# tgsstdio/BirdNest.Audio

Measured on AMD Instinct MI355X. Metric: decoded PCM MSamples/s/GPU (bit-exact) + achieved HBM GB/s vs roofline, higher is better.
Workload: dtype int32; 1 GPU; C2: 1024-frame batches, 44.1 kHz/16-bit stereo, bs 4096, LPC-8, Rice partition order 4 -> FLACDecoder 16-bit LE interleaved PCM; frames_per_batch=1024, compressed_bytes_per_batch=10724000, pcm_bytes_per_batch=16777216, parallelism=corpus of 1 x 1024 batches partitioned per rank (shard.partition) x1

## Files before the change

### birdnest/audio_amd/csrc/bnflac_kernels.hip

```cpp
#include <stdlib.h>
#include <atomic>
#include <mutex>

#include "bnf_bitreader.h"
#include "bnf_crc16.h"
#include "bnf_crc16_tab.h"
#include "bnf_frame.h"
#include "bnf_residual.h"

#define WR_SLOTS 8
#define WR_WIN 256u
struct WR {
    const uint32_t *__restrict__ w;
    uint32_t nblk;
    lds_u32 *ring;
    uint32_t w0;
    uint32_t issued;
    uint32_t landed;
    uint64_t pos;
    uint64_t st[8];
};
DEV uint32_t wr_u(uint32_t v) { return __builtin_amdgcn_readfirstlane(v); }
DEV void wr_issue(WR &r) {
    const uint32_t j = r.issued++;
// ... 617 lines not shown
        uint32_t incl = x;
        for (int o = 1; o < 64; o <<= 1) {
            uint32_t y = __shfl_up(incl, o);
            if ((threadIdx.x & 63) >= (unsigned)o) incl += y;
        }
        if ((threadIdx.x & 63) == 63) wsum[threadIdx.x >> 6] = incl;
        __syncthreads();
        if (threadIdx.x < 16) {
            uint32_t s = wsum[threadIdx.x];
            for (int o = 1; o < 16; o <<= 1) {
                uint32_t y = __shfl_up(s, o, 16);
                if (threadIdx.x >= (unsigned)o) s += y;
            }
            wsum[threadIdx.x] = s;
        }
        __syncthreads();
        uint32_t wprefix = (threadIdx.x >= 64) ? wsum[(threadIdx.x >> 6) - 1] : 0u;
        if (i < n) v[i] = carry + wprefix + incl - x;
        __syncthreads();
        if (threadIdx.x == 1023) carry += wprefix + incl;
        __syncthreads();
    }
    if (threadIdx.x == 0) *total = carry;
}

__global__ void __launch_bounds__(SCAN_THREADS) k_sync_write(const uint8_t *__restrict__ d, uint64_t n,
                                                             const uint32_t *__restrict__ block_offs,
                                                             uint64_t *__restrict__ out, uint32_t cap) {
    __shared__ uint32_t wtot[SCAN_THREADS / 64];
    uint64_t base = ((uint64_t)blockIdx.x * SCAN_THREADS + threadIdx.x) * SCAN_BYTES_PER_THREAD;
    uint32_t c = 0;
    for (int i = 0; i < SCAN_BYTES_PER_THREAD; i++) c += is_sync(d, n, base + i) ? 1u : 0u;
    uint32_t incl = c;
    const uint32_t lane = threadIdx.x & 63;
    for (int o = 1; o < 64; o <<= 1) {
        uint32_t y = __shfl_up(incl, o);
        if (lane >= (unsigned)o) incl += y;
    }
    if (lane == 63) wtot[threadIdx.x >> 6] = incl;
    __syncthreads();
    uint32_t wpre = 0;
    for (uint32_t wv = 0; wv < (threadIdx.x >> 6); wv++) wpre += wtot[wv];
    uint32_t pos = block_offs[blockIdx.x] + wpre + incl - c;
    for (int i = 0; i < SCAN_BYTES_PER_THREAD; i++) {
        if (is_sync(d, n, base + i)) {
            if (pos < cap) out[pos] = base + i;
            pos++;
        }
    }
}

#define PARSE_RD 8
static_assert(PARSE_RD == 8, "pk_ra and the walk's pair steps (slot masks 0x3F3 / 0x1C0C, slot bits 10-12) assume an 8-slot ring");
template <int CPM>
DEV void parse_frame(const uint32_t *__restrict__ words, uint64_t nbytes, const uint64_t *__restrict__ frame_offs,
                     uint32_t nframes, const bnf_stream_params &sp, const uint64_t *__restrict__ out_sample_in,
                     uint64_t base_sample, bnf_frame_info *__restrict__ info, uint32_t ablate, lds_u32 *ring,
                     uint32_t f, uint32_t *__restrict__ crcp) {
    if (f >= nframes) return;
    bnf_frame_info fi;
    fi.status = BNF_ST_OK;
    fi.err = -1;
    fi.frame_off = frame_offs[f];
    fi.resume_bit = 0;
    fi.cached = -1;
    fi.blocksize = fi.sample_rate = fi.channels = fi.assignment = fi.bps = 0;
    fi.number_type = 0;
    fi.unparseable = 0;
    fi.number = 0;
    fi.out_sample = 0;
    fi.crc8 = fi.crc16_calc = fi.crc16_read = fi.crc_ok = 0;
    fi.flags = 0;
    fi.reserved = 0;
    uint32_t ss[8];
#pragma unroll
    for (int c = 0; c < 8; c++) ss[c] = 0;
    const uint64_t limit = nbytes * 8u;
    const uint64_t fbit = fi.frame_off * 8u;
    BR b;
    br_init(b, words, nbytes, ring, threadIdx.x, PARSE_RD);
    CrcP cp;
    crcp_init(cp);
    uint32_t st = parse_header(b, fbit, limit, sp, fi);
    if (st == BNF_ST_ERROR && br_pos(b) > limit) st = BNF_ST_TRUNC;
    if (CPM && crcp != nullptr && st == BNF_ST_OK && fi.channels == 2u && !(ablate & BNF_ABLATE_NO_WALK)) {
        const uint32_t h = (uint32_t)(fi.frame_off & 63u);
        const uint64_t l0 = fi.frame_off & ~(uint64_t)63u, lend = (nbytes + 15u) & ~(uint64_t)15u;
        const u32x4 *g = (const u32x4 *)((const uint8_t *)words + l0);
        u32x4 v[4];
#pragma unroll
        for (uint32_t i = 0; i < 4; i++) {
            v[i] = l0 + 16u * i < lend ? g[i] : u32x4{0u, 0u, 0u, 0u};
            v[i].x &= st_hmask(h, 16u * i);
            v[i].y &= st_hmask(h, 16u * i + 4u);
            v[i].z &= st_hmask(h, 16u * i + 8u);
            v[i].w &= st_hmask(h, 16u * i + 12u);
        }
        cp.wc = (uint32_t)(fi.frame_off >> 6);
        crcp_fold(cp, v);
    }
    if (st == BNF_ST_OK) {
        uint64_t sample;
        if (fi.number_type == 1) sample = fi.number;
        else if (sp.has_stream_info && sp.min_blocksize == sp.max_blocksize) sample = (uint64_t)sp.min_blocksize * fi.number;
        else sample = (uint64_t)fi.blocksize * fi.number;
        fi.out_sample = out_sample_in ? out_sample_in[f] : sample - base_sample;
        uint32_t maxorder = 0;
        bool raw = false;
        for (uint32_t ch = 0; ch < fi.channels; ch++) {
            const uint32_t here = (uint32_t)(br_pos(b) - fbit);
#pragma unroll
            for (int c = 0; c < 8; c++) ss[c] = (uint32_t)c == ch ? here : ss[c];
            if (ch + 1 == fi.channels) {
                const uint32_t x = br_peek(b) >> 24;
                if (!(x & 0x80u) && (x & 0x7Eu) >= 0x40u) maxorder = max(maxorder, ((x >> 1) & 31u) + 1u);
                raw = raw || (x & 0x7Eu) < 4u;
                break;
            }
            if (ablate & BNF_ABLATE_NO_WALK) {
#pragma unroll
                for (int c = 0; c < 8; c++) ss[c] = (uint32_t)c == ch + 1 ? here : ss[c];
                continue;
            }
            SubHdr h;
            int32_t err = -1;
            uint32_t bps = sub_bps(fi, ch);
            st = parse_subframe_head<false>(b, bps, fi.blocksize, limit, h, nullptr, nullptr, err);
            if (st == BNF_ST_OK) {
                if (h.type == T_LPC) maxorder = max(maxorder, h.order);
                raw = raw || h.type == T_CONST || h.type == T_VERB;
                if (!(h.type == T_FIXED || h.type == T_LPC) || h.order > (fi.bps > 16u ? 12u : 8u)) cp.wc = ~0u;
                if (h.type == T_VERB) br_skip(b, (uint64_t)h.bps * fi.blocksize);
                else if (h.type == T_FIXED || h.type == T_LPC) st = skip_residual<CPM != 0>(b, h, fi.blocksize, limit, ablate, cp);
                if (st == BNF_ST_OK && br_pos(b) > limit) st = BNF_ST_TRUNC;
            }
            if (st == BNF_ST_ERROR && br_pos(b) > limit) st = BNF_ST_TRUNC;
            if (st != BNF_ST_OK) {
                if (st == BNF_ST_ERROR) {
                    fi.err = err;
                    fi.resume_bit = br_pos(b);
                }
                break;
            }
        }
        if (maxorder > 16) fi.flags |= BNF_FL_W32;
        else if (maxorder > 8 || (maxorder > 0 && fi.bps > 16)) fi.flags |= BNF_FL_W16;
        else if (fi.channels == 2 && fi.bps <= 16 && !raw) fi.flags |= BNF_FL_ST;
        if (maxorder > 0 && maxorder <= 12 && fi.channels == 2 && fi.bps > 16 && fi.bps <= 24 && !raw) fi.flags |= BNF_FL_SW;
    }
    fi.status = st;
#pragma unroll
    for (int c = 0; c < 8; c++) fi.sub_start[c] = ss[c];
    info[f] = fi;
    if (CPM && crcp) {
        u32x4 o = u32x4{0u, 0u, 0u, 0u}, o2 = u32x4{0u, 0u, 0u, 0u};
        const uint32_t l1 = (uint32_t)(br_pos(b) >> 9);
        if (cp.wc != ~0u && st == BNF_ST_OK) {
            crcp_hook<true>(cp, b, threadIdx.x & 63u, l1);
            const CrcZ z = crcp_z(cp);
            o = u32x4{z.r0, (z.r1 & 0x0FFFFFFFu) | ((uint32_t)(__builtin_popcount(z.px) & 1) << 31),
                      cp.wc - (uint32_t)(fi.frame_off >> 6) + 1u, (uint32_t)fi.frame_off};
            const uint64_t nx = CPM == 2 && f + 1u < nframes ? frame_offs[f + 1u] : 0u;
            if (CPM == 2 && nx >= (uint64_t)cp.wc * 64u && nx <= nbytes && nx - fi.frame_off < (1u << 24))
                o2 = u32x4{(uint32_t)(nx - fi.frame_off),
                           st_crc16_ok<2>((const uint8_t *)words, fi.frame_off, nx, z, (uint64_t)cp.wc * 64u) ? 1u : 0u,
                           (uint32_t)fi.frame_off, 0u};
        }
        *(u32x4 *)(crcp + CRCP_WORDS * (uint64_t)f) = o;
        *(u32x4 *)(crcp + CRCP_WORDS * (uint64_t)f + 4u) = o2;
    }
}

#endif


DEV int32_t sat16(int32_t x) { return (int32_t)(int16_t)min(max(x, -32768), 32767); }
DEV int32_t tr16(int32_t x) { return (int32_t)(int16_t)(uint16_t)(uint32_t)x; }
struct Pred {
    int32_t sh;
    uint32_t order;
    uint32_t wasted;
    bool mmx, wide;
};

template <int T, int W, int NT>
DEV int32_t pred_at(const int32_t (&c)[W], const int32_t (&x)[W], const int32_t (&xt)[4], const Pred &p) {
    int64_t s0 = 0, s1 = 0;
#pragma unroll
    for (int t = 0; t < NT; t++) {
        const int32_t hv = (t < 4) ? xt[(T - 1 - t) & 3] : x[((T - 1 - t) % W + W) % W];
        if (t & 1) s1 += (int64_t)c[t] * (int64_t)hv;
        else s0 += (int64_t)c[t] * (int64_t)hv;
    }
    asm volatile("" : "+v"(s0), "+v"(s1));
    const int64_t S = s0 + s1;
    return p.wide ? (int32_t)(S >> p.sh) : ((int32_t)S >> p.sh);
}
template <int T, int W>
DEV void push_at(int32_t (&x)[W], int32_t (&xt)[4], const Pred &p, int32_t s) {
    x[T % W] = p.mmx ? sat16(s) : s;
    xt[T & 3] = p.mmx ? tr16(s) : s;
}

template <int T, int W, int NT>
DEV void restore_steps(int32_t *row, const int32_t (&c)[W], int32_t (&x)[W], int32_t (&xt)[4], const Pred &p,
                       uint32_t n, uint32_t nv, uint32_t j) {
    if constexpr (T < W) {
        const int32_t v = row[(j + T) * RP];
        const int32_t pr = pred_at<T, W, NT>(c, x, xt, p);
        const int32_t s = (n + (uint32_t)T < p.order) ? v : (int32_t)((uint32_t)v + (uint32_t)pr);
        push_at<T, W>(x, xt, p, s);
        if (j + (uint32_t)T < nv) row[(j + T) * RP] = (int32_t)((uint32_t)s << p.wasted);
        restore_steps<T + 1, W, NT>(row, c, x, xt, p, n, nv, j);
    }
}

template <int T, int W, int NT>
DEV void fused_steps(BR &b, RS &rs, int32_t *row, const int32_t (&c)[W], int32_t (&x)[W], int32_t (&xt)[4],
                     const Pred &p, uint64_t limit, uint32_t &trunc, PendW &pw, uint32_t j) {
    if constexpr (T < W) {
        const int32_t r = rice_fused(b, rs, limit, trunc, &pw);
        const int32_t s = (int32_t)((uint32_t)r + (uint32_t)pred_at<T, W, NT>(c, x, xt, p));
        push_at<T, W>(x, xt, p, s);
        pw.v = (int32_t)((uint32_t)s << p.wasted);
        pw.at = row + (j + T) * RP;
        pw.on = true;
        fused_steps<T + 1, W, NT>(b, rs, row, c, x, xt, p, limit, trunc, pw, j);
    }
}
template <int CH, int W, int NT>
DEV void fused_chunk(BR &b, RS &rs, int32_t *row, const int32_t (&c)[W], int32_t (&x)[W], int32_t (&xt)[4],
                     const Pred &p, uint64_t limit, uint32_t &trunc) {
    PendW pw;
    pw.at = row;
    pw.v = 0;
    pw.on = false;
#pragma unroll 1
    for (uint32_t j = 0; j < (uint32_t)CH; j += W) fused_steps<0, W, NT>(b, rs, row, c, x, xt, p, limit, trunc, pw, j);
    *pw.at = pw.v;
}

template <int CH, int W, int NT>
DEV void restore_chunk(int32_t *row, const int32_t (&c)[W], int32_t (&x)[W], int32_t (&xt)[4], const Pred &p,
                       uint32_t n0, uint32_t nv) {
#pragma unroll 1
    for (uint32_t j = 0; j < (uint32_t)CH; j += W) restore_steps<0, W, NT>(row, c, x, xt, p, n0 + j, nv, j);
}


#ifdef BNF_K_PARSE
template <int CPM>
__global__ void __launch_bounds__(64) k_parse(const uint32_t *__restrict__ words, uint64_t nbytes,
                                              const uint64_t *__restrict__ frame_offs, uint32_t nframes,
                                              bnf_stream_params sp, const uint64_t *__restrict__ out_sample_in,
                                              uint64_t base_sample, bnf_frame_info *__restrict__ info, uint32_t ablate,
                                              const uint32_t *__restrict__ perm, uint32_t *__restrict__ crcp) {
    __shared__ LDS_DMA_ALIGN uint32_t ring[PARSE_RD * RING_LANE_DW];
    const uint32_t slot = blockIdx.x * 64u + threadIdx.x;
    parse_frame<CPM>(words, nbytes, frame_offs, nframes, sp, out_sample_in, base_sample, info, ablate, (lds_u32 *)ring,
                (perm && slot < nframes) ? perm[slot] : slot, crcp);
}

__global__ void __launch_bounds__(64) k_parse_wave(const uint32_t *__restrict__ words, uint64_t nbytes,
                                                   const uint64_t *__restrict__ frame_offs, uint32_t nframes,
                                                   bnf_stream_params sp, const uint64_t *__restrict__ out_sample_in,
                                                   uint64_t base_sample, bnf_frame_info *__restrict__ info,
                                                   uint32_t stats, int seg) {
    __shared__ LDS_DMA_ALIGN uint32_t ring[WR_SLOTS * WR_WIN];
    const uint32_t lane = threadIdx.x, f = blockIdx.x;
    if (f >= nframes) return;
    bnf_frame_info fi;
    fi.status = BNF_ST_OK;
    fi.err = -1;
    fi.frame_off = frame_offs[f];
    fi.resume_bit = 0;
    fi.cached = -1;
    fi.blocksize = fi.sample_rate = fi.channels = fi.assignment = fi.bps = 0;
    fi.number_type = 0;
    fi.unparseable = 0;
    fi.number = 0;
    fi.out_sample = 0;
    fi.crc8 = fi.crc16_calc = fi.crc16_read = fi.crc_ok = 0;
    fi.flags = 0;
    fi.reserved = 0;
    uint32_t ss[8];
#pragma unroll
    for (int c = 0; c < 8; c++) ss[c] = 0;
    const uint64_t limit = nbytes * 8u;
    const uint64_t fbit = fi.frame_off * 8u;
    WR r;
    wr_init(r, words, nbytes, (lds_u32 *)ring, fbit);
    pw_stat(r, stats != 0u, 4);
    uint32_t st = parse_header(r, fbit, limit, sp, fi);
    if (st == BNF_ST_ERROR && br_pos(r) > limit) st = BNF_ST_TRUNC;
    if (st == BNF_ST_OK) {
        uint64_t sample;
        if (fi.number_type == 1) sample = fi.number;
        else if (sp.has_stream_info && sp.min_blocksize == sp.max_blocksize) sample = (uint64_t)sp.min_blocksize * fi.number;
        else sample = (uint64_t)fi.blocksize * fi.number;
        fi.out_sample = out_sample_in ? out_sample_in[f] : sample - base_sample;
        uint32_t maxorder = 0;
        bool raw = false;
        const uint32_t nch = wr_u(fi.channels), bs = wr_u(fi.blocksize);
        for (uint32_t ch = 0; ch < nch; ch++) {
            const uint32_t here = (uint32_t)(br_pos(r) - fbit);
#pragma unroll
            for (int c = 0; c < 8; c++) ss[c] = (uint32_t)c == ch ? here : ss[c];
            if (ch + 1 == nch) {
                const uint32_t x = br_peek(r) >> 24;
                if (!(x & 0x80u) && (x & 0x7Eu) >= 0x40u) maxorder = max(maxorder, ((x >> 1) & 31u) + 1u);
                raw = raw || (x & 0x7Eu) < 4u;
                break;
            }
            SubHdr h;
            int32_t err = -1;
            st = parse_subframe_head<false>(r, sub_bps(fi, ch), bs, limit, h, nullptr, nullptr, err);
            if (st == BNF_ST_OK) {
                if (h.type == T_LPC) maxorder = max(maxorder, h.order);
                raw = raw || h.type == T_CONST || h.type == T_VERB;
                if (h.type == T_VERB) br_skip(r, (uint64_t)h.bps * bs);
                else if (h.type == T_FIXED || h.type == T_LPC) {
                    const uint64_t t0 = stats ? __builtin_amdgcn_s_memtime() : 0ull;
                    st = wave_skip_residual(r, h, bs, limit, stats != 0u, seg);
                    if (stats) pw_stat(r, true, 5, __builtin_amdgcn_s_memtime() - t0);
                }
                if (st == BNF_ST_OK && br_pos(r) > limit) st = BNF_ST_TRUNC;
            }
            if (st == BNF_ST_ERROR && br_pos(r) > limit) st = BNF_ST_TRUNC;
            if (st != BNF_ST_OK) {
                if (st == BNF_ST_ERROR) {
                    fi.err = err;
                    fi.resume_bit = br_pos(r);
                }
                break;
            }
        }
        if (maxorder > 16) fi.flags |= BNF_FL_W32;
        else if (maxorder > 8 || (maxorder > 0 && fi.bps > 16)) fi.flags |= BNF_FL_W16;
        else if (fi.channels == 2 && fi.bps <= 16 && !raw) fi.flags |= BNF_FL_ST;
        if (maxorder > 0 && maxorder <= 12 && fi.channels == 2 && fi.bps > 16 && fi.bps <= 24 && !raw) fi.flags |= BNF_FL_SW;
    }
    fi.status = st;
#pragma unroll
    for (int c = 0; c < 8; c++) fi.sub_start[c] = ss[c];
    wait_vm();
    pw_flush(r, stats != 0u);
    const uint32_t *src = (const uint32_t *)&fi;
    uint32_t v = 0;
#pragma unroll
    for (int i = 0; i < 32; i++) v = lane == (uint32_t)i ? src[i] : v;
    if (lane < 32u) ((uint32_t *)&info[f])[lane] = v;
}


__global__ void __launch_bounds__(64) k_fill_bad(const bnf_frame_info *__restrict__ info, uint32_t nframes,
                                                 bnf_stream_params sp, int fmt, uint8_t *__restrict__ out,
                                                 uint64_t out_bytes) {
    const uint32_t f = blockIdx.x * 64u + threadIdx.x;
    bool bad = false;
    uint64_t start = 0, n = 0;
    if (f < nframes) {
        const uint32_t st = info[f].status;
        if ((st == BNF_ST_ERROR || st == BNF_ST_TRUNC) && info[f].sub_start[0] != 0u) {
            const uint32_t C = info[f].channels, bsz = info[f].blocksize;
            const uint64_t os = info[f].out_sample;
            switch (fmt) {
            case BNF_OUT_PLANAR32: start = os * sp.channels * 4u; n = (uint64_t)min(C, sp.channels) * bsz * 4u; break;
            case BNF_OUT_INTERLEAVED32: start = os * sp.channels * 4u; n = (uint64_t)sp.channels * bsz * 4u; break;
            case BNF_OUT_FLACDECODER: start = os * (C == 2 ? 4u : 2u); n = (uint64_t)bsz * (C == 2 ? 4u : 2u); break;
            default: {
                const uint32_t fb = sp.bps == 24 ? 3u : 2u;
                start = os * sp.channels * fb;
                n = (uint64_t)bsz * sp.channels * fb;
            }
            }
            bad = n != 0 && start <= out_bytes && n <= out_bytes - start;
        }
    }
    uint64_t m = __ballot(bad);
    while (m) {
        const uint32_t l = (uint32_t)__builtin_ctzll(m);
        m &= m - 1u;
        const uint64_t s0 = __shfl(start, l), n0 = __shfl(n, l);
        for (uint64_t i = threadIdx.x; i < n0; i += 64u) out[s0 + i] = 0;
    }
}
#endif


template <int FMT, int CH> constexpr uint32_t pack_fast_stores() { return FMT == BNF_OUT_INTERLEAVED32 ? CH / 4 : CH / 8; }

DEV void pack4(const int32_t (&v)[4], uint32_t fb, uint32_t (&d)[3]) {
    if (fb == 3) {
        d[0] = ((uint32_t)v[0] & 0xFFFFFFu) | ((uint32_t)v[1] << 24);
        d[1] = (((uint32_t)v[1] >> 8) & 0xFFFFu) | ((uint32_t)v[2] << 16);
        d[2] = (((uint32_t)v[2] >> 16) & 0xFFu) | ((uint32_t)v[3] << 8);
    } else {
        d[0] = ((uint32_t)v[0] & 0xFFFFu) | ((uint32_t)v[1] << 16);
        d[1] = ((uint32_t)v[2] & 0xFFFFu) | ((uint32_t)v[3] << 16);
        d[2] = 0;
    }
}

template <int FMT, int CH>
DEV uint32_t pack_lane(const int32_t *lds, uint32_t lane, uint32_t chn_lanes, uint32_t n0, bool fok, uint32_t bs,
                       uint32_t C, uint32_t as, uint64_t os, uint32_t stream_channels, uint32_t fr_bytes,
                       uint8_t *__restrict__ out) {
    const uint32_t lg = __builtin_ctz(chn_lanes);
    const uint32_t per = (uint32_t)CH >> lg;
    const uint32_t fl = lane >> lg, part = lane & (chn_lanes - 1u);
// ... 537 lines not shown
            part = crc16_shift(part, f_off + len - s1);
        }
    }
    uint32_t acc = part;
    for (uint32_t o = 1; o < chn_lanes; o <<= 1) acc ^= __shfl_xor(acc, o);
    if ((ablate & BNF_ABLATE_NO_CRC16) && last && t_status == BNF_ST_OK) acc = t_crc_read;
    if (last) {
        bnf_frame_info fo = info[f];
        fo.status = t_status;
        if (t_status == BNF_ST_ERROR) fo.err = t_err;
        if (t_resume_set) fo.resume_bit = t_resume;
        if (t_status == BNF_ST_OK) {
            fo.crc16_read = t_crc_read;
            fo.crc16_calc = acc;
            fo.crc_ok = (acc == t_crc_read) ? 1u : 0u;
            if (!fo.crc_ok) t_bad[fl] = 2;
        }
        info[f] = fo;
    }
    __syncthreads();
    if (tmon && lane == 0) {
        const uint64_t t_end = tnow(tmon);
        atomicAdd(&g_stats[8], (unsigned long long)(t_loop - t_start));
        atomicAdd(&g_stats[9], (unsigned long long)tm_dec);
        atomicAdd(&g_stats[10], (unsigned long long)tm_ref);
        atomicAdd(&g_stats[11], (unsigned long long)tm_pack);
        atomicAdd(&g_stats[12], (unsigned long long)(t_end - t_loopend));
    }
    for (uint32_t fl2 = 0; fl2 < fpb; fl2++) {
        if (t_bad[fl2] != 2 || !t_ok[fl2]) continue;
        uint64_t nbytes_fr, start;
        const uint32_t C = t_ch[fl2], bsz = t_bs[fl2];
        switch (fmt) {
        case BNF_OUT_PLANAR32: start = t_out[fl2] * sp.channels * 4u; nbytes_fr = (uint64_t)C * bsz * 4u; break;
        case BNF_OUT_INTERLEAVED32: start = t_out[fl2] * sp.channels * 4u; nbytes_fr = (uint64_t)sp.channels * bsz * 4u; break;
        case BNF_OUT_FLACDECODER: start = t_out[fl2] * (C == 2 ? 4u : 2u); nbytes_fr = (uint64_t)bsz * (C == 2 ? 4u : 2u); break;
        default: {
            const uint32_t fb = sp.bps == 24 ? 3u : 2u;
            start = t_out[fl2] * sp.channels * fb;
            nbytes_fr = (uint64_t)bsz * sp.channels * fb;
        }
        }
        for (uint64_t i = lane; i < nbytes_fr; i += DEC_LANES) out[start + i] = 0;
    }
    wait_vm();
}

template <int MAXW, int CHK, int RD>
__global__ void __launch_bounds__(DEC_LANES, 2) k_decode(const uint32_t *__restrict__ words, uint64_t nbytes,
                                                      uint32_t nframes, bnf_stream_params sp, uint32_t chn_lanes,
                                                      int fmt, uint8_t *__restrict__ out, uint64_t out_bytes,
                                                      bnf_frame_info *__restrict__ info,
                                                      const uint32_t *__restrict__ perm, uint32_t ablate,
                                                      const uint32_t *__restrict__ seg) {
    __shared__ LDS_DMA_ALIGN uint32_t ring[RD * RING_LANE_DW];
    __shared__ int32_t lds[CHK * RP];
    if (seg) {
        const uint32_t fpb = DEC_LANES >> __builtin_ctz(chn_lanes);
        const uint32_t c = MAXW == 32 ? 3u : MAXW == 16 ? 2u : (ablate & BNF_MODE_NOST) ? 1u : 0u;
        const uint32_t lo = c ? seg[c * 64u - 1u] / fpb : 0u, end = (seg[c * 64u + 63u] + fpb - 1u) / fpb;
        if (blockIdx.x < lo || blockIdx.x >= end) return;
    }
    decode_block<MAXW, CHK, RD>(blockIdx.x, ring, lds, words, nbytes, nframes, sp, chn_lanes, fmt, out, out_bytes, info,
                                perm, ablate);
}

template <int MAXW, int CHK, int RD>
__global__ void __launch_bounds__(DEC_LANES, 2) k_decode_list(const uint32_t *__restrict__ words, uint64_t nbytes,
                                                           bnf_stream_params sp, uint32_t chn_lanes, int fmt,
                                                           uint8_t *__restrict__ out, uint64_t out_bytes,
                                                           bnf_frame_info *__restrict__ info,
                                                           const uint32_t *__restrict__ list, uint32_t ablate) {
    __shared__ LDS_DMA_ALIGN uint32_t ring[RD * RING_LANE_DW];
    __shared__ int32_t lds[CHK * RP];
    const uint32_t cnt = __builtin_amdgcn_readfirstlane(list[0]);
    const uint32_t fpb = DEC_LANES >> __builtin_ctz(chn_lanes);
    const uint32_t nb = (cnt + fpb - 1u) / fpb;
    for (uint32_t blk = blockIdx.x; blk < nb; blk += gridDim.x) {
        decode_block<MAXW, CHK, RD>(blk, ring, lds, words, nbytes, cnt, sp, chn_lanes, fmt, out, out_bytes, info, list + 4,
                                    ablate | BNF_MODE_LIST | BNF_MODE_WREDO);
        __syncthreads();
    }
}

template <int MAXW, int CHK, int RD>
__global__ void __launch_bounds__(DEC_LANES, 2) k_decode_seg(const uint32_t *__restrict__ words, uint64_t nbytes,
                                                          uint32_t nframes, bnf_stream_params sp, uint32_t chn_lanes,
                                                          int fmt, uint8_t *__restrict__ out, uint64_t out_bytes,
                                                          bnf_frame_info *__restrict__ info,
                                                          const uint32_t *__restrict__ perm, uint32_t ablate,
                                                          const uint32_t *__restrict__ seg) {
    __shared__ LDS_DMA_ALIGN uint32_t ring[RD * RING_LANE_DW];
    __shared__ int32_t lds[CHK * RP];
    const uint32_t fpb = DEC_LANES >> __builtin_ctz(chn_lanes);
    const uint32_t lo = __builtin_amdgcn_readfirstlane(seg[2u * 64u - 1u]) / fpb;
    const uint32_t end = (__builtin_amdgcn_readfirstlane(seg[3u * 64u + 63u]) + fpb - 1u) / fpb;
    for (uint32_t blk = lo + blockIdx.x; blk < end; blk += gridDim.x) {
        decode_block<MAXW, CHK, RD>(blk, ring, lds, words, nbytes, nframes, sp, chn_lanes, fmt, out, out_bytes, info,
                                    perm, ablate);
        __syncthreads();
    }
}

#ifdef BNF_K_PARSE
#define CHAIN_WIN (1u << 16)
#define KEY_OK 0x10000u

__global__ void __launch_bounds__(256) k_gap_crc(const uint8_t *__restrict__ bytes, uint64_t nbytes,
                                                 const uint64_t *__restrict__ cand, uint32_t ncand,
                                                 uint32_t *__restrict__ gap_w) {
    __shared__ uint16_t tab[8 * 256];
    for (uint32_t i = threadIdx.x; i < 8u * 256u; i += 256u) tab[i] = (&g_crc16_tab[0][0])[i];
    __syncthreads();
    const lds_u16 *T = (const lds_u16 *)(lds_u32 *)tab;
    const uint32_t g = blockIdx.x * 4u + (threadIdx.x >> 6);
    const uint32_t lane = threadIdx.x & 63u;
    if (g >= ncand) return;
    const uint64_t b0 = cand[g];
    const uint64_t b1 = g + 1 < ncand ? cand[g + 1] : nbytes;
    const uint64_t slice = ((b1 - b0 + 63u) / 64u + 15u) & ~15ull;
    const uint64_t s0 = min(b1, b0 + slice * lane);
    const uint64_t s1 = min(b1, s0 + slice);
    uint32_t c = s0 < s1 ? crc16_shift(crc16_range(bytes, s0, s1, T), nbytes - s1) : 0u;
    for (int o = 32; o > 0; o >>= 1) c ^= __shfl_xor(c, o);
    if (lane == 0) gap_w[g] = c;
}

__global__ void __launch_bounds__(1024) k_chain_keys(uint32_t *__restrict__ v, uint32_t n,
                                                     const bnf_frame_info *__restrict__ info) {
    __shared__ uint32_t wsum[16];
    __shared__ uint32_t carry;
    if (threadIdx.x == 0) carry = 0;
    __syncthreads();
    for (uint32_t base = 0; base < n; base += 1024) {
        const uint32_t i = base + threadIdx.x;
        const uint32_t x = i < n ? v[i] : 0u;
        uint32_t incl = x;
        for (int o = 1; o < 64; o <<= 1) {
            const uint32_t y = __shfl_up(incl, o);
            if ((threadIdx.x & 63) >= (unsigned)o) incl ^= y;
        }
        if ((threadIdx.x & 63) == 63) wsum[threadIdx.x >> 6] = incl;
        __syncthreads();
        if (threadIdx.x == 0)
            for (int w = 1; w < 16; w++) wsum[w] ^= wsum[w - 1];
        __syncthreads();
// ... 279 lines not shown
        const uint64_t ex64 = ms_block_excl<uint64_t, false>(i < n ? a[i] : 0ull, ws64, tot64);
        if (i <= n && ao) ao[i] = asum[blockIdx.x] + ex64;
    }
}

DEV uint32_t ms_lower(const uint64_t *__restrict__ cand, uint32_t n, uint64_t x) {
    uint32_t lo = 0, hi = n;
    while (lo < hi) {
        const uint32_t mid = lo + ((hi - lo) >> 1);
        if (cand[mid] < x) lo = mid + 1u;
        else hi = mid;
    }
    return lo;
}

__global__ void __launch_bounds__(256) k_ms_ranges(const uint64_t *__restrict__ cand, const uint32_t *__restrict__ ctl,
                                                   const bnf_stream_desc *__restrict__ sd, uint32_t nstreams,
                                                   uint32_t *__restrict__ clo, uint32_t *__restrict__ chi) {
    const uint32_t s = blockIdx.x * 256u + threadIdx.x;
    if (s >= nstreams) return;
    const uint32_t n = ms_n(ctl);
    uint32_t lo = 0, hi = 0;
    if (n) {
        const bnf_stream_desc d = sd[s];
        lo = ms_lower(cand, n, d.begin);
        hi = d.end - d.begin >= 2u ? ms_lower(cand, n, d.end - 1u) : lo;
    }
    clo[s] = lo;
    chi[s] = hi;
}

__global__ void __launch_bounds__(256) k_ms_owner(const uint32_t *__restrict__ ctl, const uint32_t *__restrict__ clo,
                                                  const uint32_t *__restrict__ chi, uint32_t nstreams,
                                                  int32_t *__restrict__ seg) {
    const uint32_t i = blockIdx.x * 256u + threadIdx.x;
    if (i >= ms_n(ctl)) return;
    uint32_t lo = 0, hi = nstreams;
    while (lo < hi) {
        const uint32_t mid = lo + ((hi - lo) >> 1);
        if (chi[mid] <= i) lo = mid + 1u;
        else hi = mid;
    }
    seg[i] = (lo < nstreams && clo[lo] <= i) ? (int32_t)lo : -1;
}

__global__ void __launch_bounds__(64) k_ms_parse(const uint32_t *__restrict__ words, uint64_t nbytes,
                                                 const uint64_t *__restrict__ cand, const uint32_t *__restrict__ ctl,
                                                 bnf_stream_params sp, const int32_t *__restrict__ seg,
                                                 bnf_frame_info *__restrict__ info) {
    __shared__ LDS_DMA_ALIGN uint32_t ring[PARSE_RD * RING_LANE_DW];
    const uint32_t i = blockIdx.x * 64u + threadIdx.x, n = ms_n(ctl);
    if (blockIdx.x * 64u >= n) return;
    const bool mine = i < n && seg[i] >= 0;
    parse_frame<0>(words, nbytes, cand, n, sp, nullptr, 0, info, 0u, (lds_u32 *)ring, mine ? i : ~0u, nullptr);
}

__global__ void __launch_bounds__(256) k_ms_gap_crc(const uint8_t *__restrict__ bytes, uint64_t nbytes,
                                                    const uint64_t *__restrict__ cand, const uint32_t *__restrict__ ctl,
                                                    uint32_t *__restrict__ gap_w) {
    __shared__ uint16_t tab[8 * 256];
    const uint32_t ncand = ms_n(ctl);
    if (blockIdx.x * 4u >= ncand) return;
    for (uint32_t i = threadIdx.x; i < 8u * 256u; i += 256u) tab[i] = (&g_crc16_tab[0][0])[i];
    __syncthreads();
    const lds_u16 *T = (const lds_u16 *)(lds_u32 *)tab;
    const uint32_t g = blockIdx.x * 4u + (threadIdx.x >> 6);
    const uint32_t lane = threadIdx.x & 63u;
    if (g >= ncand) return;
    const uint64_t b0 = cand[g];
    const uint64_t b1 = g + 1 < ncand ? cand[g + 1] : nbytes;
    const uint64_t slice = ((b1 - b0 + 63u) / 64u + 15u) & ~15ull;
    const uint64_t s0 = min(b1, b0 + slice * lane);
    const uint64_t s1 = min(b1, s0 + slice);
    uint32_t c = s0 < s1 ? crc16_shift(crc16_range(bytes, s0, s1, T), nbytes - s1) : 0u;
    for (int o = 32; o > 0; o >>= 1) c ^= __shfl_xor(c, o);
    if (lane == 0) gap_w[g] = c;
}

__global__ void __launch_bounds__(256) k_ms_succ(const uint64_t *__restrict__ cand, const uint32_t *__restrict__ ctl,
                                                 const uint32_t *__restrict__ key, const int32_t *__restrict__ seg,
                                                 const bnf_stream_desc *__restrict__ sd, const uint32_t *__restrict__ chi,
                                                 int32_t *__restrict__ succ, int32_t *__restrict__ head) {
    const uint32_t i = blockIdx.x * 256u + threadIdx.x, lane = threadIdx.x & 63u;
    const bool live = i < ms_n(ctl);
    const uint32_t want = live ? key[i] : 0u;
    const bool valid = (want & KEY_OK) != 0u;
    const int32_t s = valid ? seg[i] : -1;
    const bool after = valid && cand[i] >= sd[s].first_offset;
    const uint64_t votes = __ballot(after);
    if (votes) {
        const int first = __ffsll((unsigned long long)votes) - 1;
        const int32_t s_first = __shfl(s, first);
        if (__ballot(after && s != s_first) == 0ull) {
            if ((int)lane == first) atomicMin(&head[s], (int32_t)i);
        } else if (after) {
            atomicMin(&head[s], (int32_t)i);
        }
    }
    if (!live) return;
    int32_t r = -1;
    if (valid) {
        const uint32_t jend = (uint32_t)min((uint64_t)chi[s], (uint64_t)i + 1u + CHAIN_WIN);
        for (uint32_t j = i + 1; j < jend; j++)
            if (key[j] == want) {
                r = (int32_t)j;
                break;
            }
// ... 665 lines not shown
    bool sl0, sl1;
    const uint32_t n0 = st_rice_pair(z0, u0a, u0b, sl0), n1 = st_rice_pair(z1, u1a, u1b, sl1);
    const uint32_t laneb = lane << 4;
    st_adv_nc(z0.b, n0, laneb);
    st_adv_nc(z1.b, n1, laneb);
    constexpr bool CHK = (T & 2) == 0;
    const bool ld0 = CHK && z0.b.wi >= z0.b.vlim, ld1 = CHK && z1.b.wi >= z1.b.vlim;
    st_next_word(z0.b);
    st_next_word(z1.b);
    if (__builtin_expect(any_lane(sl0 || sl1 || ld0 || ld1), 0)) {
        st_rare_pair(z0, sl0, ld0, u0a, u0b, limit, trunc, nqt, lane);
        st_rare_pair(z1, sl1, ld1, u1a, u1b, limit, trunc, nqt, lane);
    }
    st_lpc_out<T, FMT, AS, PO, NPK>(z0, z1, u0a, u1a, L, R, as_uni, as_u, as, dst, nbase, al, bs, store, pk, pre0, pre1, anyw);
    st_lpc_out<T + 1, FMT, AS, PO, NPK>(z0, z1, u0b, u1b, L, R, as_uni, as_u, as, dst, nbase, al, bs, store, pk, pre0, pre1, anyw);
}

template <int T, int FMT>
DEV bool st_gen_step(StCh &z0, StCh &z1, int32_t (&L)[4], int32_t (&R)[4], uint64_t limit, uint32_t &trunc,
                     uint32_t nst, bool as_uni, uint32_t as_u, uint32_t as, uint8_t *dst, uint32_t n, bool valid,
                     bool al, uint32_t bs, bool store) {
    const bool v = valid && n < bs;
    int32_t s0 = 0, s1 = 0;
    if (v) {
        int32_t p0, p1;
        st_dot2<T>(z0, z1, p0, p1);
        if (n < z0.order()) s0 = (int32_t)(int16_t)z0.q[T];
        else s0 = (int32_t)((uint32_t)st_next(z0, bs, limit, trunc, nst) + (uint32_t)(p0 >> z0.sh));
        if (n < z1.order()) s1 = (int32_t)(int16_t)z1.q[T];
        else s1 = (int32_t)((uint32_t)st_next(z1, bs, limit, trunc, nst) + (uint32_t)(p1 >> z1.sh));
        st_range(z0, s0, s0);
        st_range(z1, s1, s1);
        z0.q[T] = __builtin_amdgcn_perm(z0.q[(T + 7) & 7], (uint32_t)s0, 0x05040100u);
        z1.q[T] = __builtin_amdgcn_perm(z1.q[(T + 7) & 7], (uint32_t)s1, 0x05040100u);
    }
    L[T & 3] = (int32_t)((uint32_t)s0 << z0.wasted());
    R[T & 3] = (int32_t)((uint32_t)s1 << z1.wasted());
    bool stored = false;
    if ((T & 3) == 3) {
        const uint32_t nq = n - 3u;
        const uint32_t nv = (valid && nq < bs) ? min(4u, bs - nq) : 0u;
        st_decor4(as_uni, as_u, as, L, R);
        if (store) stored = st_emit4<FMT>(dst, nq, nv, al, bs, L, R);
    }
    return stored;
}

template <int FMT>
__global__ void __launch_bounds__(64, 2) k_decode_st(const uint32_t *__restrict__ words, uint64_t nbytes,
                                                     uint32_t nframes, bnf_stream_params sp, uint32_t chn_lanes,
                                                     uint8_t *__restrict__ out, uint64_t out_bytes,
                                                     bnf_frame_info *__restrict__ info,
                                                     const uint32_t *__restrict__ perm, uint32_t ablate,
                                                     const uint32_t *__restrict__ crcp) {
    constexpr bool STG = (FMT == BNF_OUT_FLACDECODER || FMT == BNF_OUT_FILEREADER);
    constexpr uint32_t ST_SPG = (FMT == BNF_OUT_INTERLEAVED32 || FMT == BNF_OUT_PLANAR32) ? 2u : 1u;
    __shared__ LDS_DMA_ALIGN uint32_t ring[2 * ST_RD * RING_LANE_DW + 1024];
    static_assert((ST_RD * RING_LANE_DW * 4) % 1024 == 0, "channel 1's ring base must stay 1 KiB aligned (LDS-DMA)");
    const uint32_t lane = threadIdx.x;
    const uint32_t slot = blockIdx.x * 64u + lane;
    const uint32_t f = (perm && slot < nframes) ? perm[slot] : slot;
    const uint64_t limit = nbytes * 8u;
    bnf_frame_info fi;
    const bool have = f < nframes;
    if (have) fi = info[f];
    const bool mine = have && fi.status == BNF_ST_OK && (fi.flags & BNF_FL_ST) && !(fi.flags & BNF_FL_REDO) &&
                      (!(ablate & BNF_MODE_WREDO) || (fi.flags & BNF_FL_WAVE_REDO));
    if (!__any(mine)) return;

    uint64_t stride = 0;
    bool ok = mine && fi.channels == 2 && chn_lanes >= 2;
    if (FMT == BNF_OUT_FLACDECODER) { stride = 4; ok = ok && fi.bps == 16 && sp.channels >= 2; }
    else if (FMT == BNF_OUT_FILEREADER) { stride = 4; ok = ok && sp.channels == 2 && sp.bps == 16; }
    else if (FMT == BNF_OUT_INTERLEAVED32) { stride = 8; ok = ok && sp.channels == 2; }
    else { stride = 4ull * sp.channels; ok = ok && sp.channels == 2; }
    const uint32_t bs = ok ? fi.blocksize : 0u;
    const uint64_t os = ok ? fi.out_sample : 0u;
    ok = ok && (os + bs) * stride <= out_bytes;
    uint8_t *dst = out + os * stride;
    const bool al = (((uintptr_t)dst) & 15u) == 0 && (FMT != BNF_OUT_PLANAR32 || (bs & 3u) == 0);

    StCh z0, z1;
    lds_u32 *ring0 = (lds_u32 *)ring, *ring1 = (lds_u32 *)ring + ST_RD * RING_LANE_DW;
    br_init(z0.b, words, nbytes, ring0, lane, ST_RD);
    br_init(z1.b, words, nbytes, ring1, lane, ST_RD);
    z0.b.stats = z1.b.stats = (ablate & BNF_ABLATE_STATS) != 0;
    STAT(z0.b.stats, 5);
    const bool tmon = z0.b.stats;
    const uint64_t t_start = tnow(tmon);
    uint64_t tm_dec = 0, tm_ref = 0, tm_pack = 0;
    if (ok) {
        br_seek(z0.b, fi.frame_off * 8u + fi.sub_start[0]);
        ok = st_setup(z0, sub_bps(fi, 0), bs, limit);
    }
    if (ok) {
        br_seek(z1.b, fi.frame_off * 8u + fi.sub_start[1]);
        ok = st_setup(z1, sub_bps(fi, 1), bs, limit);
    }
    const uint32_t as = ok ? fi.assignment : 0u;
    const bool anyw = any_lane(ok && (z0.wasted() | z1.wasted()) != 0u);
    const uint32_t as_u = __builtin_amdgcn_readfirstlane(as);
    const bool as_uni = !any_lane(ok && as != as_u);
    const int as_fix = (as_uni && !anyw && as_u <= 3u) ? (int)as_u : -1;
    lds_u32x4 *stg = (lds_u32x4 *)((lds_u32 *)ring + 2u * ST_RD * RING_LANE_DW);
    static_assert(sizeof(ring) >= (2 * ST_RD * RING_LANE_DW + 1024) * 4, "the flush's 4 KB staging tile lies past the two rings");

    uint32_t mybs = ok ? bs : 0u;
    for (int o = 32; o > 0; o >>= 1) mybs = max(mybs, (uint32_t)__shfl_xor(mybs, o));
    const uint32_t nchunks = (mybs + ST2_CHK - 1) / ST2_CHK;
    uint32_t trunc = 0;
    const bool fold_on = crcp != nullptr && !(ablate & (BNF_ABLATE_NO_STFOLD | BNF_ABLATE_NO_CRC16));
    StFold fold;
    st_fold_start(fold, z1.b, words, crcp, f, ok ? fi.frame_off : 0u, fold_on && ok);
    wait_vm();
// ... 129 lines not shown
    const uint64_t t_loopend = tnow(tmon);

    uint32_t crc_read = 0;
    uint64_t end_byte = 0, resume = 0;
    if (ok) {
        if (z0.mx > ST_LIM || z0.mn < -ST_LIM - 1 || z1.mx > ST_LIM || z1.mn < -ST_LIM - 1) ok = false;
        if (trunc) ok = false;
    }
    if (ok) {
        while (z1.parts_left()) {
            const uint32_t kk = br_read(z1.b, z1.plen());
            if (kk >= z1.pesc()) br_read(z1.b, 5);
            z1.pw++;
        }
        const uint32_t padbits = (uint32_t)((8u - (br_pos(z1.b) & 7u)) & 7u);
        const uint32_t zp = br_read(z1.b, padbits);
        if (br_pos(z1.b) > limit || zp != 0) ok = false;
        end_byte = br_pos(z1.b) >> 3;
        crc_read = br_read(z1.b, 16);
        if (br_pos(z1.b) > limit) ok = false;
        resume = br_pos(z1.b);
    }
    const uint32_t fl_flags = mine ? info[f].flags : 0u;
    const uint64_t frame_off = ok ? info[f].frame_off : 0u;
    uint32_t crc = crc_read;
    if (ok && !(ablate & BNF_ABLATE_NO_CRC16)) {
        bool used;
#ifdef BNFLAC_CRC_FOLD_CHECK
        CrcZ ra = CrcZ{0u, 0u, 0u}, rb = CrcZ{0u, 0u, 0u};
        StFold none;
        none.c = CrcZ{0u, 0u, 0u};
        none.fl = ~0u;
        bool unused;
        const bool va = st_crc16_run((const uint8_t *)words, crcp, f, frame_off, end_byte + 2u, fold, used, &ra);
        const bool vb = st_crc16_run((const uint8_t *)words, crcp, f, frame_off, end_byte + 2u, none, unused, &rb);
        const bool differ = used && (va != vb || ra.r0 != rb.r0 || ((ra.r1 ^ rb.r1) & 0x0FFFFFFFu) != 0u ||
                                     (__builtin_popcount(ra.px ^ rb.px) & 1) != 0);
        if (differ) atomicAdd(&g_stats[7], 1ull);
        if (!va) ok = false;
#else
        if (!st_crc16_run((const uint8_t *)words, crcp, f, frame_off, end_byte + 2u, fold, used)) ok = false;
#endif
        if (z0.b.stats && used) atomicAdd(&g_stats[6], 1ull);
    }
    if (ok && crc != crc_read) ok = false;
    if (ok) {
        info[f].resume_bit = resume;
        info[f].crc16_read = crc_read;
        info[f].crc16_calc = crc;
        info[f].crc_ok = 1u;
    } else if (mine) {
        info[f].flags = fl_flags | BNF_FL_REDO;
    }
    if (tmon && lane == 0) {
        const uint64_t t_end = tnow(tmon);
        atomicAdd(&g_stats[8], (unsigned long long)(t_loop - t_start));
        atomicAdd(&g_stats[9], (unsigned long long)tm_dec);
        atomicAdd(&g_stats[10], (unsigned long long)tm_ref);
        atomicAdd(&g_stats[11], (unsigned long long)tm_pack);
        atomicAdd(&g_stats[12], (unsigned long long)(t_end - t_loopend));
    }
}

#ifdef BNF_K_SW
#define SW_TAPS 12
struct StW {
    BR b;
    int32_t c[SW_TAPS];
    int32_t x[16];
    int32_t sh;
    uint32_t wide;
    uint32_t k, km, k1, k32;
    uint32_t esc, left, pidx, nparts, psamples, plen, pesc, porder, order;
    uint32_t wasted;
};

DEV bool sw_setup(StW &z, uint32_t bps, uint32_t bs, uint64_t limit) {
    SubHdr h;
    int32_t warm[SW_TAPS], coef[SW_TAPS], err = -1;
    const uint32_t st = parse_subframe_head<true, SW_TAPS>(z.b, bps, bs, limit, h, warm, coef, err);
    if (st != BNF_ST_OK) return false;
    if (h.type != T_FIXED && h.type != T_LPC) return false;
    if (h.order > SW_TAPS) return false;
    if (h.type == T_LPC && h.path == P_MMX16) return false;
    if (h.type == T_LPC && h.path == P_WIDE && ((uint32_t)h.shift & 0xFFu) >= 32u) return false;
#pragma unroll
    for (int t = 0; t < SW_TAPS; t++) z.c[t] = (h.type == T_LPC && (uint32_t)t < h.order) ? coef[t] : 0;
    if (h.type == T_FIXED) {
        const uint32_t o = h.order;
        z.c[0] = o == 1 ? 1 : o == 2 ? 2 : o == 3 ? 3 : o == 4 ? 4 : 0;
        z.c[1] = o == 2 ? -1 : o == 3 ? -3 : o == 4 ? -6 : 0;
        z.c[2] = o == 3 ? 1 : o == 4 ? 4 : 0;
        z.c[3] = o == 4 ? -1 : 0;
    }
#pragma unroll
    for (int t = 0; t < 16; t++) z.x[t] = (t < SW_TAPS && (uint32_t)t < h.order) ? warm[t < SW_TAPS ? t : 0] : 0;
    z.wide = (h.type == T_LPC && h.path == P_WIDE) ? 1u : 0u;
    z.sh = h.type == T_LPC ? (int32_t)((uint32_t)h.shift & (z.wide ? 0xFFu : 31u)) : 0;
    z.order = h.order;
    z.wasted = h.wasted;
    z.porder = h.porder;
    z.nparts = 1u << h.porder;
    z.psamples = h.porder ? bs >> h.porder : bs - h.order;
    z.plen = h.rice2 ? 5u : 4u;
    z.pesc = h.rice2 ? 31u : 15u;
    z.left = 0;
// ... 187 lines not shown
        st_rare(z1, sl1, ld1, u1, limit, trunc, nq, lane);
    }
    const int32_t s0 = (int32_t)(((u0 >> 1) ^ (0u - (u0 & 1u))) + (uint32_t)p0);
    const int32_t s1 = (int32_t)(((u1 >> 1) ^ (0u - (u1 & 1u))) + (uint32_t)p1);
    z0.x[T] = s0;
    z1.x[T] = s1;
    L[T & 7] = (int32_t)((uint32_t)s0 << z0.wasted);
    R[T & 7] = (int32_t)((uint32_t)s1 << z1.wasted);
    if ((T & 7) == 7) {
#pragma unroll
        for (int i = 0; i < 8; i++) sw_decor<AS>(as, L[i], R[i]);
        if (LN) {
            uint32_t d[12];
            sw_pack24(L, R, d);
            sw_line_group(stg, lane, odd, carry, q, d, T >> 3, dst + (uint64_t)nbase * 6u);
        } else if (sto) {
            sw_emit8<FMT>(dst, nbase + (uint32_t)T - 7u, 8u, al, bs, L, R);
        }
    }
}

template <int T, int FMT>
DEV bool sw_gen_step(StW &z0, StW &z1, int32_t (&L)[8], int32_t (&R)[8], uint64_t limit, uint32_t &trunc, uint32_t nst,
                     uint32_t as, uint8_t *dst, uint32_t n, bool valid, bool al, uint32_t bs, bool sto) {
    const bool v = valid && n < bs;
    int32_t s0 = 0, s1 = 0;
    if (v) {
        if (n < z0.order) s0 = z0.x[T];
        else s0 = (int32_t)((uint32_t)st_next(z0, limit, trunc, nst) + (uint32_t)sw_full<T, 2>(z0));
        if (n < z1.order) s1 = z1.x[T];
        else s1 = (int32_t)((uint32_t)st_next(z1, limit, trunc, nst) + (uint32_t)sw_full<T, 2>(z1));
        z0.x[T] = s0;
        z1.x[T] = s1;
    }
    L[T & 7] = (int32_t)((uint32_t)s0 << z0.wasted);
    R[T & 7] = (int32_t)((uint32_t)s1 << z1.wasted);
    bool stored = false;
    if ((T & 7) == 7) {
        const uint32_t nq = n - 7u;
        const uint32_t nv = (valid && nq < bs) ? min(8u, bs - nq) : 0u;
#pragma unroll
        for (int q = 0; q < 8; q++) decorrelate(as, L[q], R[q]);
        if (sto) stored = sw_emit8<FMT>(dst, nq, nv, al, bs, L, R);
    }
    return stored;
}

template <int FMT>
__global__ void __launch_bounds__(64, 2) k_decode_sw(const uint32_t *__restrict__ words, uint64_t nbytes,
                                                     uint32_t nframes, bnf_stream_params sp, uint32_t chn_lanes,
                                                     uint8_t *__restrict__ out, uint64_t out_bytes,
                                                     bnf_frame_info *__restrict__ info,
                                                     const uint32_t *__restrict__ perm, uint32_t ablate,
                                                     const uint32_t *__restrict__ crcp) {
    constexpr uint32_t SPG = sw_stores8<FMT>();
    __shared__ LDS_DMA_ALIGN uint32_t ring[2 * ST_RD * RING_LANE_DW + 1024];
    const uint32_t lane = threadIdx.x;
    const uint32_t slot = blockIdx.x * 64u + lane;
    const uint32_t f = (perm && slot < nframes) ? perm[slot] : slot;
    const uint64_t limit = nbytes * 8u;
    bnf_frame_info fi;
    const bool have = f < nframes;
    if (have) fi = info[f];
    const bool mine = have && fi.status == BNF_ST_OK && (fi.flags & BNF_FL_SW) && !(fi.flags & BNF_FL_REDO) &&
                      (!(ablate & BNF_MODE_WREDO) || (fi.flags & BNF_FL_WAVE_REDO));
    if (!__any(mine)) return;

    uint64_t stride = 8;
    bool ok = mine && fi.channels == 2 && chn_lanes >= 2 && sp.channels == 2;
    if (FMT == BNF_OUT_FILEREADER) { stride = 6; ok = ok && sp.bps == 24; }
    const uint32_t bs = ok ? fi.blocksize : 0u;
    const uint64_t os = ok ? fi.out_sample : 0u;
    ok = ok && (os + bs) * stride <= out_bytes;
    uint8_t *dst = out + os * stride;
    const bool hot = (ablate & BNF_ABLATE_HOT_WINDOW) != 0 && out_bytes >= (1u << 20);
    if (hot) dst = out + (uint64_t)(blockIdx.x & 7u) * 65536u + lane * 1024u;
    const bool al = (((uintptr_t)dst) & 15u) == 0 && (FMT != BNF_OUT_PLANAR32 || (bs & 3u) == 0);
    const bool all_al = !any_lane(ok && !al);

    StW z0, z1;
    lds_u32 *ring0 = (lds_u32 *)ring, *ring1 = (lds_u32 *)ring + ST_RD * RING_LANE_DW;
    br_init(z0.b, words, nbytes, ring0, lane, ST_RD);
    br_init(z1.b, words, nbytes, ring1, lane, ST_RD);
    if (ok) {
        br_seek(z0.b, fi.frame_off * 8u + fi.sub_start[0]);
        ok = sw_setup(z0, sub_bps(fi, 0), bs, limit);
    }
    if (ok) {
        br_seek(z1.b, fi.frame_off * 8u + fi.sub_start[1]);
        ok = sw_setup(z1, sub_bps(fi, 1), bs, limit);
    }
    const uint32_t as = ok ? fi.assignment : 0u;
    const uint32_t as_u = __builtin_amdgcn_readfirstlane(as);
    const bool as_uni = !any_lane(ok && as != as_u);
    const bool all_wide = !any_lane(ok && !(z0.wide && z1.wide));
    const int fix = (as_uni && all_wide && as_u <= 3u) ? (int)as_u : -1;

    uint32_t mybs = ok ? bs : 0u;
    for (int o = 32; o > 0; o >>= 1) mybs = max(mybs, (uint32_t)__shfl_xor(mybs, o));
    const uint32_t nchunks = (mybs + ST_CHK - 1) / ST_CHK;
    uint32_t trunc = 0;
    const bool sto = !(ablate & BNF_ABLATE_NO_STORE);
    const bool line = FMT == BNF_OUT_FILEREADER && sto && !hot && all_al && !(ablate & BNF_ABLATE_SW_NO_LINE) &&
                      !any_lane(ok && (((uintptr_t)dst) & 63u) != 0);
    lds_u32x4 *stg = (lds_u32x4 *)((lds_u32 *)ring + 2u * ST_RD * RING_LANE_DW);
    static_assert(sizeof(ring) >= (2 * ST_RD * RING_LANE_DW + 1024) * 4, "the flush's 4 KB staging tile lies past the two rings");
    static_assert(sizeof(ring) >= (2u * ST_RD * RING_LANE_DW + 1024u) * 4u, "line slots past the rings");
    SwLn q;
    SwRuns runs;
    if (line) sw_runs(runs, ok ? (uint64_t)(uintptr_t)dst : 0ull, bs, lane);
    bool carry = false, cvalid = false;
    uint32_t carry_b = 0;
// ... 104 lines not shown
    }

    if (carry && cvalid) {
        gst128((uint64_t)(uintptr_t)dst + carry_b, q.c0);
        gst128((uint64_t)(uintptr_t)dst + carry_b + 16u, q.c1);
    }

    uint32_t crc_read = 0;
    uint64_t end_byte = 0, resume = 0;
    if (ok && trunc) ok = false;
    if (ok) {
        while (z1.pidx < z1.nparts) {
            const uint32_t kk = br_read(z1.b, z1.plen);
            if (kk >= z1.pesc) br_read(z1.b, 5);
            z1.pidx++;
        }
        const uint32_t padbits = (uint32_t)((8u - (br_pos(z1.b) & 7u)) & 7u);
        const uint32_t zp = br_read(z1.b, padbits);
        if (br_pos(z1.b) > limit || zp != 0) ok = false;
        end_byte = br_pos(z1.b) >> 3;
        crc_read = br_read(z1.b, 16);
        if (br_pos(z1.b) > limit) ok = false;
        resume = br_pos(z1.b);
    }
    uint32_t crc = crc_read;
    if (ok && !(ablate & BNF_ABLATE_NO_CRC16) && !st_crc16_frame((const uint8_t *)words, crcp, f, fi.frame_off, end_byte + 2u)) ok = false;
    if (ok && crc != crc_read) ok = false;
    if (ok) {
        info[f].resume_bit = resume;
        info[f].crc16_read = crc_read;
        info[f].crc16_calc = crc;
        info[f].crc_ok = 1u;
    } else if (mine) {
        info[f].flags = fi.flags | BNF_FL_REDO;
    }
}
#endif
#endif

#ifdef BNF_DEC_W
#if BNF_DEC_W == 8
#define TU_FN(name) name##_w8
#elif BNF_DEC_W == 16
#define TU_FN(name) name##_w16
#else
#define TU_FN(name) name##_w32
#endif
#define DEC_W BNF_DEC_W
#define DEC_RD 8
bnf_tu_ops TU_FN(bnf_ops_decode) = {tu_upload_tables, tu_stats};
extern "C" {
hipError_t TU_FN(bnf_launch_decode)(const uint32_t *words, uint64_t nbytes, uint32_t nframes, bnf_stream_params sp,
                                    uint32_t chn_lanes, int fmt, uint8_t *out, uint64_t out_bytes, bnf_frame_info *info,
                                    const uint32_t *perm, uint32_t mode, const uint32_t *seg, hipStream_t s) {
    const uint32_t fpb = DEC_LANES / chn_lanes;
    const uint32_t nb = (nframes + fpb - 1) / fpb;
    if (!perm || (DEC_W == 8 && !(mode & (BNF_MODE_NOST | BNF_MODE_STREDO)))) seg = nullptr;
    hipLaunchKernelGGL((k_decode<DEC_W, 32, DEC_RD>), dim3(nb), dim3(DEC_LANES), 0, s, words, nbytes, nframes, sp, chn_lanes,
                       fmt, out, out_bytes, info, perm, (bnf_ablate_flags() & BNF_ABLATE_K_DECODE) | (mode & BNF_MODE_K_DECODE), seg);
    return hipGetLastError();
}
#if BNF_DEC_W == 32
hipError_t bnf_launch_decode_list(const uint32_t *words, uint64_t nbytes, uint32_t nframes, bnf_stream_params sp,
                                      uint32_t chn_lanes, int fmt, uint8_t *out, uint64_t out_bytes, bnf_frame_info *info,
                                      const uint32_t *list, uint32_t mode, hipStream_t s) {
    const uint32_t fpb = DEC_LANES / chn_lanes;
    const uint32_t nb = std::min<uint32_t>((nframes + fpb - 1) / fpb, 512u);
    hipLaunchKernelGGL((k_decode_list<DEC_W, 32, DEC_RD>), dim3(std::max(nb, 1u)), dim3(DEC_LANES), 0, s, words, nbytes, sp,
                       chn_lanes, fmt, out, out_bytes, info, list, (bnf_ablate_flags() & BNF_ABLATE_K_DECODE) | (mode & BNF_MODE_K_DECODE));
    return hipGetLastError();
}
hipError_t bnf_launch_decode_seg(const uint32_t *words, uint64_t nbytes, uint32_t nframes, bnf_stream_params sp,
                                     uint32_t chn_lanes, int fmt, uint8_t *out, uint64_t out_bytes, bnf_frame_info *info,
                                     const uint32_t *perm, uint32_t mode, const uint32_t *seg, hipStream_t s) {
    const uint32_t fpb = DEC_LANES / chn_lanes;
    const uint32_t nb = std::min<uint32_t>((nframes + fpb - 1) / fpb, 512u);
    hipLaunchKernelGGL((k_decode_seg<DEC_W, 32, DEC_RD>), dim3(std::max(nb, 1u)), dim3(DEC_LANES), 0, s, words, nbytes,
                       nframes, sp, chn_lanes, fmt, out, out_bytes, info, perm, (bnf_ablate_flags() & BNF_ABLATE_K_DECODE) | (mode & BNF_MODE_K_DECODE) | BNF_MODE_SEG, seg);
    return hipGetLastError();
}
#endif
}
#endif

#ifdef BNF_ST_FD
#if BNF_ST_FD
#define TU_FN(name) name##_st_fd
#else
#define TU_FN(name) name##_st_any
#endif
bnf_tu_ops TU_FN(bnf_ops_decode) = {tu_upload_tables, tu_stats};
extern "C" {
hipError_t TU_FN(bnf_launch_decode)(const uint32_t *words, uint64_t nbytes, uint32_t nframes, bnf_stream_params sp,
                                    uint32_t chn_lanes, int fmt, uint8_t *out, uint64_t out_bytes, bnf_frame_info *info,
                                    const uint32_t *perm, uint32_t mode, const uint32_t *crcp, hipStream_t s) {
    const dim3 grid((nframes + 63) / 64);
    const uint32_t ab = (bnf_ablate_flags() & BNF_ABLATE_K_DECODE_ST) | (mode & BNF_MODE_K_DECODE_ST);
    if (ab & BNF_ABLATE_NO_ST) return hipSuccess;
#if BNF_ST_FD
    (void)fmt;
    hipLaunchKernelGGL(k_decode_st<BNF_OUT_FLACDECODER>, grid, dim3(64), 0, s, words, nbytes, nframes, sp, chn_lanes, out, out_bytes, info, perm, ab, crcp);
#else
    switch (fmt) {
    case BNF_OUT_PLANAR32:
        hipLaunchKernelGGL(k_decode_st<BNF_OUT_PLANAR32>, grid, dim3(64), 0, s, words, nbytes, nframes, sp, chn_lanes, out, out_bytes, info, perm, ab, crcp);
        break;
    case BNF_OUT_INTERLEAVED32:
        hipLaunchKernelGGL(k_decode_st<BNF_OUT_INTERLEAVED32>, grid, dim3(64), 0, s, words, nbytes, nframes, sp, chn_lanes, out, out_bytes, info, perm, ab, crcp);
        break;
    default:
        hipLaunchKernelGGL(k_decode_st<BNF_OUT_FILEREADER>, grid, dim3(64), 0, s, words, nbytes, nframes, sp, chn_lanes, out, out_bytes, info, perm, ab, crcp);
        break;
    }
#endif
    return hipGetLastError();
}
}
#endif

#ifdef BNF_K_SW
bnf_tu_ops bnf_ops_decode_sw = {tu_upload_tables, tu_stats};
extern "C" {
hipError_t bnf_launch_decode_sw(const uint32_t *words, uint64_t nbytes, uint32_t nframes, bnf_stream_params sp,
                                    uint32_t chn_lanes, int fmt, uint8_t *out, uint64_t out_bytes, bnf_frame_info *info,
                                    const uint32_t *perm, uint32_t mode, const uint32_t *crcp, hipStream_t s) {
    const dim3 grid((nframes + 63) / 64);
    const uint32_t ab = (bnf_ablate_flags() & BNF_ABLATE_K_DECODE_SW) | (mode & BNF_MODE_K_DECODE_SW);
    switch (fmt) {
    case BNF_OUT_PLANAR32:
        hipLaunchKernelGGL(k_decode_sw<BNF_OUT_PLANAR32>, grid, dim3(64), 0, s, words, nbytes, nframes, sp, chn_lanes, out, out_bytes, info, perm, ab, crcp);
        break;
    case BNF_OUT_INTERLEAVED32:
        hipLaunchKernelGGL(k_decode_sw<BNF_OUT_INTERLEAVED32>, grid, dim3(64), 0, s, words, nbytes, nframes, sp, chn_lanes, out, out_bytes, info, perm, ab, crcp);
        break;
    case BNF_OUT_FILEREADER:
        hipLaunchKernelGGL(k_decode_sw<BNF_OUT_FILEREADER>, grid, dim3(64), 0, s, words, nbytes, nframes, sp, chn_lanes, out, out_bytes, info, perm, ab, crcp);
        break;
    default: return hipErrorInvalidValue;
    }
    return hipGetLastError();
}
}
#endif

#ifdef BNF_K_PARSE
static std::atomic<uint32_t> g_ablate{0xFFFFFFFFu};
static const bnf_tu_ops *const g_tus[] = {&bnf_ops_decode_w8,  &bnf_ops_decode_w32, &bnf_ops_decode_st_fd, &bnf_ops_decode_st_any,
                                          &bnf_ops_decode_w16, &bnf_ops_decode_sw,  &bnf_ops_decode_sys};
extern "C" {
uint32_t bnf_ablate_flags(void) {
    uint32_t v = g_ablate.load(std::memory_order_relaxed);
    if (v == 0xFFFFFFFFu) {
        const char *e = getenv("BNFLAC_ABLATE");
        v = e ? (uint32_t)strtoul(e, nullptr, 0) : 0u;
        g_ablate.store(v, std::memory_order_relaxed);
    }
    return v;
}

hipError_t bnf_upload_tables(const uint8_t *crc8, const uint16_t *crc16x8, const uint16_t *xpow) {
    hipError_t e = tu_upload_tables(crc8, crc16x8, xpow);
    for (const bnf_tu_ops *tu : g_tus)
        if (e == hipSuccess) e = tu->upload_tables(crc8, crc16x8, xpow);
    return e;
}

hipError_t bnf_launch_sync_scan(const uint8_t *d, uint64_t n, uint32_t *d_block_counts, uint32_t *d_total,
                                uint64_t *d_out, uint32_t cap, hipStream_t s) {
    const uint64_t per_block = (uint64_t)SCAN_THREADS * SCAN_BYTES_PER_THREAD;
    const uint32_t nblocks = (uint32_t)((n + per_block - 1) / per_block);
    if (nblocks == 0) return hipMemsetAsync(d_total, 0, sizeof(uint32_t), s);
    hipLaunchKernelGGL(k_sync_count, dim3(nblocks), dim3(SCAN_THREADS), 0, s, d, n, d_block_counts);
    hipLaunchKernelGGL(k_scan_u32, dim3(1), dim3(1024), 0, s, d_block_counts, nblocks, d_total);
    hipLaunchKernelGGL(k_sync_write, dim3(nblocks), dim3(SCAN_THREADS), 0, s, d, n, d_block_counts, d_out, cap);
    return hipGetLastError();
}

uint32_t bnf_scan_blocks(uint64_t n) {
    const uint64_t per_block = (uint64_t)SCAN_THREADS * SCAN_BYTES_PER_THREAD;
    return (uint32_t)((n + per_block - 1) / per_block);
}

void bnf_set_ablate(uint32_t v) { g_ablate.store(v, std::memory_order_relaxed); }

hipError_t bnf_stats(uint64_t *out16, int reset) {
    for (int i = 0; i < 16; i++) out16[i] = 0;
    hipError_t e = hipSuccess;
    for (const bnf_tu_ops *tu : g_tus)
        if (e == hipSuccess) e = tu->stats(out16, reset);
    return e;
}

}

#define ORDER_NB 256
DEV uint32_t order_bucket(uint32_t work) { return 63u - min(work >> 8, 63u); }
template <int MODE>
DEV uint32_t order_key(const bnf_frame_info *__restrict__ info, const uint8_t *__restrict__ bytes, uint64_t nbytes,
                       const uint64_t *__restrict__ offs, uint32_t f) {
    if (MODE == 0) {
        const uint32_t st = info[f].status, fl = info[f].flags, bs = info[f].blocksize;
        const uint32_t c = st != BNF_ST_OK ? 1u : (fl & BNF_FL_W32) ? 3u : (fl & BNF_FL_W16) ? 2u : (fl & BNF_FL_ST) ? 0u : 1u;
        return c * 64u + order_bucket(bs ? bs - 1u : 0u);
    }
    const uint64_t o = offs[f];
    if (o + 16u > nbytes) return 63u;
    const uint32_t code = bytes[o + 2] >> 4, chc = bytes[o + 3] >> 4;
    const uint32_t C = chc < 8u ? chc + 1u : 2u;
    uint32_t bs = 0;
    if (code == 1u) bs = 192u;
    else if (code >= 2u && code <= 5u) bs = 576u << (code - 2u);
    else if (code >= 8u) bs = 256u << (code - 8u);
    else if (code == 6u || code == 7u) {
        const uint32_t lead = bytes[o + 4];
        const uint32_t n = lead < 0x80u ? 1u : (uint32_t)__builtin_clz(~(lead << 24));
        const uint64_t q = o + 4u + min(n, 7u);
        bs = (code == 6u ? bytes[q] : ((uint32_t)bytes[q] << 8 | bytes[q + 1])) + 1u;
    }
    return order_bucket((bs * (C > 1u ? C - 1u : 1u)) >> 1);
}
template <int MODE>
__global__ void __launch_bounds__(256) k_order_count(const bnf_frame_info *__restrict__ info,
                                                     const uint8_t *__restrict__ bytes, uint64_t nbytes,
                                                     const uint64_t *__restrict__ offs, uint32_t nframes,
                                                     uint32_t *__restrict__ hist) {
    __shared__ uint32_t h[ORDER_NB];
    h[threadIdx.x] = 0;
    __syncthreads();
    const uint32_t f = blockIdx.x * 256u + threadIdx.x;
    if (f < nframes) atomicAdd(&h[order_key<MODE>(info, bytes, nbytes, offs, f)], 1u);
    __syncthreads();
    if (h[threadIdx.x]) atomicAdd(&hist[threadIdx.x], h[threadIdx.x]);
}
__global__ void __launch_bounds__(ORDER_NB) k_order_scan(uint32_t *__restrict__ hist, uint32_t *__restrict__ cls) {
    __shared__ uint32_t t[ORDER_NB];
    const uint32_t i = threadIdx.x;
    const uint32_t v = hist[i];
    t[i] = v;
    __syncthreads();
    for (uint32_t o = 1; o < ORDER_NB; o <<= 1) {
        const uint32_t a = i >= o ? t[i - o] : 0u;
        __syncthreads();
        t[i] += a;
        __syncthreads();
    }
    hist[i] = t[i] - v;
    if (cls && i == ORDER_NB - 1u) {
        cls[0] = t[3u * 64u - 1u] - t[2u * 64u - 1u];
        cls[1] = t[4u * 64u - 1u] - t[3u * 64u - 1u];
        cls[2] = t[ORDER_NB - 1u];
        cls[3] = t[2u * 64u - 1u] - t[64u - 1u];
    }
}
template <int MODE>
__global__ void __launch_bounds__(256) k_order_place(const bnf_frame_info *__restrict__ info,
                                                     const uint8_t *__restrict__ bytes, uint64_t nbytes,
                                                     const uint64_t *__restrict__ offs, uint32_t nframes,
                                                     uint32_t *__restrict__ off, uint32_t *__restrict__ perm) {
    __shared__ uint32_t h[ORDER_NB], base[ORDER_NB];
    h[threadIdx.x] = 0;
    __syncthreads();
    const uint32_t f = blockIdx.x * 256u + threadIdx.x;
    uint32_t k = 0, r = 0;
    if (f < nframes) {
        k = order_key<MODE>(info, bytes, nbytes, offs, f);
        r = atomicAdd(&h[k], 1u);
    }
    __syncthreads();
    if (h[threadIdx.x]) base[threadIdx.x] = atomicAdd(&off[threadIdx.x], h[threadIdx.x]);
    __syncthreads();
    if (f < nframes) perm[base[k] + r] = f;
}
template <int MODE>
static hipError_t launch_order(const bnf_frame_info *info, const uint8_t *bytes, uint64_t nbytes, const uint64_t *offs,
                               uint32_t nframes, uint32_t *order, const uint32_t **perm, hipStream_t s,
                               uint32_t *cls = nullptr) {
    uint32_t *hist = order, *pm = order + ORDER_NB;
    hipError_t e = hipMemsetAsync(hist, 0, ORDER_NB * sizeof(uint32_t), s);
    if (e != hipSuccess) return e;
    const dim3 g((nframes + 255) / 256);
    hipLaunchKernelGGL(k_order_count<MODE>, g, dim3(256), 0, s, info, bytes, nbytes, offs, nframes, hist);
    hipLaunchKernelGGL(k_order_scan, dim3(1), dim3(ORDER_NB), 0, s, hist, cls);
    hipLaunchKernelGGL(k_order_place<MODE>, g, dim3(256), 0, s, info, bytes, nbytes, offs, nframes, hist, pm);
    *perm = pm;
    return hipGetLastError();
}

struct SideQ {
    hipStream_t st[3];
    hipEvent_t fork, join[3];
    uint32_t *cls;
};
static std::mutex g_side_mu;
static std::atomic<uint64_t> g_seg_launches{0};
static SideQ g_side[64];
static int decode_fork_mode() {
    static const int m = [] {
        const char *e = getenv("BNFLAC_DECODE_SERIAL");
        if (e && atoi(e) != 0) return 0;
        const char *f = getenv("BNFLAC_DECODE_FORK");
        return (f && atoi(f) == 1) ? 1 : 2;
    }();
    return m;
}
static SideQ *side_queue() {
    int dev = 0;
    if (hipGetDevice(&dev) != hipSuccess || dev < 0 || dev >= 64) return nullptr;
    SideQ &q = g_side[dev];
    if (!q.st[1]) {
        SideQ n = {};
        bool ok = hipEventCreateWithFlags(&n.fork, hipEventDisableTiming) == hipSuccess;
        for (int i = 0; i < 3 && ok; i++)
            ok = hipStreamCreateWithFlags(&n.st[i], hipStreamNonBlocking) == hipSuccess &&
                 hipEventCreateWithFlags(&n.join[i], hipEventDisableTiming) == hipSuccess;
        if (ok && hipHostMalloc((void **)&n.cls, 64, hipHostMallocCoherent) != hipSuccess) n.cls = nullptr;
        if (n.cls) n.cls[0] = n.cls[1] = n.cls[2] = n.cls[3] = ~0u;
        if (!ok) {
            for (int i = 0; i < 3; i++) {
                if (n.join[i]) (void)hipEventDestroy(n.join[i]);
                if (n.st[i]) (void)hipStreamDestroy(n.st[i]);
            }
            if (n.fork) (void)hipEventDestroy(n.fork);
            return nullptr;
        }
        q = n;
    }
    return &q;
}

static std::atomic<int> g_parse_wave{-1};
static bool use_parse_wave(uint32_t nframes, const bnf_stream_params &sp) {
    int m = g_parse_wave.load(std::memory_order_relaxed);
    if (m < 0) {
        const char *e = getenv("BNFLAC_PARSE_WAVE");
        m = e ? (atoi(e) ? 1 : 0) : 2;
        g_parse_wave.store(m, std::memory_order_relaxed);
    }
    if (m != 2) return m == 1;
    return nframes <= 8192u || (nframes <= 32768u && (sp.bps > 16u || sp.channels > 2u));
}

#define SYS_AUTO_WAVES 1024u
static std::atomic<int> g_decode_sys{-1};
static bool use_decode_sys(uint32_t nframes, const bnf_stream_params &sp, uint32_t chn_lanes) {
    int m = g_decode_sys.load(std::memory_order_relaxed);
    if (m < 0) {
        const char *e = getenv("BNFLAC_DECODE_SYS");
        m = e ? (atoi(e) ? 1 : 0) : 2;
        g_decode_sys.store(m, std::memory_order_relaxed);
    }
    if (chn_lanes > 8u || m == 0) return false;
    if (m == 1) return true;
    static const uint32_t lim = [] {
        const char *e = getenv("BNFLAC_SYS_WAVES");
        return e ? (uint32_t)strtoul(e, nullptr, 0) : SYS_AUTO_WAVES;
    }();
    uint64_t scale = 1;
    if (sp.has_stream_info && sp.max_blocksize > sp.min_blocksize && sp.max_blocksize > 4096u) scale = sp.max_blocksize / 2048u;
    return (uint64_t)nframes * chn_lanes < (uint64_t)lim * 64u * scale;
}

static std::atomic<int> g_crc_mode{-1};
static int crc_mode() {
    int m = g_crc_mode.load(std::memory_order_relaxed);
    if (m < 0) {
        const char *e = getenv("BNFLAC_CRC_MODE");
        m = e ? std::min(std::max(atoi(e), 0), 3) : 3;
        g_crc_mode.store(m, std::memory_order_relaxed);
    }
    return m;
}

extern "C" {
int bnf_crc_mode() { return crc_mode(); }
void bnf_set_crc_mode(int mode) { g_crc_mode.store(mode < 0 ? -1 : std::min(mode, 3), std::memory_order_relaxed); }
uint64_t bnf_decode_seg_launches() { return g_seg_launches.load(std::memory_order_relaxed); }
void bnf_set_decode_sys(int mode) { g_decode_sys.store(mode < 0 ? 2 : (mode ? 1 : 0), std::memory_order_relaxed); }
void bnf_set_parse_wave(int mode) { g_parse_wave.store(mode < 0 ? 2 : (mode ? 1 : 0), std::memory_order_relaxed); }
hipError_t bnf_parse_wave_stats(uint64_t *out8, int reset) {
    hipError_t e = hipMemcpyFromSymbol(out8, HIP_SYMBOL(g_pw_stats), 8 * sizeof(uint64_t));
    if (e == hipSuccess && reset) {
        static const uint64_t z[8] = {0};
        e = hipMemcpyToSymbol(HIP_SYMBOL(g_pw_stats), z, sizeof z);
    }
    return e;
}
hipError_t bnf_launch_parse(const uint32_t *words, uint64_t nbytes, const uint64_t *frame_offs, uint32_t nframes,
                            bnf_stream_params sp, const uint64_t *out_sample_in, uint64_t base_sample,
                            bnf_frame_info *info, uint32_t *order, uint32_t *crcp, bool *handed, hipStream_t s) {
    if (handed) *handed = false;
    if (!nframes || !nbytes) return hipSuccess;
    if (use_parse_wave(nframes, sp)) {
        static const uint32_t pws = getenv("BNFLAC_PW_STATS") ? 1u : 0u;
        static const int seg = [] { const char *e = getenv("BNFLAC_PW_SEG"); return e ? atoi(e) : 0; }();
        hipLaunchKernelGGL(k_parse_wave, dim3(nframes), dim3(64), 0, s, words, nbytes, frame_offs, nframes, sp,
                           out_sample_in, base_sample, info, pws, seg);
        return hipGetLastError();
    }
    const uint32_t *perm = nullptr;
    const bool fixed_bs = sp.has_stream_info && sp.min_blocksize == sp.max_blocksize;
    if (order && !fixed_bs) {
        hipError_t e = launch_order<1>(nullptr, (const uint8_t *)words, nbytes, frame_offs, nframes, order, &perm, s);
        if (e != hipSuccess) return e;
    }
    int cm = crcp ? crc_mode() : 0;
    if (cm == 3 && sp.bps <= 16u) {
        std::lock_guard<std::mutex> lk(g_side_mu);
        const SideQ *sq = side_queue();
        if (sq && sq->cls) {
            const uint32_t w16 = __atomic_load_n(&sq->cls[0], __ATOMIC_RELAXED), w32 = __atomic_load_n(&sq->cls[1], __ATOMIC_RELAXED),
                           n = __atomic_load_n(&sq->cls[2], __ATOMIC_RELAXED);
            if (w16 != ~0u && w32 != ~0u && n != ~0u && 4ull * ((uint64_t)w16 + w32) >= n && n) cm = 0;
        }
    }
    if (cm == 3) cm = 1;
    if (handed) *handed = cm != 0;
    const dim3 g((nframes + 63) / 64);
    if (cm == 2)
        hipLaunchKernelGGL(k_parse<2>, g, dim3(64), 0, s, words, nbytes, frame_offs, nframes, sp, out_sample_in,
                           base_sample, info, bnf_ablate_flags() & BNF_ABLATE_K_PARSE, perm, crcp);
    else if (cm == 1)
        hipLaunchKernelGGL(k_parse<1>, g, dim3(64), 0, s, words, nbytes, frame_offs, nframes, sp, out_sample_in,
                           base_sample, info, bnf_ablate_flags() & BNF_ABLATE_K_PARSE, perm, crcp);
    else
        hipLaunchKernelGGL(k_parse<0>, g, dim3(64), 0, s, words, nbytes, frame_offs, nframes, sp, out_sample_in,
                           base_sample, info, bnf_ablate_flags() & BNF_ABLATE_K_PARSE, perm, nullptr);
    return hipGetLastError();
}

hipError_t bnf_launch_fill_bad(const bnf_frame_info *info, uint32_t nframes, bnf_stream_params sp, int fmt,
                               uint8_t *out, uint64_t out_bytes, hipStream_t s) {
    if (!nframes) return hipSuccess;
    hipLaunchKernelGGL(k_fill_bad, dim3((nframes + 63) / 64), dim3(64), 0, s, info, nframes, sp, fmt, out, out_bytes);
    return hipGetLastError();
}

hipError_t bnf_launch_decode(const uint32_t *words, uint64_t nbytes, uint32_t nframes, bnf_stream_params sp,
                             uint32_t chn_lanes, int fmt, uint8_t *out, uint64_t out_bytes, bnf_frame_info *info,
                             uint32_t *order, const uint32_t *crcp, hipStream_t s) {
    if (!nframes || !nbytes) return hipSuccess;
    uint32_t mode = 0;
    if (order && use_decode_sys(nframes, sp, chn_lanes)) {
        const uint32_t *perm = nullptr;
        uint32_t *list = order + 256u + nframes;
        hipError_t e = hipMemsetAsync(list, 0, 16, s);
        if (e == hipSuccess) e = launch_order<0>(info, nullptr, 0, nullptr, nframes, order, &perm, s);
        if (e == hipSuccess)
            e = bnf_launch_decode_sys(words, nbytes, nframes, sp, chn_lanes, fmt, out, out_bytes, info, perm, list, mode, s);
        if (e == hipSuccess)
            e = bnf_launch_decode_list(words, nbytes, nframes, sp, chn_lanes, fmt, out, out_bytes, info, list, mode, s);
        return e;
    }
    static const bool seg_on = [] { const char *e = getenv("BNFLAC_DECODE_SEG"); return !e || atoi(e) != 0; }();
    const int fm = sp.bps > 16 ? 0 : decode_fork_mode();
    const bool sw = sp.bps > 16 && sp.bps <= 24 && fmt != BNF_OUT_FLACDECODER && !(bnf_ablate_flags() & BNF_ABLATE_NO_SW);
    std::unique_lock<std::mutex> lk(g_side_mu, std::defer_lock);
    SideQ *sq = nullptr;
    if (fm) {
        lk.lock();
        sq = side_queue();
    }
    uint32_t *cls = (sq && seg_on && order) ? sq->cls : nullptr;
    const bool seg_only = cls && __atomic_load_n(&cls[0], __ATOMIC_RELAXED) == 0u &&
                          __atomic_load_n(&cls[1], __ATOMIC_RELAXED) == 0u;
    const uint32_t *perm = nullptr;
    hipError_t e = hipSuccess;
    if (order) e = launch_order<0>(info, nullptr, 0, nullptr, nframes, order, &perm, s, cls);
    const uint32_t *seg = (perm && seg_on) ? order : nullptr;
    if (seg_only) {
        sq = nullptr;
        lk.unlock();
    }
    const bool w8split = sq && seg && cls && __atomic_load_n(&cls[3], __ATOMIC_RELAXED) != 0u &&
                         !(bnf_ablate_flags() & BNF_ABLATE_NO_W8SPLIT);
    const int nside = w8split ? 3 : 2;
    auto fork = [&]() -> hipError_t {
        hipError_t r = hipEventRecord(sq->fork, s);
        for (int i = 0; i < nside && r == hipSuccess; i++) r = hipStreamWaitEvent(sq->st[i], sq->fork, 0);
        if (r == hipSuccess)
            r = bnf_launch_decode_w32(words, nbytes, nframes, sp, chn_lanes, fmt, out, out_bytes, info, perm, mode, seg, sq->st[1]);
        if (r == hipSuccess)
            r = bnf_launch_decode_w16(words, nbytes, nframes, sp, chn_lanes, fmt, out, out_bytes, info, perm, mode, seg, sq->st[0]);
        if (r == hipSuccess && w8split)
            r = bnf_launch_decode_w8(words, nbytes, nframes, sp, chn_lanes, fmt, out, out_bytes, info, perm,
                                      mode | BNF_MODE_NOST, seg, sq->st[2]);
        for (int i = 0; i < nside && r == hipSuccess; i++) r = hipEventRecord(sq->join[i], sq->st[i]);
        return r;
    };
    if (sq && fm == 2 && e == hipSuccess) e = fork();
    if (sw) {
        if (e == hipSuccess) e = bnf_launch_decode_sw(words, nbytes, nframes, sp, chn_lanes, fmt, out, out_bytes, info, perm, mode, crcp, s);
        mode |= BNF_MODE_SW;
    }
    if (e == hipSuccess)
        e = fmt == BNF_OUT_FLACDECODER
                ? bnf_launch_decode_st_fd(words, nbytes, nframes, sp, chn_lanes, fmt, out, out_bytes, info, perm, mode, crcp, s)
                : bnf_launch_decode_st_any(words, nbytes, nframes, sp, chn_lanes, fmt, out, out_bytes, info, perm, mode, crcp, s);
    if (sq && fm == 1 && e == hipSuccess) e = fork();
    if (e == hipSuccess)
        e = w8split ? bnf_launch_decode_w8(words, nbytes, nframes, sp, chn_lanes, fmt, out, out_bytes, info, perm,
                                            mode | BNF_MODE_STREDO, seg, s)
                    : bnf_launch_decode_w8(words, nbytes, nframes, sp, chn_lanes, fmt, out, out_bytes, info, perm, mode, nullptr, s);
    if (sq) {
        for (int i = 0; i < nside; i++) {
            const hipError_t ej = hipStreamWaitEvent(s, sq->join[i], 0);
            if (e == hipSuccess) e = ej;
        }
        lk.unlock();
    } else if (seg_only) {
        g_seg_launches.fetch_add(1, std::memory_order_relaxed);
        if (e == hipSuccess)
            e = bnf_launch_decode_seg(words, nbytes, nframes, sp, chn_lanes, fmt, out, out_bytes, info, perm, mode, seg, s);
    } else {
        if (e == hipSuccess) e = bnf_launch_decode_w16(words, nbytes, nframes, sp, chn_lanes, fmt, out, out_bytes, info, perm, mode, seg, s);
        if (e == hipSuccess) e = bnf_launch_decode_w32(words, nbytes, nframes, sp, chn_lanes, fmt, out, out_bytes, info, perm, mode, seg, s);
    }
    return e;
}

hipError_t bnf_launch_chain(const uint8_t *bytes, uint64_t nbytes, const uint64_t *cand, uint32_t ncand,
                            const bnf_frame_info *info, uint64_t first_off, bnf_stream_params sp, uint32_t *gap_crc,
                            int32_t *jump, uint32_t levels, uint32_t *mark, uint32_t *pos, uint64_t *bs, uint8_t *small,
                            uint64_t *d_offs, uint64_t *d_os, bnf_frame_info *d_info, uint32_t cap, uint32_t *nframes,
                            hipStream_t s) {
    int32_t *head = (int32_t *)small;
    uint32_t *chain_len = (uint32_t *)(small + 8);
    uint64_t *samples = (uint64_t *)(small + 16);
    hipError_t e = hipMemsetAsync(head, 0x7f, 4, s);
    if (e == hipSuccess) e = hipMemsetAsync(mark, 0, sizeof(uint32_t) * (size_t)ncand, s);
    if (e != hipSuccess) return e;
    const dim3 g256((ncand + 255) / 256);
    if (ncand) {
        hipLaunchKernelGGL(k_gap_crc, dim3((ncand + 3) / 4), dim3(256), 0, s, bytes, nbytes, cand, ncand, gap_crc);
        hipLaunchKernelGGL(k_chain_keys, dim3(1), dim3(1024), 0, s, gap_crc, ncand, info);
        hipLaunchKernelGGL(k_chain_succ, g256, dim3(256), 0, s, cand, ncand, gap_crc, first_off, jump, head);
        for (uint32_t k = 0; k + 1 < levels; k++)
            hipLaunchKernelGGL(k_chain_jump, g256, dim3(256), 0, s, jump + (size_t)k * ncand,
                               jump + (size_t)(k + 1) * ncand, ncand);
        hipLaunchKernelGGL(k_chain_mark, g256, dim3(256), 0, s, jump, mark, ncand, head, 1);
        for (int k = (int)levels - 1; k >= 0; k--)
            hipLaunchKernelGGL(k_chain_mark, g256, dim3(256), 0, s, jump + (size_t)k * ncand, mark, ncand, head, 0);
        e = hipMemcpyAsync(pos, mark, sizeof(uint32_t) * (size_t)ncand, hipMemcpyDeviceToDevice, s);
        if (e != hipSuccess) return e;
    }
    hipLaunchKernelGGL(k_scan_u32, dim3(1), dim3(1024), 0, s, pos, ncand, chain_len);
    hipLaunchKernelGGL(k_chain_compact, g256, dim3(256), 0, s, cand, ncand, info, mark, pos, bs, ncand);
    hipLaunchKernelGGL(k_scan_u64, dim3(1), dim3(1024), 0, s, bs, chain_len, ncand, samples);
    e = hipMemcpyAsync(nframes, chain_len, 4, hipMemcpyDeviceToDevice, s);
    if (e != hipSuccess) return e;
    if (ncand)
        hipLaunchKernelGGL(k_chain_emit, g256, dim3(256), 0, s, cand, ncand, info, mark, pos, bs, sp, d_offs, d_os,
                           d_info, cap, nframes);
    return hipGetLastError();
}

static void ms_scan_add(const uint32_t *c, const uint64_t *a, const uint32_t *n_ptr, uint32_t cap, uint32_t *csum,
                        uint64_t *asum, uint32_t *co, uint64_t *ao, hipStream_t s) {
    const uint32_t nb = cap / MS_SCAN + 1u;
    hipLaunchKernelGGL(k_ms_add_reduce, dim3(nb), dim3(MS_SCAN), 0, s, c, a, n_ptr, cap, csum, a ? asum : nullptr);
    hipLaunchKernelGGL(k_ms_add_sums, dim3(1), dim3(MS_SCAN), 0, s, csum, a ? asum : nullptr, nb);
    hipLaunchKernelGGL(k_ms_add_apply, dim3(nb), dim3(MS_SCAN), 0, s, c, a, n_ptr, cap, csum, asum, co, ao);
}

hipError_t bnf_launch_chain_streams(const uint8_t *bytes, uint64_t nbytes, const bnf_stream_desc *sd, uint32_t nstreams,
                                    bnf_stream_params sp, uint32_t cand_cap, bnf_ms_scratch w, uint64_t *d_offs,
                                    uint64_t *d_os, bnf_frame_info *d_info, uint32_t cap, uint32_t *d_sf, uint64_t *d_ss,
                                    uint32_t *d_status, hipStream_t s) {
    const uint32_t C = cand_cap, S = nstreams;
// ... 49 lines not shown
```

### birdnest/audio_amd/csrc/bnflac_launch.h

```cpp
#ifndef BNFLAC_LAUNCH_H
#define BNFLAC_LAUNCH_H

#include <hip/hip_runtime.h>
#include <stdint.h>

#include "bnflac_device.h"


#define BNF_ABLATE_NO_CRC16 0x1u
#define BNF_ABLATE_NO_STORE 0x2u
#define BNF_ABLATE_NO_RESTORE 0x4u
#define BNF_ABLATE_NO_RICE 0x8u
#define BNF_ABLATE_NO_WALK 0x10u
#define BNF_ABLATE_NO_WALK_REFILL 0x20u
#define BNF_ABLATE_NO_STFOLD 0x40u
#define BNF_ABLATE_STATS 0x100u
#define BNF_ABLATE_NO_ST 0x400u
#define BNF_ABLATE_NO_FUSED 0x800u
#define BNF_ABLATE_NO_WIDE24 0x2000u
#define BNF_ABLATE_NO_SW 0x10000u
#define BNF_ABLATE_SYS_MIXED 0x40000u
#define BNF_ABLATE_SYS_LAND_ONLY 0x80000u
#define BNF_ABLATE_NO_W8SPLIT 0x100000u
#define BNF_ABLATE_SYS_NO_RUN 0x200000u
#define BNF_ABLATE_SYS_NO_PACK_FAST 0x400000u
#define BNF_ABLATE_PARSE_BLKREFILL 0x800000u
#define BNF_ABLATE_SYS_REFILL_HALF 0x1000000u
#define BNF_ABLATE_HOT_WINDOW 0x10000000u
#define BNF_ABLATE_SW_NO_LINE 0x20000000u

#define BNF_MODE_WREDO 0x4000u
#define BNF_MODE_SW 0x8000u
#define BNF_MODE_LIST 0x20000u
#define BNF_MODE_NOST 0x40000u
#define BNF_MODE_STREDO 0x80000u
#define BNF_MODE_SEG 0x80000000u

#define BNF_MODE_K_PARSE 0u
#define BNF_ABLATE_K_PARSE (BNF_ABLATE_NO_WALK | BNF_ABLATE_NO_WALK_REFILL | BNF_ABLATE_PARSE_BLKREFILL)
#define BNF_MODE_K_DECODE (BNF_MODE_WREDO | BNF_MODE_SW | BNF_MODE_LIST | BNF_MODE_NOST | BNF_MODE_STREDO | BNF_MODE_SEG)
#define BNF_ABLATE_K_DECODE                                                                                      \
    (BNF_ABLATE_NO_CRC16 | BNF_ABLATE_NO_STORE | BNF_ABLATE_NO_RESTORE | BNF_ABLATE_NO_RICE | BNF_ABLATE_STATS | \
     BNF_ABLATE_NO_ST | BNF_ABLATE_NO_FUSED | BNF_ABLATE_NO_WIDE24)
#define BNF_MODE_K_DECODE_ST (BNF_MODE_WREDO | BNF_MODE_SW)
#define BNF_ABLATE_K_DECODE_ST                                                                                      \
    (BNF_ABLATE_NO_CRC16 | BNF_ABLATE_NO_STORE | BNF_ABLATE_NO_RESTORE | BNF_ABLATE_NO_RICE | BNF_ABLATE_NO_STFOLD | \
     BNF_ABLATE_STATS | BNF_ABLATE_NO_ST | BNF_ABLATE_HOT_WINDOW)
#define BNF_MODE_K_DECODE_SW BNF_MODE_WREDO
#define BNF_ABLATE_K_DECODE_SW                                                                                       \
    (BNF_ABLATE_NO_CRC16 | BNF_ABLATE_NO_STORE | BNF_ABLATE_NO_RESTORE | BNF_ABLATE_NO_RICE | BNF_ABLATE_HOT_WINDOW | \
     BNF_ABLATE_SW_NO_LINE)
#define BNF_MODE_K_DECODE_SYS 0u
#define BNF_ABLATE_K_DECODE_SYS                                                                                  \
    (BNF_ABLATE_NO_CRC16 | BNF_ABLATE_NO_STORE | BNF_ABLATE_NO_RESTORE | BNF_ABLATE_NO_RICE | BNF_ABLATE_STATS | \
     BNF_ABLATE_SYS_MIXED | BNF_ABLATE_SYS_LAND_ONLY | BNF_ABLATE_SYS_NO_RUN | BNF_ABLATE_SYS_NO_PACK_FAST |     \
     BNF_ABLATE_SYS_REFILL_HALF)
#define BNF_MODE_MASK (BNF_MODE_K_PARSE | BNF_MODE_K_DECODE | BNF_MODE_K_DECODE_ST | BNF_MODE_K_DECODE_SW | BNF_MODE_K_DECODE_SYS)

static_assert(!(BNF_ABLATE_K_PARSE & BNF_MODE_K_PARSE), "k_parse: an ablation bit is a mode bit");
static_assert(!(BNF_ABLATE_K_DECODE & BNF_MODE_K_DECODE), "k_decode<W>: an ablation bit is a mode bit");
static_assert(!(BNF_ABLATE_K_DECODE_ST & BNF_MODE_K_DECODE_ST), "k_decode_st: an ablation bit is a mode bit");
static_assert(!(BNF_ABLATE_K_DECODE_SW & BNF_MODE_K_DECODE_SW), "k_decode_sw: an ablation bit is a mode bit");
static_assert(!(BNF_ABLATE_K_DECODE_SYS & BNF_MODE_K_DECODE_SYS), "k_decode_sys: an ablation bit is a mode bit");
static_assert(!((BNF_ABLATE_NO_SW | BNF_ABLATE_NO_W8SPLIT) & BNF_MODE_MASK), "a host ablation bit is a mode bit");

typedef struct {
    hipError_t (*upload_tables)(const uint8_t *crc8, const uint16_t *crc16x8, const uint16_t *xpow);
    hipError_t (*stats)(uint64_t *out16, int reset);
} bnf_tu_ops;
extern bnf_tu_ops bnf_ops_decode_w8, bnf_ops_decode_w16, bnf_ops_decode_w32, bnf_ops_decode_st_fd, bnf_ops_decode_st_any,
    bnf_ops_decode_sw, bnf_ops_decode_sys;

extern "C" {
uint32_t bnf_ablate_flags(void);
void bnf_set_ablate(uint32_t v);

#define BNF_DECODE_ARGS                                                                                              \
    const uint32_t *words, uint64_t nbytes, uint32_t nframes, bnf_stream_params sp, uint32_t chn_lanes, int fmt,   \
        uint8_t *out, uint64_t out_bytes, bnf_frame_info *info
hipError_t bnf_launch_decode_w8(BNF_DECODE_ARGS, const uint32_t *perm, uint32_t mode, const uint32_t *seg, hipStream_t s);
hipError_t bnf_launch_decode_w16(BNF_DECODE_ARGS, const uint32_t *perm, uint32_t mode, const uint32_t *seg, hipStream_t s);
hipError_t bnf_launch_decode_w32(BNF_DECODE_ARGS, const uint32_t *perm, uint32_t mode, const uint32_t *seg, hipStream_t s);
hipError_t bnf_launch_decode_list(BNF_DECODE_ARGS, const uint32_t *list, uint32_t mode, hipStream_t s);
hipError_t bnf_launch_decode_seg(BNF_DECODE_ARGS, const uint32_t *perm, uint32_t mode, const uint32_t *seg, hipStream_t s);
hipError_t bnf_launch_decode_st_fd(BNF_DECODE_ARGS, const uint32_t *perm, uint32_t mode, const uint32_t *crcp, hipStream_t s);
hipError_t bnf_launch_decode_st_any(BNF_DECODE_ARGS, const uint32_t *perm, uint32_t mode, const uint32_t *crcp, hipStream_t s);
hipError_t bnf_launch_decode_sw(BNF_DECODE_ARGS, const uint32_t *perm, uint32_t mode, const uint32_t *crcp, hipStream_t s);
hipError_t bnf_launch_decode_sys(BNF_DECODE_ARGS, const uint32_t *perm, uint32_t *redo, uint32_t mode, hipStream_t s);

hipError_t bnf_upload_tables(const uint8_t *crc8, const uint16_t *crc16x8, const uint16_t *xpow);
hipError_t bnf_stats(uint64_t *out16, int reset);
hipError_t bnf_launch_sync_scan(const uint8_t *d, uint64_t n, uint32_t *d_block_counts, uint32_t *d_total,
                                uint64_t *d_out, uint32_t cap, hipStream_t s);
uint32_t bnf_scan_blocks(uint64_t n);
hipError_t bnf_launch_scan_u32(uint32_t *v, uint32_t n, uint32_t *total, hipStream_t s);
int bnf_crc_mode(void);
void bnf_set_crc_mode(int mode);
void bnf_set_decode_sys(int mode);
void bnf_set_parse_wave(int mode);
uint64_t bnf_decode_seg_launches(void);
hipError_t bnf_parse_wave_stats(uint64_t *out8, int reset);
hipError_t bnf_launch_parse(const uint32_t *words, uint64_t nbytes, const uint64_t *frame_offs, uint32_t nframes,
                            bnf_stream_params sp, const uint64_t *out_sample_in, uint64_t base_sample,
                            bnf_frame_info *info, uint32_t *order, uint32_t *crcp, bool *handed, hipStream_t s);
hipError_t bnf_launch_decode(const uint32_t *words, uint64_t nbytes, uint32_t nframes, bnf_stream_params sp,
                             uint32_t chn_lanes, int fmt, uint8_t *out, uint64_t out_bytes, bnf_frame_info *info,
                             uint32_t *order, const uint32_t *crcp, hipStream_t s);
hipError_t bnf_launch_fill_bad(const bnf_frame_info *info, uint32_t nframes, bnf_stream_params sp, int fmt,
                               uint8_t *out, uint64_t out_bytes, hipStream_t s);
hipError_t bnf_launch_chain(const uint8_t *bytes, uint64_t nbytes, const uint64_t *cand, uint32_t ncand,
                            const bnf_frame_info *info, uint64_t first_off, bnf_stream_params sp, uint32_t *gap_crc,
                            int32_t *jump, uint32_t levels, uint32_t *mark, uint32_t *pos, uint64_t *bs, uint8_t *small,
                            uint64_t *d_offs, uint64_t *d_os, bnf_frame_info *d_info, uint32_t cap, uint32_t *nframes,
                            hipStream_t s);
hipError_t bnf_launch_chain_streams(const uint8_t *bytes, uint64_t nbytes, const bnf_stream_desc *sd, uint32_t nstreams,
                                    bnf_stream_params sp, uint32_t cand_cap, bnf_ms_scratch w, uint64_t *d_offs,
                                    uint64_t *d_os, bnf_frame_info *d_info, uint32_t cap, uint32_t *d_sf, uint64_t *d_ss,
                                    uint32_t *d_status, hipStream_t s);

hipError_t bnf_launch_md5_streams(const uint8_t *pcm, uint64_t pcm_bytes, uint32_t unit, uint32_t src,
                                  const uint64_t *bounds, uint32_t nstreams, const uint8_t *expected, uint8_t *md5,
                                  uint32_t *verdict, uint32_t *status, hipStream_t s);

hipError_t bnf_launch_scan_streams(const uint8_t *bytes, uint64_t nbytes, bnf_stream_desc *sd, uint32_t nstreams,
                                   const bnf_stream_params *expect, bnf_stream_meta *meta, uint8_t *md5,
                                   uint32_t *status, hipStream_t s);
}

#endif
```

### birdnest/audio_amd/csrc/bnflac_runtime.cpp

```cpp
#include <hip/hip_runtime.h>

#include <algorithm>
#include <cstdio>
#include <cstdlib>
#include <cstring>
#include <mutex>
#include <string>
#include <sys/stat.h>
#include <vector>

#include "../../../include/bnflac.h"
#include "bnf_metadata.h"
#include "bnflac_device.h"
#include "bnflac_launch.h"
#include "bnflac_md5.h"

static_assert(sizeof(bnflac_frame_info) == sizeof(bnf_frame_info), "frame info layout");
static_assert(sizeof(bnf_frame_info) == 128, "frame info is 128 bytes");
static_assert(offsetof(FLAC__FrameHeader, number) == 24, "FrameHeader.FrameOrSampleNumber @24 (LibFLACSharp.cs:232)");
static_assert(offsetof(FLAC__FrameHeader, crc) == 32, "FrameHeader.Crc @32 (LibFLACSharp.cs:233)");
static_assert(offsetof(FLAC__StreamMetadata, data) == 16, "StreamMetadata.data @16 (LibFLACSharp.cs:299)");
static_assert(offsetof(FLAC__StreamMetadata, data.stream_info.sample_rate) == 32, "sample_rate @32");
static_assert(offsetof(FLAC__StreamMetadata, data.stream_info.total_samples) == 48, "total_samples @48");

// ... 65 lines not shown
}

extern "C" BNFLAC_API void bnflac_debug_set_ablate(uint32_t flags) { bnf_set_ablate(flags); }
extern "C" BNFLAC_API int bnflac_debug_crc_fold_check(void) {
#ifdef BNFLAC_CRC_FOLD_CHECK
    return 1;
#else
    return 0;
#endif
}
extern "C" BNFLAC_API void bnflac_debug_set_parse_wave(int mode) { bnf_set_parse_wave(mode); }
extern "C" BNFLAC_API void bnflac_debug_set_decode_sys(int mode) { bnf_set_decode_sys(mode); }
extern "C" BNFLAC_API void bnflac_debug_set_crc_mode(int mode) { bnf_set_crc_mode(mode); }
extern "C" BNFLAC_API uint64_t bnflac_debug_decode_seg_launches(void) { return bnf_decode_seg_launches(); }
extern "C" BNFLAC_API int bnflac_debug_parse_wave_stats(uint64_t *out8, int reset) {
    return bnf_parse_wave_stats(out8, reset) == hipSuccess ? 0 : -1;
}
extern "C" BNFLAC_API int bnflac_debug_stats(uint64_t *out16, int reset) {
    return bnf_stats(out16, reset) == hipSuccess ? 0 : fail("bnflac_debug_stats failed");
}

extern "C" BNFLAC_API int bnflac_device_count(void) {
    int n = 0;
    if (hipGetDeviceCount(&n) != hipSuccess) return 0;
    return n;
}

struct CtxBuf {
    void *p = nullptr;
    size_t cap = 0;
    bool grow(size_t n) {
        if (n <= cap) return true;
        if (p) (void)hipFree(p);
        p = nullptr;
        cap = 0;
        if (hipMalloc(&p, n) != hipSuccess) return false;
        cap = n;
        return true;
    }
    void release() {
        if (p) (void)hipFree(p);
        p = nullptr;
        cap = 0;
    }
};

struct bnflac_ctx {
    int device;
    uint32_t *d_block_counts = nullptr;
    uint32_t block_cap = 0;
    CtxBuf cand, info, gap, jump, mark, pos, bs, small;
    CtxBuf ms;
    CtxBuf order, porder;
    CtxBuf crcp;
    const void *crcp_bytes = nullptr, *crcp_info = nullptr;
    uint64_t crcp_nbytes = 0;
    uint32_t crcp_n = 0;
};

static bool crc_prefix_on() { return bnf_crc_mode() != 0; }

extern "C" BNFLAC_API int bnflac_ctx_create(int device, bnflac_ctx **out) {
    *out = nullptr;
    if (ensure_device(device)) return -1;
    bnflac_ctx *c = new bnflac_ctx();
    c->device = device;
    *out = c;
    return 0;
}

extern "C" BNFLAC_API int bnflac_debug_crc_handoff(bnflac_ctx *ctx, uint32_t *out, uint32_t nframes) {
    if (!ctx || !out) return fail("bnflac_debug_crc_handoff: null argument");
    if (!ctx->crcp_bytes || ctx->crcp_n != nframes) return fail("bnflac_debug_crc_handoff: no hand-off for this batch");
    DevGuard dg(ctx->device);
    if (hipDeviceSynchronize() != hipSuccess || hipMemcpy(out, ctx->crcp.p, 32ull * nframes, hipMemcpyDeviceToHost) != hipSuccess)
        return fail("bnflac_debug_crc_handoff: HIP error");
    return 0;
}

extern "C" BNFLAC_API void bnflac_ctx_destroy(bnflac_ctx *ctx) {
    if (!ctx) return;
    if (ctx->d_block_counts) (void)hipFree(ctx->d_block_counts);
    for (CtxBuf *b : {&ctx->cand, &ctx->info, &ctx->gap, &ctx->jump, &ctx->mark, &ctx->pos, &ctx->bs, &ctx->small,
                      &ctx->ms, &ctx->order, &ctx->porder, &ctx->crcp})
        b->release();
    delete ctx;
}

static uint32_t lanes_for(uint32_t channels) {
    uint32_t l = 1;
    while (l < channels) l <<= 1;
    return l > 8 ? 8 : l;
}

extern "C" BNFLAC_API uint32_t bnflac_out_stride(int fmt, const bnflac_stream_params *sp) {
    switch (fmt) {
    case BNFLAC_OUT_PLANAR32:
    case BNFLAC_OUT_INTERLEAVED32: return 4u * sp->channels;
    case BNFLAC_OUT_FLACDECODER: return sp->channels == 2 ? 4u : 2u;
    default: return sp->channels * (sp->bps == 24 ? 3u : 2u);
    }
}

extern "C" BNFLAC_API int bnflac_md5_interleaved32(const int32_t *pcm, uint64_t nsamples, uint32_t channels,
                                                   uint32_t bps, uint8_t out_md5[16]) {
    if ((!pcm && nsamples) || !out_md5) return fail("bnflac_md5_interleaved32: null pointer");
    if (channels < 1 || channels > FLAC__MAX_CHANNELS || bps < 4 || bps > 32)
        return fail("bnflac_md5_interleaved32: bad channels/bps");
    Md5 m;
    md5_init(m);
    const int32_t *chan[FLAC__MAX_CHANNELS];
    for (uint32_t c = 0; c < channels; c++) chan[c] = pcm + c;
    md5_accumulate(m, chan, channels, nsamples, channels, (bps + 7) / 8);
    md5_final(m, out_md5);
    return 0;
}

extern "C" BNFLAC_API uint32_t bnflac_md5_layout(int fmt, const bnflac_stream_params *sp) {
    if (!sp || sp->channels < 1 || sp->channels > FLAC__MAX_CHANNELS || sp->bps < 4 || sp->bps > 32) return 0;
    const uint32_t B = (sp->bps + 7) / 8;
    switch (fmt) {
    case BNFLAC_OUT_INTERLEAVED32: return B;
    case BNFLAC_OUT_FLACDECODER: return sp->bps == 16 && sp->channels <= 2 ? B : 0;
    case BNFLAC_OUT_FILEREADER: return sp->bps == 16 || sp->bps == 24 ? B : 0;
    default: return 0;
    }
}

extern "C" BNFLAC_API int bnflac_md5_streams(bnflac_ctx *ctx, const uint8_t *d_pcm, uint64_t pcm_bytes, int fmt,
                                             const bnflac_stream_params *sp, const uint64_t *d_stream_samples,
                                             uint32_t nstreams, const uint8_t *d_expected, uint8_t *d_md5,
                                             uint32_t *d_verdict, uint32_t *d_status, void *hs) {
    if (!ctx || !sp) return fail("bnflac_md5_streams: null argument");
    DevGuard dg(ctx->device);
    if (!d_status || (nstreams && (!d_stream_samples || !d_md5))) return fail("bnflac_md5_streams: null output");
    if (pcm_bytes && !d_pcm) return fail("bnflac_md5_streams: null d_pcm");
    if (((uintptr_t)d_pcm) & 15u) return fail("bnflac_md5_streams: d_pcm must be 16-byte aligned");
    if (nstreams >= (1u << 30)) return fail("bnflac_md5_streams: too many streams");
    const uint32_t B = bnflac_md5_layout(fmt, sp);
    if (!B) return fail("bnflac_md5_streams: layout does not carry the MD5 bytes");
    const bool int32_src = fmt == BNFLAC_OUT_INTERLEAVED32;
    hipError_t e = bnf_launch_md5_streams(d_pcm, pcm_bytes, bnflac_out_stride(fmt, sp), int32_src ? B : 0, d_stream_samples,
                                          nstreams, d_expected, d_md5, d_verdict, d_status, (hipStream_t)hs);
    return e == hipSuccess ? 0 : fail(std::string("bnflac_md5_streams: ") + hipGetErrorString(e));
}

extern "C" BNFLAC_API int bnflac_index_frames(bnflac_ctx *ctx, const uint8_t *d_bytes, uint64_t nbytes,
                                              uint64_t *d_offsets, uint32_t cap, uint32_t *d_count, void *hs) {
    if (!ctx) return fail("bnflac_index_frames: null ctx");
    DevGuard dg(ctx->device);
    if (((uintptr_t)d_bytes) & 3u) return fail("bnflac_index_frames: d_bytes must be 4-byte aligned");
    const uint32_t nb = bnf_scan_blocks(nbytes);
    if (nb > ctx->block_cap) {
        if (ctx->d_block_counts) (void)hipFree(ctx->d_block_counts);
        ctx->d_block_counts = nullptr;
        if (hipMalloc(&ctx->d_block_counts, sizeof(uint32_t) * (size_t)std::max(nb, 1u)) != hipSuccess)
            return fail("bnflac_index_frames: out of device memory");
        ctx->block_cap = nb;
    }
    hipError_t e = bnf_launch_sync_scan(d_bytes, nbytes, ctx->d_block_counts, d_count, d_offsets, cap, (hipStream_t)hs);
    return e == hipSuccess ? 0 : fail(std::string("bnflac_index_frames: ") + hipGetErrorString(e));
}

static int check_args(bnflac_ctx *ctx, const uint8_t *d_bytes, uint64_t nbytes, const bnflac_stream_params *sp,
                      const char *who) {
    if (!ctx || !sp) return fail(std::string(who) + ": null argument");
    if (((uintptr_t)d_bytes) & 15u) return fail(std::string(who) + ": d_bytes must be 16-byte aligned");
    if (sp->channels < 1 || sp->channels > 8) return fail(std::string(who) + ": channels must be 1..8");
    if (nbytes >= (1ull << 34)) return fail(std::string(who) + ": buffer larger than 16 GiB");
    return 0;
}

extern "C" BNFLAC_API int bnflac_parse_frames(bnflac_ctx *ctx, const uint8_t *d_bytes, uint64_t nbytes,
                                              const uint64_t *d_frame_offsets, uint32_t nframes,
                                              const bnflac_stream_params *sp, const uint64_t *d_out_sample,
                                              uint64_t base_sample, bnflac_frame_info *d_info, void *hs) {
    if (check_args(ctx, d_bytes, nbytes, sp, "bnflac_parse_frames")) return -1;
    DevGuard dg(ctx->device);
    bnf_stream_params p;
    memcpy(&p, sp, sizeof p);
    if (!ctx->porder.grow(sizeof(uint32_t) * (256u + (size_t)nframes)))
        return fail("bnflac_parse_frames: out of device memory (parse-order scratch)");
    ctx->crcp_bytes = ctx->crcp_info = nullptr;
    const bool pre = crc_prefix_on() && ctx->crcp.grow(32u * std::max<size_t>(nframes, 1u));
    bool handed = false;
    hipError_t e = bnf_launch_parse((const uint32_t *)d_bytes, nbytes, d_frame_offsets,
                                    nframes, p, d_out_sample, base_sample, (bnf_frame_info *)d_info,
                                    (uint32_t *)ctx->porder.p, pre ? (uint32_t *)ctx->crcp.p : nullptr, &handed,
                                    (hipStream_t)hs);
    if (e == hipSuccess && pre && handed) {
        ctx->crcp_bytes = d_bytes;
        ctx->crcp_info = d_info;
        ctx->crcp_nbytes = nbytes;
        ctx->crcp_n = nframes;
    }
    return e == hipSuccess ? 0 : fail(std::string("k_parse: ") + hipGetErrorString(e));
}

extern "C" BNFLAC_API int bnflac_decode_parsed(bnflac_ctx *ctx, const uint8_t *d_bytes, uint64_t nbytes, uint32_t nframes,
                                               const bnflac_stream_params *sp, int out_format, uint8_t *d_out,
                                               uint64_t out_bytes, bnflac_frame_info *d_info, void *hs) {
    if (check_args(ctx, d_bytes, nbytes, sp, "bnflac_decode_parsed")) return -1;
    DevGuard dg(ctx->device);
    if (out_format < 0 || out_format > 3) return fail("bnflac_decode_parsed: bad out_format");
    bnf_stream_params p;
    memcpy(&p, sp, sizeof p);
    if (!ctx->order.grow(sizeof(uint32_t) * (260u + 2u * (size_t)nframes)))
        return fail("bnflac_decode_parsed: out of device memory (decode-order scratch)");
    const bool pre = ctx->crcp_bytes == d_bytes && ctx->crcp_info == d_info && ctx->crcp_nbytes == nbytes &&
                     ctx->crcp_n == nframes;
    ctx->crcp_bytes = ctx->crcp_info = nullptr;
    hipError_t e = bnf_launch_decode((const uint32_t *)d_bytes, nbytes, nframes, p,
                                     lanes_for(sp->channels), out_format, d_out, out_bytes, (bnf_frame_info *)d_info,
                                     (uint32_t *)ctx->order.p, pre ? (const uint32_t *)ctx->crcp.p : nullptr,
                                     (hipStream_t)hs);
    if (e == hipSuccess)
        e = bnf_launch_fill_bad((const bnf_frame_info *)d_info, nframes, p, out_format, d_out, out_bytes, (hipStream_t)hs);
    return e == hipSuccess ? 0 : fail(std::string("k_decode: ") + hipGetErrorString(e));
}

extern "C" BNFLAC_API int bnflac_decode_frames(bnflac_ctx *ctx, const uint8_t *d_bytes, uint64_t nbytes,
                                               const uint64_t *d_frame_offsets, uint32_t nframes,
                                               const bnflac_stream_params *sp, const uint64_t *d_out_sample,
                                               uint64_t base_sample, int out_format, uint8_t *d_out, uint64_t out_bytes,
                                               bnflac_frame_info *d_info, void *hs) {
    if (out_format < 0 || out_format > 3) return fail("bnflac_decode_frames: bad out_format");
    int rc = bnflac_parse_frames(ctx, d_bytes, nbytes, d_frame_offsets, nframes, sp, d_out_sample, base_sample, d_info, hs);
    if (rc) return rc;
    return bnflac_decode_parsed(ctx, d_bytes, nbytes, nframes, sp, out_format, d_out, out_bytes, d_info, hs);
}

extern "C" BNFLAC_API int bnflac_index_stream(bnflac_ctx *ctx, const uint8_t *d_bytes, uint64_t nbytes,
                                              uint64_t first_offset, const bnflac_stream_params *sp,
                                              uint64_t *d_frame_offsets, uint64_t *d_out_sample,
                                              bnflac_frame_info *d_info, uint32_t cap, uint32_t *d_nframes, void *hs) {
    if (check_args(ctx, d_bytes, nbytes, sp, "bnflac_index_stream")) return -1;
    DevGuard dg(ctx->device);
    if (!d_frame_offsets || !d_nframes) return fail("bnflac_index_stream: null output");
    hipStream_t s = (hipStream_t)hs;
    uint32_t ccap = (uint32_t)std::min<uint64_t>(nbytes / 1024 + 4096, 1u << 30), ncand = 0;
    for (int attempt = 0;; attempt++) {
        if (!ctx->cand.grow(sizeof(uint64_t) * ccap) || !ctx->small.grow(64))
            return fail("bnflac_index_stream: out of device memory");
        if (bnflac_index_frames(ctx, d_bytes, nbytes, (uint64_t *)ctx->cand.p, ccap, (uint32_t *)ctx->small.p, hs))
            return -1;
        if (hipMemcpyAsync(&ncand, ctx->small.p, 4, hipMemcpyDeviceToHost, s) != hipSuccess ||
            hipStreamSynchronize(s) != hipSuccess)
            return fail("bnflac_index_stream: HIP error reading the candidate count");
        if (ncand <= ccap) break;
        if (attempt) return fail("bnflac_index_stream: candidate count changed");
        ccap = ncand;
    }
    if (ncand >= (1u << 30)) return fail("bnflac_index_stream: too many sync candidates");
    uint32_t levels = 1;
    while ((1ull << levels) <= ncand) levels++;
    const size_t n = std::max<uint32_t>(ncand, 1u);
    if (!ctx->info.grow(sizeof(bnf_frame_info) * n) || !ctx->gap.grow(4 * n) || !ctx->jump.grow(4 * n * levels) ||
        !ctx->mark.grow(4 * n) || !ctx->pos.grow(4 * n) || !ctx->bs.grow(8 * n))
        return fail("bnflac_index_stream: out of device memory");
    bnf_stream_params p;
    memcpy(&p, sp, sizeof p);
    ctx->crcp_bytes = ctx->crcp_info = nullptr;
    hipError_t e = bnf_launch_parse((const uint32_t *)d_bytes, nbytes, (const uint64_t *)ctx->cand.p, ncand, p, nullptr,
                                    0, (bnf_frame_info *)ctx->info.p, nullptr, nullptr, nullptr, s);
    if (e == hipSuccess)
        e = bnf_launch_chain(d_bytes, nbytes, (const uint64_t *)ctx->cand.p, ncand, (const bnf_frame_info *)ctx->info.p,
                             first_offset, p, (uint32_t *)ctx->gap.p, (int32_t *)ctx->jump.p, levels,
                             (uint32_t *)ctx->mark.p, (uint32_t *)ctx->pos.p, (uint64_t *)ctx->bs.p,
                             (uint8_t *)ctx->small.p + 16, d_frame_offsets, d_out_sample, (bnf_frame_info *)d_info, cap,
                             d_nframes, s);
    return e == hipSuccess ? 0 : fail(std::string("bnflac_index_stream: ") + hipGetErrorString(e));
}

static_assert(sizeof(bnflac_stream_desc) == sizeof(bnf_stream_desc), "stream descriptor layout");

extern "C" BNFLAC_API int bnflac_index_streams(bnflac_ctx *ctx, const uint8_t *d_bytes, uint64_t nbytes,
                                               const bnflac_stream_desc *d_streams, uint32_t nstreams,
                                               const bnflac_stream_params *sp, uint32_t cand_cap,
                                               uint64_t *d_frame_offsets, uint64_t *d_out_sample,
                                               bnflac_frame_info *d_info, uint32_t cap, uint32_t *d_stream_frames,
                                               uint64_t *d_stream_samples, uint32_t *d_status, void *hs) {
    if (check_args(ctx, d_bytes, nbytes, sp, "bnflac_index_streams")) return -1;
    DevGuard dg(ctx->device);
    if (!d_stream_frames || !d_status || (cap && !d_frame_offsets)) return fail("bnflac_index_streams: null output");
    if (nstreams && !d_streams) return fail("bnflac_index_streams: null descriptor table");
    if (nstreams >= (1u << 30)) return fail("bnflac_index_streams: too many streams");
    hipStream_t s = (hipStream_t)hs;
    ctx->crcp_bytes = ctx->crcp_info = nullptr;
    if (!nstreams || !nbytes) {
        hipError_t e = hipMemsetAsync(d_status, 0, 4 * sizeof(uint32_t), s);
        if (e == hipSuccess) e = hipMemsetAsync(d_stream_frames, 0, sizeof(uint32_t) * ((size_t)nstreams + 1), s);
        if (e == hipSuccess && d_stream_samples)
            e = hipMemsetAsync(d_stream_samples, 0, sizeof(uint64_t) * ((size_t)nstreams + 1), s);
        return e == hipSuccess ? 0 : fail(std::string("bnflac_index_streams: ") + hipGetErrorString(e));
    }
    const uint64_t C64 = cand_cap ? cand_cap : nbytes / 1024 + 4096;
    if (C64 >= (1u << 30)) return fail("bnflac_index_streams: cand_cap too large");
    const size_t C = (size_t)C64, S = nstreams, B = bnf_scan_blocks(nbytes);
    const size_t nsum = std::max(B, std::max(C, S)) / 1024 + 2;
    size_t off = 0;
    auto take = [&off](size_t bytes) {
        const size_t at = off;
        off += (bytes + 15) & ~(size_t)15;
        return at;
    };
    const size_t o_ctl = take(16), o_blk = take(4 * (B + 1)), o_csum = take(4 * nsum), o_asum = take(8 * nsum),
                 o_cand = take(8 * C), o_info = take(sizeof(bnf_frame_info) * C), o_seg = take(4 * C), o_key = take(4 * C),
                 o_mark = take(4 * C), o_pos = take(4 * (C + 1)), o_bs = take(8 * C), o_smp = take(8 * (C + 1)),
                 o_jump = take(8 * C), o_clo = take(4 * S), o_chi = take(4 * S), o_kept = take(4 * S), o_head = take(4 * S),
                 o_ssum = take(8 * S), o_ss = take(8 * (S + 1));
    if (!ctx->ms.grow(off)) return fail("bnflac_index_streams: out of device memory");
    uint8_t *m = (uint8_t *)ctx->ms.p;
    bnf_ms_scratch w;
    w.ctl = (uint32_t *)(m + o_ctl);
    w.blk = (uint32_t *)(m + o_blk);
    w.csum = (uint32_t *)(m + o_csum);
    w.asum = (uint64_t *)(m + o_asum);
    w.cand = (uint64_t *)(m + o_cand);
    w.info = (bnf_frame_info *)(m + o_info);
    w.seg = (int32_t *)(m + o_seg);
    w.key = (uint32_t *)(m + o_key);
    w.mark = (uint32_t *)(m + o_mark);
    w.pos = (uint32_t *)(m + o_pos);
    w.bs = (uint64_t *)(m + o_bs);
    w.smp = (uint64_t *)(m + o_smp);
    w.jump = (int32_t *)(m + o_jump);
    w.clo = (uint32_t *)(m + o_clo);
    w.chi = (uint32_t *)(m + o_chi);
    w.kept = (uint32_t *)(m + o_kept);
    w.head = (int32_t *)(m + o_head);
    w.ssum = (uint64_t *)(m + o_ssum);
    w.ss = (uint64_t *)(m + o_ss);
    bnf_stream_params p;
    memcpy(&p, sp, sizeof p);
    hipError_t e = bnf_launch_chain_streams(d_bytes, nbytes, (const bnf_stream_desc *)d_streams, nstreams, p, (uint32_t)C, w,
                                            d_frame_offsets, d_out_sample, (bnf_frame_info *)d_info, cap, d_stream_frames,
                                            d_stream_samples, d_status, s);
    return e == hipSuccess ? 0 : fail(std::string("bnflac_index_streams: ") + hipGetErrorString(e));
}

static_assert(sizeof(bnflac_stream_meta) == sizeof(bnf_stream_meta) && sizeof(bnf_stream_meta) == 64, "stream meta layout");
// ... 401 lines not shown
    bnflac_ctx_destroy(d->ctx);
    d->ctx = nullptr;
    d->gpu_ready = false;
}

bool decode_window(Dec *d, uint64_t base) {
    if (!gpu_init(d)) {
        d->state = FLAC__STREAM_DECODER_MEMORY_ALLOCATION_ERROR;
        return false;
    }
    DevGuard g(d->device);
    const uint64_t n = bend(d) - base;
    const size_t padded = (size_t)((n + 3) & ~3ull) + 16;
    if (!d->d_bytes.grow(padded)) goto oom;
    if (hipMemsetAsync((uint8_t *)d->d_bytes.p + (n & ~3ull), 0, padded - (n & ~3ull), d->stream) != hipSuccess) goto hip_fail;
    if (hipMemcpyAsync(d->d_bytes.p, d->buf.data() + (base - d->buf_base), n, hipMemcpyHostToDevice, d->stream) != hipSuccess) goto hip_fail;
    {
        uint32_t cap = (uint32_t)std::min<uint64_t>(n / 2 + 16, 1u << 30);
        cap = std::min<uint32_t>(cap, (uint32_t)(n / 64 + 4096));
        for (int attempt = 0; attempt < 2; attempt++) {
            if (!d->d_cand.grow(sizeof(uint64_t) * cap) || !d->d_count.grow(16)) goto oom;
            if (bnflac_index_frames(d->ctx, (const uint8_t *)d->d_bytes.p, n, (uint64_t *)d->d_cand.p, cap,
                                    (uint32_t *)d->d_count.p, d->stream) != 0)
                goto hip_fail;
            uint32_t cnt = 0;
            if (hipMemcpyAsync(&cnt, d->d_count.p, 4, hipMemcpyDeviceToHost, d->stream) != hipSuccess) goto hip_fail;
            if (hipStreamSynchronize(d->stream) != hipSuccess) goto hip_fail;
            if (cnt <= cap) {
                cap = cnt;
                break;
            }
            cap = cnt;
        }
        const uint32_t ncand = cap;
        d->cand.resize(ncand);
        d->info.resize(ncand);
        if (ncand) {
            if (hipMemcpyAsync(d->cand.data(), d->d_cand.p, sizeof(uint64_t) * ncand, hipMemcpyDeviceToHost, d->stream) != hipSuccess)
                goto hip_fail;
            bnf_stream_params sp;
            memset(&sp, 0, sizeof sp);
            if (d->has_stream_info) {
                const FLAC__StreamMetadata_StreamInfo &si = d->stream_info.data.stream_info;
                sp.has_stream_info = 1;
                sp.min_blocksize = si.min_blocksize;
                sp.max_blocksize = si.max_blocksize;
                sp.sample_rate = si.sample_rate;
                sp.channels = si.channels;
                sp.bps = si.bits_per_sample;
                sp.total_samples = si.total_samples;
            }
            if (!d->d_info.grow(sizeof(bnf_frame_info) * ncand)) goto oom;
            if (bnf_launch_parse((const uint32_t *)d->d_bytes.p, n, (const uint64_t *)d->d_cand.p, ncand, sp,
                                 nullptr, 0, (bnf_frame_info *)d->d_info.p, nullptr, nullptr, nullptr, d->stream) != hipSuccess)
                goto hip_fail;
            if (hipMemcpyAsync(d->info.data(), d->d_info.p, sizeof(bnf_frame_info) * ncand, hipMemcpyDeviceToHost, d->stream) != hipSuccess)
                goto hip_fail;
            if (hipStreamSynchronize(d->stream) != hipSuccess) goto hip_fail;
            uint64_t tot = 0;
            uint32_t pcm_ch = 1;
            for (auto &fi : d->info) {
                fi.out_sample = tot;
                if (fi.status == BNF_ST_OK) {
                    tot += fi.blocksize;
                    pcm_ch = std::max(pcm_ch, std::min<uint32_t>(fi.channels, 8u));
                }
            }
            d->pcm_ch = pcm_ch;
            if (!d->d_pcm.grow(sizeof(int32_t) * (size_t)std::max<uint64_t>(tot, 1) * pcm_ch)) goto oom;
            if (hipMemcpyAsync(d->d_info.p, d->info.data(), sizeof(bnf_frame_info) * ncand, hipMemcpyHostToDevice, d->stream) != hipSuccess)
                goto hip_fail;
            bnf_stream_params spd = sp;
            spd.channels = pcm_ch;
            if (bnf_launch_decode((const uint32_t *)d->d_bytes.p, n, ncand, spd, lanes_for(pcm_ch), BNF_OUT_PLANAR32,
                                  (uint8_t *)d->d_pcm.p, (uint64_t)std::max<uint64_t>(tot, 1) * pcm_ch * 4,
                                  (bnf_frame_info *)d->d_info.p, nullptr, nullptr, d->stream) != hipSuccess)
                goto hip_fail;
            d->pcm.resize((size_t)tot * pcm_ch);
            if (tot && hipMemcpyAsync(d->pcm.data(), d->d_pcm.p, sizeof(int32_t) * (size_t)tot * pcm_ch, hipMemcpyDeviceToHost, d->stream) != hipSuccess)
                goto hip_fail;
            if (hipMemcpyAsync(d->info.data(), d->d_info.p, sizeof(bnf_frame_info) * ncand, hipMemcpyDeviceToHost, d->stream) != hipSuccess)
                goto hip_fail;
            if (hipStreamSynchronize(d->stream) != hipSuccess) goto hip_fail;
        }
    }
    d->win_base = base;
    d->win_end = bend(d);
    d->win_valid = true;
    d->read_ahead_cur = std::min(d->read_ahead, d->read_ahead_cur * 2);
    return true;
oom:
    fail("bnflac: out of device memory");
    d->state = FLAC__STREAM_DECODER_MEMORY_ALLOCATION_ERROR;
    return false;
hip_fail:
    fail(std::string("bnflac: HIP error in decode window: ") + hipGetErrorString(hipGetLastError()));
    d->state = FLAC__STREAM_DECODER_MEMORY_ALLOCATION_ERROR;
    return false;
}

const bnf_frame_info *lookup(Dec *d, uint64_t p) {
    if (!d->win_valid || p < d->win_base || p >= d->win_end) return nullptr;
    uint64_t rel = p - d->win_base;
    auto it = std::lower_bound(d->cand.begin(), d->cand.end(), rel);
    if (it == d->cand.end() || *it != rel) return nullptr;
    return &d->info[(size_t)(it - d->cand.begin())];
}

void allocate_output(Dec *d, unsigned size, unsigned ch) {
    if (size <= d->output_capacity && ch <= d->output_channels) return;
    for (unsigned i = 0; i < FLAC__MAX_CHANNELS; i++) d->output[i].clear();
    for (unsigned i = 0; i < ch; i++) d->output[i].assign(2u * (size ? size : 1), 0);
    d->output_capacity = size;
    d->output_channels = ch;
}

bool read_frame(Dec *d, bool *got) {
    *got = false;
    const uint64_t p = d->pos - 2;
    const bnf_frame_info *fi = nullptr;
    for (int tries = 0;; tries++) {
        fi = lookup(d, p);
        if (fi && fi->status != BNF_ST_TRUNC) break;
        if (tries > 200) {
            fail("bnflac: frame window did not converge");
            d->state = FLAC__STREAM_DECODER_ABORTED;
            return false;
        }
        if (d->client_done) {
// ... 521 lines not shown
```

### birdnest/audio_amd/libflac.py

```python
from __future__ import annotations

import ctypes
import enum
from typing import Optional

import numpy as np

from ._lib import lib_path


class StreamDecoderState(enum.IntEnum):
    SearchForMetadata = 0
    ReadMetadata = 1
    SearchForFrameSync = 2
    ReadFrame = 3
    EndOfStream = 4
    OggError = 5
    SeekError = 6
    Aborted = 7
    MemoryAllocationError = 8
    Uninitialized = 9


class StreamDecoderReadStatus(enum.IntEnum):
# ... 42 lines not shown
    Picture = 6
    Undefined = 7


class FrameHeader(ctypes.Structure):
    _fields_ = [("BlockSize", ctypes.c_int32), ("SampleRate", ctypes.c_int32), ("Channels", ctypes.c_int32),
                ("ChannelAssignment", ctypes.c_int32), ("BitsPerSample", ctypes.c_int32),
                ("NumberType", ctypes.c_int32), ("FrameOrSampleNumber", ctypes.c_int64), ("Crc", ctypes.c_uint8)]


class FLACMetaData(ctypes.Structure):
    _pack_ = 4
    _fields_ = [("MetaDataType", ctypes.c_int32), ("IsLast", ctypes.c_int32), ("Length", ctypes.c_int32),
                ("Data", ctypes.c_uint8 * 100)]


class FLACStreamInfo(ctypes.Structure):
    _pack_ = 1
    _fields_ = [("_hdr", ctypes.c_int32), ("MinBlocksize", ctypes.c_int32), ("MaxBlocksize", ctypes.c_int32),
                ("min_framesize", ctypes.c_int32), ("max_framesize", ctypes.c_int32), ("SampleRate", ctypes.c_int32),
                ("Channels", ctypes.c_int32), ("BitsPerSample", ctypes.c_int32), ("TotalSamplesHi", ctypes.c_int32),
                ("TotalSamplesLo", ctypes.c_int32)]


_DEC = ctypes.c_void_p
DecoderReadCallback = ctypes.CFUNCTYPE(ctypes.c_int, _DEC, ctypes.POINTER(ctypes.c_uint8),
                                       ctypes.POINTER(ctypes.c_size_t), ctypes.c_void_p)
DecoderSeekCallback = ctypes.CFUNCTYPE(ctypes.c_int, _DEC, ctypes.c_uint64, ctypes.c_void_p)
DecoderTellCallback = ctypes.CFUNCTYPE(ctypes.c_int, _DEC, ctypes.POINTER(ctypes.c_uint64), ctypes.c_void_p)
DecoderLengthCallback = ctypes.CFUNCTYPE(ctypes.c_int, _DEC, ctypes.POINTER(ctypes.c_uint64), ctypes.c_void_p)
DecoderEofCallback = ctypes.CFUNCTYPE(ctypes.c_int, _DEC, ctypes.c_void_p)
DecoderWriteCallbackWithStatus = ctypes.CFUNCTYPE(ctypes.c_int, _DEC, ctypes.c_void_p,
                                                  ctypes.POINTER(ctypes.POINTER(ctypes.c_int32)), ctypes.c_void_p)
Decoder_WriteCallback = DecoderWriteCallbackWithStatus
Decoder_MetadataCallback = ctypes.CFUNCTYPE(None, _DEC, ctypes.c_void_p, ctypes.c_void_p)
Decoder_ErrorCallback = ctypes.CFUNCTYPE(None, _DEC, ctypes.c_int, ctypes.c_void_p)

DECODER_SYMBOLS = [
    "FLAC__stream_decoder_new", "FLAC__stream_decoder_finish", "FLAC__stream_decoder_delete",
    "FLAC__stream_decoder_init_file", "FLAC__stream_decoder_process_single",
    "FLAC__stream_decoder_process_until_end_of_metadata", "FLAC__stream_decoder_process_until_end_of_stream",
    "FLAC__stream_decoder_seek_absolute", "FLAC__stream_decoder_get_decode_position",
    "FLAC__stream_decoder_get_total_samples", "FLAC__stream_decoder_get_channels",
    "FLAC__stream_decoder_get_bits_per_sample", "FLAC__stream_decoder_get_sample_rate",
    "FLAC__stream_decoder_get_state", "FLAC__stream_decoder_reset", "FLAC__stream_decoder_init_stream",
    "FLAC__stream_decoder_set_md5_checking", "FLAC__stream_decoder_get_md5_checking",
]
BATCH_SYMBOLS = ["bnflac_ctx_create", "bnflac_ctx_destroy", "bnflac_last_error", "bnflac_device_count",
                 "bnflac_index_frames", "bnflac_decode_frames", "bnflac_parse_frames", "bnflac_decode_parsed",
                 "bnflac_out_stride", "bnflac_debug_set_ablate", "bnflac_debug_stats", "bnflac_debug_set_parse_wave", "bnflac_debug_parse_wave_stats",
                 "bnflac_debug_set_decode_sys", "bnflac_debug_decode_seg_launches", "bnflac_md5_interleaved32", "bnflac_index_stream",
                 "bnflac_index_streams", "bnflac_md5_layout", "bnflac_md5_streams",
                 "bnflac_scan_streams", "bnflac_scan_stream_host",
                 "bnflac_debug_set_crc_mode", "bnflac_debug_crc_handoff"]
READER_SYMBOLS = ["bnflac_reader_open", "bnflac_reader_params", "bnflac_reader_read", "bnflac_reader_close",
                  "bnflac_reader_last_error", "bnflac_reader_seek", "bnflac_reader_read_filereader",
                  "bnflac_reader_pool_release"]

_LIB = None


def load() -> ctypes.CDLL:
    global _LIB
    if _LIB is not None:
        return _LIB
    L = ctypes.CDLL(lib_path("libbnflac.so"))
    b, u, i, p = ctypes.c_int, ctypes.c_uint, ctypes.c_int, ctypes.c_void_p
    L.FLAC__stream_decoder_new.restype = p
    for n in ("finish", "delete", "process_single", "process_until_end_of_metadata",
              "process_until_end_of_stream", "reset"):
        f = getattr(L, "FLAC__stream_decoder_" + n)
        f.restype, f.argtypes = b, [p]
    L.FLAC__stream_decoder_init_file.restype = i
    L.FLAC__stream_decoder_init_file.argtypes = [p, ctypes.c_char_p, Decoder_WriteCallback,
                                                 Decoder_MetadataCallback, Decoder_ErrorCallback, p]
    L.FLAC__stream_decoder_init_stream.restype = i
    L.FLAC__stream_decoder_init_stream.argtypes = [p, DecoderReadCallback, DecoderSeekCallback, DecoderTellCallback,
                                                   DecoderLengthCallback, DecoderEofCallback,
                                                   DecoderWriteCallbackWithStatus, Decoder_MetadataCallback,
                                                   Decoder_ErrorCallback, p]
    L.FLAC__stream_decoder_seek_absolute.restype, L.FLAC__stream_decoder_seek_absolute.argtypes = b, [p, ctypes.c_uint64]
    L.FLAC__stream_decoder_get_decode_position.restype = b
    L.FLAC__stream_decoder_get_decode_position.argtypes = [p, ctypes.POINTER(ctypes.c_uint64)]
    L.FLAC__stream_decoder_get_total_samples.restype = ctypes.c_uint64
    L.FLAC__stream_decoder_get_total_samples.argtypes = [p]
    for n in ("get_channels", "get_bits_per_sample", "get_sample_rate", "get_state"):
        f = getattr(L, "FLAC__stream_decoder_" + n)
        f.restype, f.argtypes = u, [p]
    L.bnflac_last_error.restype = ctypes.c_char_p
    L.bnflac_ctx_create.restype, L.bnflac_ctx_create.argtypes = i, [i, ctypes.POINTER(p)]
    L.bnflac_ctx_destroy.argtypes = [p]
    L.bnflac_index_frames.restype = i
    L.bnflac_index_frames.argtypes = [p, p, ctypes.c_uint64, p, ctypes.c_uint32, p, p]
    L.bnflac_decode_frames.restype = i
    L.bnflac_decode_frames.argtypes = [p, p, ctypes.c_uint64, p, ctypes.c_uint32, p, p, ctypes.c_uint64, i, p,
                                       ctypes.c_uint64, p, p]
    L.bnflac_parse_frames.restype = i
    L.bnflac_parse_frames.argtypes = [p, p, ctypes.c_uint64, p, ctypes.c_uint32, p, p, ctypes.c_uint64, p, p]
    L.bnflac_decode_parsed.restype = i
    L.bnflac_decode_parsed.argtypes = [p, p, ctypes.c_uint64, ctypes.c_uint32, p, i, p, ctypes.c_uint64, p, p]
    L.bnflac_debug_set_ablate.argtypes = [ctypes.c_uint32]
    L.bnflac_debug_set_parse_wave.argtypes = [ctypes.c_int]
    L.bnflac_debug_set_decode_sys.argtypes = [ctypes.c_int]
    L.bnflac_debug_set_crc_mode.argtypes = [ctypes.c_int]
    L.bnflac_debug_crc_handoff.restype = i
    L.bnflac_debug_crc_handoff.argtypes = [p, p, ctypes.c_uint32]
    L.bnflac_debug_decode_seg_launches.restype, L.bnflac_debug_decode_seg_launches.argtypes = ctypes.c_uint64, []
    L.bnflac_debug_parse_wave_stats.argtypes = [ctypes.POINTER(ctypes.c_uint64), ctypes.c_int]
    L.bnflac_debug_stats.argtypes = [ctypes.POINTER(ctypes.c_uint64), ctypes.c_int]
    L.bnflac_debug_stats.restype = ctypes.c_int
    L.bnflac_out_stride.restype = ctypes.c_uint32
    L.bnflac_out_stride.argtypes = [i, p]
    L.FLAC__stream_decoder_set_md5_checking.restype = b
    L.FLAC__stream_decoder_set_md5_checking.argtypes = [p, b]
    L.FLAC__stream_decoder_get_md5_checking.restype = b
    L.FLAC__stream_decoder_get_md5_checking.argtypes = [p]
    L.bnflac_index_stream.restype = i
    L.bnflac_index_stream.argtypes = [p, p, ctypes.c_uint64, ctypes.c_uint64, p, p, p, p, ctypes.c_uint32, p, p]
    L.bnflac_index_streams.restype = i
    L.bnflac_index_streams.argtypes = [p, p, ctypes.c_uint64, p, ctypes.c_uint32, p, ctypes.c_uint32, p, p, p,
                                       ctypes.c_uint32, p, p, p, p]
    L.bnflac_reader_open.restype = i
    L.bnflac_reader_open.argtypes = [i, p, ctypes.c_uint64, i, ctypes.c_uint32, ctypes.POINTER(p)]
    L.bnflac_reader_params.restype = i
    L.bnflac_reader_params.argtypes = [p, p, ctypes.POINTER(ctypes.c_uint64), ctypes.POINTER(ctypes.c_uint32)]
    L.bnflac_reader_read.restype = ctypes.c_int64
    L.bnflac_reader_read.argtypes = [p, p, ctypes.c_uint64]
    L.bnflac_reader_close.argtypes = [p]
    L.bnflac_reader_pool_release.argtypes = [ctypes.c_int]
    L.bnflac_reader_pool_release.restype = ctypes.c_int
    L.bnflac_reader_read_filereader.restype = ctypes.c_int64
    L.bnflac_reader_read_filereader.argtypes = [p, p, ctypes.c_uint64, ctypes.c_uint64, ctypes.c_uint64]
    L.bnflac_reader_seek.restype = i
    L.bnflac_reader_seek.argtypes = [p, ctypes.c_uint64]
    L.bnflac_reader_last_error.restype = ctypes.c_char_p
    L.bnflac_md5_interleaved32.restype = i
    L.bnflac_md5_interleaved32.argtypes = [p, ctypes.c_uint64, ctypes.c_uint32, ctypes.c_uint32, p]
    L.bnflac_md5_layout.restype, L.bnflac_md5_layout.argtypes = ctypes.c_uint32, [i, p]
    L.bnflac_md5_streams.restype = i
    L.bnflac_md5_streams.argtypes = [p, p, ctypes.c_uint64, i, p, p, ctypes.c_uint32, p, p, p, p, p]
    L.bnflac_scan_streams.restype = i
    L.bnflac_scan_streams.argtypes = [p, p, ctypes.c_uint64, p, ctypes.c_uint32, p, p, p, p, p]
    L.bnflac_scan_stream_host.restype = i
    L.bnflac_scan_stream_host.argtypes = [p, ctypes.c_uint64, p, p]
    _LIB = L
    return L


class LibFLAC:

    @staticmethod
    def _l():
        return load()

    @staticmethod
    def FLAC__stream_decoder_new():
        return LibFLAC._l().FLAC__stream_decoder_new()

    @staticmethod
# ... 299 lines not shown
            ctypes.c_void_p(d_info.data_ptr()), self._stream(stream))
        if rc != 0:
            raise RuntimeError(self.L.bnflac_last_error().decode())


    def parse_frames(self, d_bytes, nbytes: int, d_offsets, nframes: int, sp: StreamParams, d_info,
                     d_out_sample=None, base_sample: int = 0, stream=None):
        rc = self.L.bnflac_parse_frames(
            self.ctx, ctypes.c_void_p(d_bytes.data_ptr()), nbytes, ctypes.c_void_p(d_offsets.data_ptr()), nframes,
            ctypes.byref(sp), ctypes.c_void_p(d_out_sample.data_ptr()) if d_out_sample is not None else None,
            base_sample, ctypes.c_void_p(d_info.data_ptr()), self._stream(stream))
        if rc != 0:
            raise RuntimeError(self.L.bnflac_last_error().decode())

    def decode_parsed(self, d_bytes, nbytes: int, nframes: int, sp: StreamParams, fmt: int, d_out, d_info,
                      stream=None):
        rc = self.L.bnflac_decode_parsed(self.ctx, ctypes.c_void_p(d_bytes.data_ptr()), nbytes, nframes,
                                         ctypes.byref(sp), fmt, ctypes.c_void_p(d_out.data_ptr()),
                                         d_out.numel() * d_out.element_size(), ctypes.c_void_p(d_info.data_ptr()),
                                         self._stream(stream))
        if rc != 0:
            raise RuntimeError(self.L.bnflac_last_error().decode())

    def md5_streams(self, d_pcm, fmt: int, sp: StreamParams, d_stream_samples, nstreams: int, d_expected=None,
                    stream=None, pcm_bytes=None):
        import torch
        dev = d_pcm.device
        s = stream if stream is not None else torch.cuda.current_stream()
        nbytes = d_pcm.numel() * d_pcm.element_size()
        if d_stream_samples.numel() < nstreams + 1 or d_stream_samples.element_size() != 8:
            raise ValueError("d_stream_samples must hold nstreams + 1 64-bit bounds")
        if d_expected is not None and d_expected.numel() * d_expected.element_size() < 16 * nstreams:
            raise ValueError("d_expected must hold 16 bytes per stream")
        with torch.cuda.stream(s):
            d_md5 = torch.zeros((nstreams, 16), dtype=torch.uint8, device=dev)
            d_verdict = torch.zeros(nstreams, dtype=torch.int32, device=dev)
            d_status = torch.zeros(4, dtype=torch.int32, device=dev)
        rc = self.L.bnflac_md5_streams(self.ctx, ctypes.c_void_p(d_pcm.data_ptr()),
                                       nbytes if pcm_bytes is None else min(pcm_bytes, nbytes), fmt, ctypes.byref(sp),
                                       ctypes.c_void_p(d_stream_samples.data_ptr()), nstreams,
                                       ctypes.c_void_p(d_expected.data_ptr()) if d_expected is not None else None,
                                       ctypes.c_void_p(d_md5.data_ptr()), ctypes.c_void_p(d_verdict.data_ptr()),
                                       ctypes.c_void_p(d_status.data_ptr()), self._stream(s))
        if rc != 0:
            raise RuntimeError(self.L.bnflac_last_error().decode())
        return d_md5, d_verdict, d_status

    def crc_handoff(self, nframes: int) -> np.ndarray:
        a = np.zeros(8 * nframes, np.uint32)
        if self.L.bnflac_debug_crc_handoff(self.ctx, a.ctypes.data_as(ctypes.c_void_p), nframes) != 0:
            raise RuntimeError(self.L.bnflac_last_error().decode())
        return a.reshape(nframes, 8)


class Reader:

    def __init__(self, data: bytes, out_format: int = OUT_FLACDECODER, window_frames: int = 0, device: int = 0):
        self.L = load()
        self._data = np.frombuffer(bytes(data), dtype=np.uint8)
        h = ctypes.c_void_p()
        rc = self.L.bnflac_reader_open(device, self._data.ctypes.data, self._data.size, out_format, window_frames,
                                       ctypes.byref(h))
        if rc != 0:
            raise RuntimeError(self.L.bnflac_reader_last_error().decode())
        self.h = h
        sp = StreamParams()
        tb, nf = ctypes.c_uint64(), ctypes.c_uint32()
        self.L.bnflac_reader_params(self.h, ctypes.byref(sp), ctypes.byref(tb), ctypes.byref(nf))
        self.stream_params, self.total_bytes, self.nframes = sp, int(tb.value), int(nf.value)

    def Read(self, buffer: bytearray, offset: int, count: int) -> int:
        if offset < 0 or count < 0 or offset + count > len(buffer):
            raise ValueError("offset/count outside the buffer")
        view = (ctypes.c_uint8 * len(buffer)).from_buffer(buffer)
        n = self.L.bnflac_reader_read(self.h, ctypes.addressof(view) + offset, count)
        if n < 0:
            raise RuntimeError(self.L.bnflac_reader_last_error().decode())
        return int(n)

    def ReadFileReader(self, buffer: bytearray, offset: int, count: int) -> int:
        if offset < 0 or count < 0:
            raise ValueError("negative offset/count")
        view = (ctypes.c_uint8 * len(buffer)).from_buffer(buffer) if len(buffer) else None
        n = self.L.bnflac_reader_read_filereader(self.h, ctypes.addressof(view) if view is not None else None, offset,
                                                 count, len(buffer))
        if n < 0:
            raise RuntimeError(self.L.bnflac_reader_last_error().decode())
        return int(n)

    def filereader_read_all(self, buf_len: int, num_bytes: int = None):
        num_bytes = buf_len if num_bytes is None else num_bytes
        out = bytearray()
        buf = bytearray(buf_len)
        try:
            while True:
                n = self.ReadFileReader(buf, 0, num_bytes)
                if n == 0:
                    return 0, bytes(out), ""
                out += buf[:n]
        except RuntimeError as e:
            return 1, bytes(out), str(e)

    def Seek(self, sample: int):
        if self.L.bnflac_reader_seek(self.h, sample) != 0:
            raise RuntimeError(self.L.bnflac_reader_last_error().decode())

# ... 24 lines not shown
```

### include/bnflac.h

```cpp
#ifndef BNFLAC_H
#define BNFLAC_H

#include "FLAC_compat.h"

#ifdef __cplusplus
extern "C" {
#endif

#if defined(__GNUC__)
#define BNFLAC_API __attribute__((visibility("default")))
#else
#define BNFLAC_API
#endif


BNFLAC_API FLAC__StreamDecoder *FLAC__stream_decoder_new(void);
BNFLAC_API FLAC__bool FLAC__stream_decoder_finish(FLAC__StreamDecoder *decoder);
BNFLAC_API FLAC__bool FLAC__stream_decoder_delete(FLAC__StreamDecoder *decoder);
BNFLAC_API int FLAC__stream_decoder_init_file(FLAC__StreamDecoder *decoder, const char *filename,
                                              FLAC__StreamDecoderWriteCallback write_callback,
                                              FLAC__StreamDecoderMetadataCallback metadata_callback,
                                              FLAC__StreamDecoderErrorCallback error_callback,
                                              void *client_data);
BNFLAC_API FLAC__bool FLAC__stream_decoder_process_single(FLAC__StreamDecoder *decoder);
// ... 72 lines not shown
    uint64_t total_samples;
} bnflac_stream_desc;

enum {
    BNFLAC_SCAN_OK = 0,
    BNFLAC_SCAN_NO_MARKER = 1,
    BNFLAC_SCAN_TRUNCATED = 2,
    BNFLAC_SCAN_NO_STREAMINFO = 3,
    BNFLAC_SCAN_TOO_MANY_BLOCKS = 4,
    BNFLAC_SCAN_BAD_RANGE = 5
};
enum { BNFLAC_SCAN_MAX_BLOCKS = 1024 };

typedef struct {
    uint32_t status;
    uint32_t flags;
    uint32_t nblocks;
    uint32_t id3_bytes;
    bnflac_stream_params sp;
    uint32_t min_framesize, max_framesize;
    uint64_t first_offset;
} bnflac_stream_meta;

BNFLAC_API int bnflac_scan_streams(bnflac_ctx *ctx, const uint8_t *d_bytes, uint64_t nbytes,
                                   bnflac_stream_desc *d_streams, uint32_t nstreams,
                                   const bnflac_stream_params *expect, bnflac_stream_meta *d_meta,
                                   uint8_t *d_md5_expected, uint32_t *d_status, void *hip_stream);

BNFLAC_API int bnflac_scan_stream_host(const uint8_t *bytes, uint64_t nbytes, bnflac_stream_meta *meta,
                                       uint8_t md5[16]);

BNFLAC_API int bnflac_index_streams(bnflac_ctx *ctx, const uint8_t *d_bytes, uint64_t nbytes,
                                    const bnflac_stream_desc *d_streams, uint32_t nstreams,
                                    const bnflac_stream_params *sp, uint32_t cand_cap, uint64_t *d_frame_offsets,
                                    uint64_t *d_out_sample, bnflac_frame_info *d_info, uint32_t cap,
                                    uint32_t *d_stream_frames, uint64_t *d_stream_samples, uint32_t *d_status,
                                    void *hip_stream);

BNFLAC_API int bnflac_decode_frames(bnflac_ctx *ctx, const uint8_t *d_bytes, uint64_t nbytes,
                                    const uint64_t *d_frame_offsets, uint32_t nframes,
                                    const bnflac_stream_params *sp, const uint64_t *d_out_sample,
                                    uint64_t base_sample, int out_format, uint8_t *d_out, uint64_t out_bytes,
                                    bnflac_frame_info *d_info, void *hip_stream);

BNFLAC_API int bnflac_parse_frames(bnflac_ctx *ctx, const uint8_t *d_bytes, uint64_t nbytes,
                                   const uint64_t *d_frame_offsets, uint32_t nframes,
                                   const bnflac_stream_params *sp, const uint64_t *d_out_sample,
                                   uint64_t base_sample, bnflac_frame_info *d_info, void *hip_stream);
BNFLAC_API int bnflac_decode_parsed(bnflac_ctx *ctx, const uint8_t *d_bytes, uint64_t nbytes, uint32_t nframes,
                                    const bnflac_stream_params *sp, int out_format, uint8_t *d_out,
                                    uint64_t out_bytes, bnflac_frame_info *d_info, void *hip_stream);

BNFLAC_API void bnflac_debug_set_ablate(uint32_t flags);
BNFLAC_API int bnflac_debug_crc_fold_check(void);
BNFLAC_API void bnflac_debug_set_parse_wave(int mode);
BNFLAC_API void bnflac_debug_set_decode_sys(int mode);
BNFLAC_API void bnflac_debug_set_crc_mode(int mode);
BNFLAC_API int bnflac_debug_crc_handoff(bnflac_ctx *ctx, uint32_t *out, uint32_t nframes);
BNFLAC_API uint64_t bnflac_debug_decode_seg_launches(void);
BNFLAC_API int bnflac_debug_parse_wave_stats(uint64_t *out8, int reset);
BNFLAC_API int bnflac_debug_stats(uint64_t *out16, int reset);

BNFLAC_API uint32_t bnflac_out_stride(int out_format, const bnflac_stream_params *sp);

BNFLAC_API int bnflac_md5_interleaved32(const int32_t *pcm, uint64_t nsamples, uint32_t channels, uint32_t bps,
                                        uint8_t out_md5[16]);

BNFLAC_API uint32_t bnflac_md5_layout(int out_format, const bnflac_stream_params *sp);

BNFLAC_API int bnflac_md5_streams(bnflac_ctx *ctx, const uint8_t *d_pcm, uint64_t pcm_bytes, int out_format,
                                  const bnflac_stream_params *sp, const uint64_t *d_stream_samples,
                                  uint32_t nstreams, const uint8_t *d_expected, uint8_t *d_md5,
                                  uint32_t *d_verdict, uint32_t *d_status, void *hip_stream);


typedef struct bnflac_reader bnflac_reader;
BNFLAC_API int bnflac_reader_open(int device, const uint8_t *bytes, uint64_t nbytes, int out_format,
                                  uint32_t window_frames, bnflac_reader **out);
BNFLAC_API int bnflac_reader_params(const bnflac_reader *reader, bnflac_stream_params *sp, uint64_t *total_bytes,
                                    uint32_t *nframes);
BNFLAC_API int64_t bnflac_reader_read(bnflac_reader *reader, uint8_t *buf, uint64_t count);
BNFLAC_API int bnflac_reader_seek(bnflac_reader *reader, uint64_t sample);
BNFLAC_API int64_t bnflac_reader_read_filereader(bnflac_reader *reader, uint8_t *buffer, uint64_t offset,
                                                 uint64_t num_bytes, uint64_t buffer_length);
BNFLAC_API void bnflac_reader_close(bnflac_reader *reader);
BNFLAC_API int bnflac_reader_pool_release(int device);
BNFLAC_API const char *bnflac_reader_last_error(void);

#ifdef __cplusplus
}
#endif

#endif
```

Baseline: 773,300 MSamples/s.

## Build decode-order histogram in parse kernel and early-exit idle fallback kernels

The parse kernel now accumulates the decode-order key histogram and bad-frame count with wave-aggregated atomics, so the decode stage can reuse it instead of running a separate histogram pass. The stereo decode kernels count redo frames into a device summary. The generic k_decode fallback and k_fill_bad kernels read that summary and return immediately when no frames need them, and the permutation is bypassed when every frame lands in one bucket. This trims launch and scan work for the common all-stereo-16-bit case, at the cost of extra atomics in parse and more state tracked on the host context.

```diff
diff --git a/birdnest/audio_amd/csrc/bnflac_kernels.hip b/birdnest/audio_amd/csrc/bnflac_kernels.hip
--- a/birdnest/audio_amd/csrc/bnflac_kernels.hip
+++ b/birdnest/audio_amd/csrc/bnflac_kernels.hip
@@ -693,11 +693,18 @@
 
 #define PARSE_RD 8
 static_assert(PARSE_RD == 8, "pk_ra and the walk's pair steps (slot masks 0x3F3 / 0x1C0C, slot bits 10-12) assume an 8-slot ring");
+DEV uint32_t order_bucket(uint32_t work) { return 63u - min(work >> 8, 63u); }
+DEV uint32_t order_key0(uint32_t st, uint32_t fl, uint32_t bs) {
+    const uint32_t c = st != BNF_ST_OK ? 1u : (fl & BNF_FL_W32) ? 3u : (fl & BNF_FL_W16) ? 2u : (fl & BNF_FL_ST) ? 0u : 1u;
+    return c * 64u + order_bucket(bs ? bs - 1u : 0u);
+}
+#define PARSE_KEY_BAD 0x100u
+
 template <int CPM>
 DEV void parse_frame(const uint32_t *__restrict__ words, uint64_t nbytes, const uint64_t *__restrict__ frame_offs,
                      uint32_t nframes, const bnf_stream_params &sp, const uint64_t *__restrict__ out_sample_in,
                      uint64_t base_sample, bnf_frame_info *__restrict__ info, uint32_t ablate, lds_u32 *ring,
-                     uint32_t f, uint32_t *__restrict__ crcp) {
+                     uint32_t f, uint32_t *__restrict__ crcp, uint32_t *__restrict__ phist) {
     if (f >= nframes) return;
     bnf_frame_info fi;
     fi.status = BNF_ST_OK;
@@ -793,6 +800,20 @@
 #pragma unroll
     for (int c = 0; c < 8; c++) fi.sub_start[c] = ss[c];
     info[f] = fi;
+    if (phist) {
+        const uint32_t key = order_key0(st, fi.flags, fi.blocksize) | ((st == BNF_ST_ERROR || st == BNF_ST_TRUNC) ? PARSE_KEY_BAD : 0u);
+        uint64_t m = __ballot(1);
+        while (m) {
+            const uint32_t l = (uint32_t)__builtin_ctzll(m);
+            const uint64_t same = __ballot(key == (uint32_t)__shfl(key, l));
+            if ((threadIdx.x & 63u) == l) {
+                const uint32_t n = (uint32_t)__builtin_popcountll(same);
+                atomicAdd(&phist[key & (BNF_ORDER_NB - 1u)], n);
+                if (key & PARSE_KEY_BAD) atomicAdd(&phist[BNF_ORDER_NB + BNF_SUM_NBAD], n);
+            }
+            m &= ~same;
+        }
+    }
     if (CPM && crcp) {
         u32x4 o = u32x4{0u, 0u, 0u, 0u}, o2 = u32x4{0u, 0u, 0u, 0u};
         const uint32_t l1 = (uint32_t)(br_pos(b) >> 9);
@@ -895,11 +916,12 @@
                                               const uint64_t *__restrict__ frame_offs, uint32_t nframes,
                                               bnf_stream_params sp, const uint64_t *__restrict__ out_sample_in,
                                               uint64_t base_sample, bnf_frame_info *__restrict__ info, uint32_t ablate,
-                                              const uint32_t *__restrict__ perm, uint32_t *__restrict__ crcp) {
+                                              const uint32_t *__restrict__ perm, uint32_t *__restrict__ crcp,
+                                              uint32_t *__restrict__ phist) {
     __shared__ LDS_DMA_ALIGN uint32_t ring[PARSE_RD * RING_LANE_DW];
     const uint32_t slot = blockIdx.x * 64u + threadIdx.x;
     parse_frame<CPM>(words, nbytes, frame_offs, nframes, sp, out_sample_in, base_sample, info, ablate, (lds_u32 *)ring,
-                (perm && slot < nframes) ? perm[slot] : slot, crcp);
+                     (perm && slot < nframes) ? perm[slot] : slot, crcp, phist);
 }
 
 __global__ void __launch_bounds__(64) k_parse_wave(const uint32_t *__restrict__ words, uint64_t nbytes,
@@ -996,7 +1018,8 @@
 
 __global__ void __launch_bounds__(64) k_fill_bad(const bnf_frame_info *__restrict__ info, uint32_t nframes,
                                                  bnf_stream_params sp, int fmt, uint8_t *__restrict__ out,
-                                                 uint64_t out_bytes) {
+                                                 uint64_t out_bytes, const uint32_t *__restrict__ sum) {
+    if (sum && (sum[BNF_SUM_NBAD] | sum[BNF_SUM_NREDO] | sum[BNF_SUM_NLANE]) == 0u) return;
     const uint32_t f = blockIdx.x * 64u + threadIdx.x;
     bool bad = false;
     uint64_t start = 0, n = 0;
@@ -1640,9 +1663,16 @@
                                                       int fmt, uint8_t *__restrict__ out, uint64_t out_bytes,
                                                       bnf_frame_info *__restrict__ info,
                                                       const uint32_t *__restrict__ perm, uint32_t ablate,
-                                                      const uint32_t *__restrict__ seg) {
+                                                      const uint32_t *__restrict__ seg,
+                                                      const uint32_t *__restrict__ sum) {
     __shared__ LDS_DMA_ALIGN uint32_t ring[RD * RING_LANE_DW];
     __shared__ int32_t lds[CHK * RP];
+    if (sum) {
+        if (MAXW == 8 && !(ablate & (BNF_ABLATE_NO_ST | BNF_MODE_WREDO | BNF_MODE_LIST | BNF_MODE_NOST)) &&
+            sum[BNF_SUM_NREDO] == 0u && ((ablate & BNF_MODE_STREDO) || sum[BNF_SUM_NW8] == 0u))
+            return;
+        if (sum[BNF_SUM_ONE]) perm = nullptr;
+    }
     if (seg) {
         const uint32_t fpb = DEC_LANES >> __builtin_ctz(chn_lanes);
         const uint32_t c = MAXW == 32 ? 3u : MAXW == 16 ? 2u : (ablate & BNF_MODE_NOST) ? 1u : 0u;
@@ -1677,9 +1707,11 @@
                                                           int fmt, uint8_t *__restrict__ out, uint64_t out_bytes,
                                                           bnf_frame_info *__restrict__ info,
                                                           const uint32_t *__restrict__ perm, uint32_t ablate,
-                                                          const uint32_t *__restrict__ seg) {
+                                                          const uint32_t *__restrict__ seg,
+                                                          const uint32_t *__restrict__ sum) {
     __shared__ LDS_DMA_ALIGN uint32_t ring[RD * RING_LANE_DW];
     __shared__ int32_t lds[CHK * RP];
+    if (sum && sum[BNF_SUM_ONE]) perm = nullptr;
     const uint32_t fpb = DEC_LANES >> __builtin_ctz(chn_lanes);
     const uint32_t lo = __builtin_amdgcn_readfirstlane(seg[2u * 64u - 1u]) / fpb;
     const uint32_t end = (__builtin_amdgcn_readfirstlane(seg[3u * 64u + 63u]) + fpb - 1u) / fpb;
@@ -2065,7 +2097,7 @@
     const uint32_t i = blockIdx.x * 64u + threadIdx.x, n = ms_n(ctl);
     if (blockIdx.x * 64u >= n) return;
     const bool mine = i < n && seg[i] >= 0;
-    parse_frame<0>(words, nbytes, cand, n, sp, nullptr, 0, info, 0u, (lds_u32 *)ring, mine ? i : ~0u, nullptr);
+    parse_frame<0>(words, nbytes, cand, n, sp, nullptr, 0, info, 0u, (lds_u32 *)ring, mine ? i : ~0u, nullptr, nullptr);
 }
 
 __global__ void __launch_bounds__(256) k_ms_gap_crc(const uint8_t *__restrict__ bytes, uint64_t nbytes,
@@ -2837,14 +2869,15 @@
                                                      uint8_t *__restrict__ out, uint64_t out_bytes,
                                                      bnf_frame_info *__restrict__ info,
                                                      const uint32_t *__restrict__ perm, uint32_t ablate,
-                                                     const uint32_t *__restrict__ crcp) {
+                                                     const uint32_t *__restrict__ crcp, uint32_t *sum) {
     constexpr bool STG = (FMT == BNF_OUT_FLACDECODER || FMT == BNF_OUT_FILEREADER);
     constexpr uint32_t ST_SPG = (FMT == BNF_OUT_INTERLEAVED32 || FMT == BNF_OUT_PLANAR32) ? 2u : 1u;
     __shared__ LDS_DMA_ALIGN uint32_t ring[2 * ST_RD * RING_LANE_DW + 1024];
     static_assert((ST_RD * RING_LANE_DW * 4) % 1024 == 0, "channel 1's ring base must stay 1 KiB aligned (LDS-DMA)");
     const uint32_t lane = threadIdx.x;
     const uint32_t slot = blockIdx.x * 64u + lane;
-    const uint32_t f = (perm && slot < nframes) ? perm[slot] : slot;
+    const bool ident = !perm || (sum && sum[BNF_SUM_ONE]);
+    const uint32_t f = (!ident && slot < nframes) ? perm[slot] : slot;
     const uint64_t limit = nbytes * 8u;
     bnf_frame_info fi;
     const bool have = f < nframes;
@@ -3080,6 +3113,10 @@
     } else if (mine) {
         info[f].flags = fl_flags | BNF_FL_REDO;
     }
+    if (sum) {
+        const uint64_t hb = __ballot(mine && !ok);
+        if (hb && lane == 0) atomicAdd(&sum[BNF_SUM_NREDO], (uint32_t)__builtin_popcountll(hb));
+    }
     if (tmon && lane == 0) {
         const uint64_t t_end = tnow(tmon);
         atomicAdd(&g_stats[8], (unsigned long long)(t_loop - t_start));
@@ -3373,12 +3410,14 @@
                                                      uint8_t *__restrict__ out, uint64_t out_bytes,
                                                      bnf_frame_info *__restrict__ info,
                                                      const uint32_t *__restrict__ perm, uint32_t ablate,
-                                                     const uint32_t *__restrict__ crcp) {
+                                                     const uint32_t *__restrict__ crcp,
+                                                     const uint32_t *__restrict__ sum) {
     constexpr uint32_t SPG = sw_stores8<FMT>();
     __shared__ LDS_DMA_ALIGN uint32_t ring[2 * ST_RD * RING_LANE_DW + 1024];
     const uint32_t lane = threadIdx.x;
     const uint32_t slot = blockIdx.x * 64u + lane;
-    const uint32_t f = (perm && slot < nframes) ? perm[slot] : slot;
+    const bool ident = !perm || (sum && sum[BNF_SUM_ONE]);
+    const uint32_t f = (!ident && slot < nframes) ? perm[slot] : slot;
     const uint64_t limit = nbytes * 8u;
     bnf_frame_info fi;
     const bool have = f < nframes;
@@ -3589,12 +3628,12 @@
 extern "C" {
 hipError_t TU_FN(bnf_launch_decode)(const uint32_t *words, uint64_t nbytes, uint32_t nframes, bnf_stream_params sp,
                                     uint32_t chn_lanes, int fmt, uint8_t *out, uint64_t out_bytes, bnf_frame_info *info,
-                                    const uint32_t *perm, uint32_t mode, const uint32_t *seg, hipStream_t s) {
+                                    const uint32_t *perm, uint32_t mode, const uint32_t *seg, const uint32_t *sum, hipStream_t s) {
     const uint32_t fpb = DEC_LANES / chn_lanes;
     const uint32_t nb = (nframes + fpb - 1) / fpb;
     if (!perm || (DEC_W == 8 && !(mode & (BNF_MODE_NOST | BNF_MODE_STREDO)))) seg = nullptr;
     hipLaunchKernelGGL((k_decode<DEC_W, 32, DEC_RD>), dim3(nb), dim3(DEC_LANES), 0, s, words, nbytes, nframes, sp, chn_lanes,
-                       fmt, out, out_bytes, info, perm, (bnf_ablate_flags() & BNF_ABLATE_K_DECODE) | (mode & BNF_MODE_K_DECODE), seg);
+                       fmt, out, out_bytes, info, perm, (bnf_ablate_flags() & BNF_ABLATE_K_DECODE) | (mode & BNF_MODE_K_DECODE), seg, sum);
     return hipGetLastError();
 }
 #if BNF_DEC_W == 32
@@ -3609,11 +3648,11 @@
 }
 hipError_t bnf_launch_decode_seg(const uint32_t *words, uint64_t nbytes, uint32_t nframes, bnf_stream_params sp,
                                      uint32_t chn_lanes, int fmt, uint8_t *out, uint64_t out_bytes, bnf_frame_info *info,
-                                     const uint32_t *perm, uint32_t mode, const uint32_t *seg, hipStream_t s) {
+                                     const uint32_t *perm, uint32_t mode, const uint32_t *seg, const uint32_t *sum, hipStream_t s) {
     const uint32_t fpb = DEC_LANES / chn_lanes;
     const uint32_t nb = std::min<uint32_t>((nframes + fpb - 1) / fpb, 512u);
     hipLaunchKernelGGL((k_decode_seg<DEC_W, 32, DEC_RD>), dim3(std::max(nb, 1u)), dim3(DEC_LANES), 0, s, words, nbytes,
-                       nframes, sp, chn_lanes, fmt, out, out_bytes, info, perm, (bnf_ablate_flags() & BNF_ABLATE_K_DECODE) | (mode & BNF_MODE_K_DECODE) | BNF_MODE_SEG, seg);
+                       nframes, sp, chn_lanes, fmt, out, out_bytes, info, perm, (bnf_ablate_flags() & BNF_ABLATE_K_DECODE) | (mode & BNF_MODE_K_DECODE) | BNF_MODE_SEG, seg, sum);
     return hipGetLastError();
 }
 #endif
@@ -3630,23 +3669,23 @@
 extern "C" {
 hipError_t TU_FN(bnf_launch_decode)(const uint32_t *words, uint64_t nbytes, uint32_t nframes, bnf_stream_params sp,
                                     uint32_t chn_lanes, int fmt, uint8_t *out, uint64_t out_bytes, bnf_frame_info *info,
-                                    const uint32_t *perm, uint32_t mode, const uint32_t *crcp, hipStream_t s) {
+                                    const uint32_t *perm, uint32_t mode, const uint32_t *crcp, uint32_t *sum, hipStream_t s) {
     const dim3 grid((nframes + 63) / 64);
     const uint32_t ab = (bnf_ablate_flags() & BNF_ABLATE_K_DECODE_ST) | (mode & BNF_MODE_K_DECODE_ST);
     if (ab & BNF_ABLATE_NO_ST) return hipSuccess;
 #if BNF_ST_FD
     (void)fmt;
-    hipLaunchKernelGGL(k_decode_st<BNF_OUT_FLACDECODER>, grid, dim3(64), 0, s, words, nbytes, nframes, sp, chn_lanes, out, out_bytes, info, perm, ab, crcp);
+    hipLaunchKernelGGL(k_decode_st<BNF_OUT_FLACDECODER>, grid, dim3(64), 0, s, words, nbytes, nframes, sp, chn_lanes, out, out_bytes, info, perm, ab, crcp, sum);
 #else
     switch (fmt) {
     case BNF_OUT_PLANAR32:
-        hipLaunchKernelGGL(k_decode_st<BNF_OUT_PLANAR32>, grid, dim3(64), 0, s, words, nbytes, nframes, sp, chn_lanes, out, out_bytes, info, perm, ab, crcp);
+        hipLaunchKernelGGL(k_decode_st<BNF_OUT_PLANAR32>, grid, dim3(64), 0, s, words, nbytes, nframes, sp, chn_lanes, out, out_bytes, info, perm, ab, crcp, sum);
         break;
     case BNF_OUT_INTERLEAVED32:
-        hipLaunchKernelGGL(k_decode_st<BNF_OUT_INTERLEAVED32>, grid, dim3(64), 0, s, words, nbytes, nframes, sp, chn_lanes, out, out_bytes, info, perm, ab, crcp);
+        hipLaunchKernelGGL(k_decode_st<BNF_OUT_INTERLEAVED32>, grid, dim3(64), 0, s, words, nbytes, nframes, sp, chn_lanes, out, out_bytes, info, perm, ab, crcp, sum);
         break;
     default:
-        hipLaunchKernelGGL(k_decode_st<BNF_OUT_FILEREADER>, grid, dim3(64), 0, s, words, nbytes, nframes, sp, chn_lanes, out, out_bytes, info, perm, ab, crcp);
+        hipLaunchKernelGGL(k_decode_st<BNF_OUT_FILEREADER>, grid, dim3(64), 0, s, words, nbytes, nframes, sp, chn_lanes, out, out_bytes, info, perm, ab, crcp, sum);
         break;
     }
 #endif
@@ -3660,18 +3699,18 @@
 extern "C" {
 hipError_t bnf_launch_decode_sw(const uint32_t *words, uint64_t nbytes, uint32_t nframes, bnf_stream_params sp,
                                     uint32_t chn_lanes, int fmt, uint8_t *out, uint64_t out_bytes, bnf_frame_info *info,
-                                    const uint32_t *perm, uint32_t mode, const uint32_t *crcp, hipStream_t s) {
+                                    const uint32_t *perm, uint32_t mode, const uint32_t *crcp, uint32_t *sum, hipStream_t s) {
     const dim3 grid((nframes + 63) / 64);
     const uint32_t ab = (bnf_ablate_flags() & BNF_ABLATE_K_DECODE_SW) | (mode & BNF_MODE_K_DECODE_SW);
     switch (fmt) {
     case BNF_OUT_PLANAR32:
-        hipLaunchKernelGGL(k_decode_sw<BNF_OUT_PLANAR32>, grid, dim3(64), 0, s, words, nbytes, nframes, sp, chn_lanes, out, out_bytes, info, perm, ab, crcp);
+        hipLaunchKernelGGL(k_decode_sw<BNF_OUT_PLANAR32>, grid, dim3(64), 0, s, words, nbytes, nframes, sp, chn_lanes, out, out_bytes, info, perm, ab, crcp, sum);
         break;
     case BNF_OUT_INTERLEAVED32:
-        hipLaunchKernelGGL(k_decode_sw<BNF_OUT_INTERLEAVED32>, grid, dim3(64), 0, s, words, nbytes, nframes, sp, chn_lanes, out, out_bytes, info, perm, ab, crcp);
+        hipLaunchKernelGGL(k_decode_sw<BNF_OUT_INTERLEAVED32>, grid, dim3(64), 0, s, words, nbytes, nframes, sp, chn_lanes, out, out_bytes, info, perm, ab, crcp, sum);
         break;
     case BNF_OUT_FILEREADER:
-        hipLaunchKernelGGL(k_decode_sw<BNF_OUT_FILEREADER>, grid, dim3(64), 0, s, words, nbytes, nframes, sp, chn_lanes, out, out_bytes, info, perm, ab, crcp);
+        hipLaunchKernelGGL(k_decode_sw<BNF_OUT_FILEREADER>, grid, dim3(64), 0, s, words, nbytes, nframes, sp, chn_lanes, out, out_bytes, info, perm, ab, crcp, sum);
         break;
     default: return hipErrorInvalidValue;
     }
@@ -3731,15 +3770,10 @@
 }
 
 #define ORDER_NB 256
-DEV uint32_t order_bucket(uint32_t work) { return 63u - min(work >> 8, 63u); }
 template <int MODE>
 DEV uint32_t order_key(const bnf_frame_info *__restrict__ info, const uint8_t *__restrict__ bytes, uint64_t nbytes,
                        const uint64_t *__restrict__ offs, uint32_t f) {
-    if (MODE == 0) {
-        const uint32_t st = info[f].status, fl = info[f].flags, bs = info[f].blocksize;
-        const uint32_t c = st != BNF_ST_OK ? 1u : (fl & BNF_FL_W32) ? 3u : (fl & BNF_FL_W16) ? 2u : (fl & BNF_FL_ST) ? 0u : 1u;
-        return c * 64u + order_bucket(bs ? bs - 1u : 0u);
-    }
+    if (MODE == 0) return order_key0(info[f].status, info[f].flags, info[f].blocksize);
     const uint64_t o = offs[f];
     if (o + 16u > nbytes) return 63u;
     const uint32_t code = bytes[o + 2] >> 4, chc = bytes[o + 3] >> 4;
@@ -3766,14 +3800,23 @@
     __syncthreads();
     const uint32_t f = blockIdx.x * 256u + threadIdx.x;
     if (f < nframes) atomicAdd(&h[order_key<MODE>(info, bytes, nbytes, offs, f)], 1u);
+    if (MODE == 0 && f < nframes) {
+        const uint32_t st = info[f].status;
+        if (st == BNF_ST_ERROR || st == BNF_ST_TRUNC) atomicAdd(&hist[ORDER_NB + BNF_SUM_NBAD], 1u);
+        if (info[f].flags & BNF_FL_REDO) atomicAdd(&hist[ORDER_NB + BNF_SUM_NREDO], 1u);
+    }
     __syncthreads();
     if (h[threadIdx.x]) atomicAdd(&hist[threadIdx.x], h[threadIdx.x]);
 }
-__global__ void __launch_bounds__(ORDER_NB) k_order_scan(uint32_t *__restrict__ hist, uint32_t *__restrict__ cls) {
+__global__ void __launch_bounds__(ORDER_NB) k_order_scan(const uint32_t *in, uint32_t *hist, uint32_t *__restrict__ cls,
+                                                         uint32_t *sum) {
     __shared__ uint32_t t[ORDER_NB];
+    __shared__ uint32_t onek;
     const uint32_t i = threadIdx.x;
-    const uint32_t v = hist[i];
+    const uint32_t v = in[i];
+    const uint32_t nbad_in = (sum && i == ORDER_NB - 1u) ? in[ORDER_NB + BNF_SUM_NBAD] : 0u;
     t[i] = v;
+    if (i == 0) onek = ~0u;
     __syncthreads();
     for (uint32_t o = 1; o < ORDER_NB; o <<= 1) {
         const uint32_t a = i >= o ? t[i - o] : 0u;
@@ -3788,13 +3831,35 @@
         cls[2] = t[ORDER_NB - 1u];
         cls[3] = t[2u * 64u - 1u] - t[64u - 1u];
     }
+    if (sum) {
+        const uint32_t total = t[ORDER_NB - 1u];
+        if (v != 0u && v == total) onek = i;
+        __syncthreads();
+        if (i == ORDER_NB - 1u) {
+            sum[BNF_SUM_ONE] = onek != ~0u ? 1u : 0u;
+            sum[BNF_SUM_KEY] = onek != ~0u ? onek : 0u;
+            sum[BNF_SUM_NW8] = t[2u * 64u - 1u] - t[64u - 1u];
+            sum[BNF_SUM_NLANE] = total - t[64u - 1u];
+            sum[BNF_SUM_SRC] = in == hist ? 1u : 2u;
+            if (in != hist) {
+                sum[BNF_SUM_NREDO] = 0u;
+                sum[BNF_SUM_NBAD] = nbad_in;
+                sum[BNF_SUM_WORDS - 1u] = 0u;
+            }
+        }
+    }
 }
 template <int MODE>
 __global__ void __launch_bounds__(256) k_order_place(const bnf_frame_info *__restrict__ info,
                                                      const uint8_t *__restrict__ bytes, uint64_t nbytes,
                                                      const uint64_t *__restrict__ offs, uint32_t nframes,
-                                                     uint32_t *__restrict__ off, uint32_t *__restrict__ perm) {
+                                                     uint32_t *__restrict__ off, uint32_t *__restrict__ perm,
+                                                     const uint32_t *__restrict__ sum) {
     __shared__ uint32_t h[ORDER_NB], base[ORDER_NB];
+    if (sum && sum[BNF_SUM_ONE]) {
+        if (blockIdx.x == 0 && threadIdx.x == 0) off[sum[BNF_SUM_KEY]] = nframes;
+        return;
+    }
     h[threadIdx.x] = 0;
     __syncthreads();
     const uint32_t f = blockIdx.x * 256u + threadIdx.x;
@@ -3811,14 +3876,19 @@
 template <int MODE>
 static hipError_t launch_order(const bnf_frame_info *info, const uint8_t *bytes, uint64_t nbytes, const uint64_t *offs,
                                uint32_t nframes, uint32_t *order, const uint32_t **perm, hipStream_t s,
-                               uint32_t *cls = nullptr) {
-    uint32_t *hist = order, *pm = order + ORDER_NB;
-    hipError_t e = hipMemsetAsync(hist, 0, ORDER_NB * sizeof(uint32_t), s);
-    if (e != hipSuccess) return e;
+                               uint32_t *cls = nullptr, bool early = false, const uint32_t *phist = nullptr) {
+    static_assert(ORDER_NB == BNF_ORDER_NB, "the summary follows the histogram");
+    uint32_t *hist = order, *sum = MODE == 0 ? order + ORDER_NB : nullptr, *pm = order + BNF_ORDER_HDR;
     const dim3 g((nframes + 255) / 256);
-    hipLaunchKernelGGL(k_order_count<MODE>, g, dim3(256), 0, s, info, bytes, nbytes, offs, nframes, hist);
-    hipLaunchKernelGGL(k_order_scan, dim3(1), dim3(ORDER_NB), 0, s, hist, cls);
-    hipLaunchKernelGGL(k_order_place<MODE>, g, dim3(256), 0, s, info, bytes, nbytes, offs, nframes, hist, pm);
+    if (MODE != 0 || !phist) {
+        phist = hist;
+        hipError_t e = hipMemsetAsync(hist, 0, BNF_ORDER_HDR * sizeof(uint32_t), s);
+        if (e != hipSuccess) return e;
+        hipLaunchKernelGGL(k_order_count<MODE>, g, dim3(256), 0, s, info, bytes, nbytes, offs, nframes, hist);
+    }
+    hipLaunchKernelGGL(k_order_scan, dim3(1), dim3(ORDER_NB), 0, s, phist, hist, cls, sum);
+    hipLaunchKernelGGL(k_order_place<MODE>, g, dim3(256), 0, s, info, bytes, nbytes, offs, nframes, hist, pm,
+                       early ? (const uint32_t *)sum : nullptr);
     *perm = pm;
     return hipGetLastError();
 }
@@ -3924,8 +3994,10 @@
 }
 hipError_t bnf_launch_parse(const uint32_t *words, uint64_t nbytes, const uint64_t *frame_offs, uint32_t nframes,
                             bnf_stream_params sp, const uint64_t *out_sample_in, uint64_t base_sample,
-                            bnf_frame_info *info, uint32_t *order, uint32_t *crcp, bool *handed, hipStream_t s) {
+                            bnf_frame_info *info, uint32_t *order, uint32_t *crcp, bool *handed, uint32_t *phist,
+                            bool *counted, hipStream_t s) {
     if (handed) *handed = false;
+    if (counted) *counted = false;
     if (!nframes || !nbytes) return hipSuccess;
     if (use_parse_wave(nframes, sp)) {
         static const uint32_t pws = getenv("BNFLAC_PW_STATS") ? 1u : 0u;
@@ -3952,36 +4024,45 @@
     }
     if (cm == 3) cm = 1;
     if (handed) *handed = cm != 0;
+    if (bnf_ablate_flags() & BNF_ABLATE_NO_EARLYOUT) phist = nullptr;
+    if (phist) {
+        hipError_t e = hipMemsetAsync(phist, 0, BNF_ORDER_HDR * sizeof(uint32_t), s);
+        if (e != hipSuccess) return e;
+        if (counted) *counted = true;
+    }
     const dim3 g((nframes + 63) / 64);
     if (cm == 2)
         hipLaunchKernelGGL(k_parse<2>, g, dim3(64), 0, s, words, nbytes, frame_offs, nframes, sp, out_sample_in,
-                           base_sample, info, bnf_ablate_flags() & BNF_ABLATE_K_PARSE, perm, crcp);
+                           base_sample, info, bnf_ablate_flags() & BNF_ABLATE_K_PARSE, perm, crcp, phist);
     else if (cm == 1)
         hipLaunchKernelGGL(k_parse<1>, g, dim3(64), 0, s, words, nbytes, frame_offs, nframes, sp, out_sample_in,
-                           base_sample, info, bnf_ablate_flags() & BNF_ABLATE_K_PARSE, perm, crcp);
+                           base_sample, info, bnf_ablate_flags() & BNF_ABLATE_K_PARSE, perm, crcp, phist);
     else
         hipLaunchKernelGGL(k_parse<0>, g, dim3(64), 0, s, words, nbytes, frame_offs, nframes, sp, out_sample_in,
-                           base_sample, info, bnf_ablate_flags() & BNF_ABLATE_K_PARSE, perm, nullptr);
+                           base_sample, info, bnf_ablate_flags() & BNF_ABLATE_K_PARSE, perm, nullptr, phist);
     return hipGetLastError();
 }
 
 hipError_t bnf_launch_fill_bad(const bnf_frame_info *info, uint32_t nframes, bnf_stream_params sp, int fmt,
-                               uint8_t *out, uint64_t out_bytes, hipStream_t s) {
+                               uint8_t *out, uint64_t out_bytes, const uint32_t *summary, hipStream_t s) {
     if (!nframes) return hipSuccess;
-    hipLaunchKernelGGL(k_fill_bad, dim3((nframes + 63) / 64), dim3(64), 0, s, info, nframes, sp, fmt, out, out_bytes);
+    hipLaunchKernelGGL(k_fill_bad, dim3((nframes + 63) / 64), dim3(64), 0, s, info, nframes, sp, fmt, out, out_bytes, summary);
     return hipGetLastError();
 }
 
 hipError_t bnf_launch_decode(const uint32_t *words, uint64_t nbytes, uint32_t nframes, bnf_stream_params sp,
                              uint32_t chn_lanes, int fmt, uint8_t *out, uint64_t out_bytes, bnf_frame_info *info,
-                             uint32_t *order, const uint32_t *crcp, hipStream_t s) {
+                             uint32_t *order, const uint32_t *crcp, const uint32_t *phist, const uint32_t **summary,
+                             hipStream_t s) {
+    if (summary) *summary = nullptr;
     if (!nframes || !nbytes) return hipSuccess;
+    if (bnf_ablate_flags() & BNF_ABLATE_NO_EARLYOUT) phist = nullptr;
     uint32_t mode = 0;
     if (order && use_decode_sys(nframes, sp, chn_lanes)) {
         const uint32_t *perm = nullptr;
-        uint32_t *list = order + 256u + nframes;
+        uint32_t *list = order + BNF_ORDER_HDR + nframes;
         hipError_t e = hipMemsetAsync(list, 0, 16, s);
-        if (e == hipSuccess) e = launch_order<0>(info, nullptr, 0, nullptr, nframes, order, &perm, s);
+        if (e == hipSuccess) e = launch_order<0>(info, nullptr, 0, nullptr, nframes, order, &perm, s, nullptr, false, phist);
         if (e == hipSuccess)
             e = bnf_launch_decode_sys(words, nbytes, nframes, sp, chn_lanes, fmt, out, out_bytes, info, perm, list, mode, s);
         if (e == hipSuccess)
@@ -4002,42 +4083,46 @@
                           __atomic_load_n(&cls[1], __ATOMIC_RELAXED) == 0u;
     const uint32_t *perm = nullptr;
     hipError_t e = hipSuccess;
-    if (order) e = launch_order<0>(info, nullptr, 0, nullptr, nframes, order, &perm, s, cls);
+    const uint32_t ab = bnf_ablate_flags();
+    const bool early = order && !(ab & BNF_ABLATE_NO_EARLYOUT);
+    if (order) e = launch_order<0>(info, nullptr, 0, nullptr, nframes, order, &perm, s, cls, early, phist);
+    uint32_t *sum = early ? order + BNF_ORDER_NB : nullptr;
+    if (summary && !(ab & BNF_ABLATE_NO_ST)) *summary = sum;
     const uint32_t *seg = (perm && seg_on) ? order : nullptr;
     if (seg_only) {
         sq = nullptr;
         lk.unlock();
     }
     const bool w8split = sq && seg && cls && __atomic_load_n(&cls[3], __ATOMIC_RELAXED) != 0u &&
-                         !(bnf_ablate_flags() & BNF_ABLATE_NO_W8SPLIT);
+                         !(ab & (BNF_ABLATE_NO_W8SPLIT | BNF_ABLATE_NO_ST));
     const int nside = w8split ? 3 : 2;
     auto fork = [&]() -> hipError_t {
         hipError_t r = hipEventRecord(sq->fork, s);
         for (int i = 0; i < nside && r == hipSuccess; i++) r = hipStreamWaitEvent(sq->st[i], sq->fork, 0);
         if (r == hipSuccess)
-            r = bnf_launch_decode_w32(words, nbytes, nframes, sp, chn_lanes, fmt, out, out_bytes, info, perm, mode, seg, sq->st[1]);
+            r = bnf_launch_decode_w32(words, nbytes, nframes, sp, chn_lanes, fmt, out, out_bytes, info, perm, mode, seg, sum, sq->st[1]);
         if (r == hipSuccess)
-            r = bnf_launch_decode_w16(words, nbytes, nframes, sp, chn_lanes, fmt, out, out_bytes, info, perm, mode, seg, sq->st[0]);
+            r = bnf_launch_decode_w16(words, nbytes, nframes, sp, chn_lanes, fmt, out, out_bytes, info, perm, mode, seg, sum, sq->st[0]);
         if (r == hipSuccess && w8split)
             r = bnf_launch_decode_w8(words, nbytes, nframes, sp, chn_lanes, fmt, out, out_bytes, info, perm,
-                                      mode | BNF_MODE_NOST, seg, sq->st[2]);
+                                      mode | BNF_MODE_NOST, seg, sum, sq->st[2]);
         for (int i = 0; i < nside && r == hipSuccess; i++) r = hipEventRecord(sq->join[i], sq->st[i]);
         return r;
     };
     if (sq && fm == 2 && e == hipSuccess) e = fork();
     if (sw) {
-        if (e == hipSuccess) e = bnf_launch_decode_sw(words, nbytes, nframes, sp, chn_lanes, fmt, out, out_bytes, info, perm, mode, crcp, s);
+        if (e == hipSuccess) e = bnf_launch_decode_sw(words, nbytes, nframes, sp, chn_lanes, fmt, out, out_bytes, info, perm, mode, crcp, sum, s);
         mode |= BNF_MODE_SW;
     }
     if (e == hipSuccess)
         e = fmt == BNF_OUT_FLACDECODER
-                ? bnf_launch_decode_st_fd(words, nbytes, nframes, sp, chn_lanes, fmt, out, out_bytes, info, perm, mode, crcp, s)
-                : bnf_launch_decode_st_any(words, nbytes, nframes, sp, chn_lanes, fmt, out, out_bytes, info, perm, mode, crcp, s);
+                ? bnf_launch_decode_st_fd(words, nbytes, nframes, sp, chn_lanes, fmt, out, out_bytes, info, perm, mode, crcp, sum, s)
+                : bnf_launch_decode_st_any(words, nbytes, nframes, sp, chn_lanes, fmt, out, out_bytes, info, perm, mode, crcp, sum, s);
     if (sq && fm == 1 && e == hipSuccess) e = fork();
     if (e == hipSuccess)
         e = w8split ? bnf_launch_decode_w8(words, nbytes, nframes, sp, chn_lanes, fmt, out, out_bytes, info, perm,
-                                            mode | BNF_MODE_STREDO, seg, s)
-                    : bnf_launch_decode_w8(words, nbytes, nframes, sp, chn_lanes, fmt, out, out_bytes, info, perm, mode, nullptr, s);
+                                            mode | BNF_MODE_STREDO, seg, sum, s)
+                    : bnf_launch_decode_w8(words, nbytes, nframes, sp, chn_lanes, fmt, out, out_bytes, info, perm, mode, nullptr, sum, s);
     if (sq) {
         for (int i = 0; i < nside; i++) {
             const hipError_t ej = hipStreamWaitEvent(s, sq->join[i], 0);
@@ -4047,10 +4132,10 @@
     } else if (seg_only) {
         g_seg_launches.fetch_add(1, std::memory_order_relaxed);
         if (e == hipSuccess)
-            e = bnf_launch_decode_seg(words, nbytes, nframes, sp, chn_lanes, fmt, out, out_bytes, info, perm, mode, seg, s);
+            e = bnf_launch_decode_seg(words, nbytes, nframes, sp, chn_lanes, fmt, out, out_bytes, info, perm, mode, seg, sum, s);
     } else {
-        if (e == hipSuccess) e = bnf_launch_decode_w16(words, nbytes, nframes, sp, chn_lanes, fmt, out, out_bytes, info, perm, mode, seg, s);
-        if (e == hipSuccess) e = bnf_launch_decode_w32(words, nbytes, nframes, sp, chn_lanes, fmt, out, out_bytes, info, perm, mode, seg, s);
+        if (e == hipSuccess) e = bnf_launch_decode_w16(words, nbytes, nframes, sp, chn_lanes, fmt, out, out_bytes, info, perm, mode, seg, sum, s);
+        if (e == hipSuccess) e = bnf_launch_decode_w32(words, nbytes, nframes, sp, chn_lanes, fmt, out, out_bytes, info, perm, mode, seg, sum, s);
     }
     return e;
 }
diff --git a/birdnest/audio_amd/csrc/bnflac_launch.h b/birdnest/audio_amd/csrc/bnflac_launch.h
--- a/birdnest/audio_amd/csrc/bnflac_launch.h
+++ b/birdnest/audio_amd/csrc/bnflac_launch.h
@@ -22,6 +22,7 @@
 #define BNF_ABLATE_SYS_MIXED 0x40000u
 #define BNF_ABLATE_SYS_LAND_ONLY 0x80000u
 #define BNF_ABLATE_NO_W8SPLIT 0x100000u
+#define BNF_ABLATE_NO_EARLYOUT 0x2000000u
 #define BNF_ABLATE_SYS_NO_RUN 0x200000u
 #define BNF_ABLATE_SYS_NO_PACK_FAST 0x400000u
 #define BNF_ABLATE_PARSE_BLKREFILL 0x800000u
@@ -62,7 +63,23 @@
 static_assert(!(BNF_ABLATE_K_DECODE_ST & BNF_MODE_K_DECODE_ST), "k_decode_st: an ablation bit is a mode bit");
 static_assert(!(BNF_ABLATE_K_DECODE_SW & BNF_MODE_K_DECODE_SW), "k_decode_sw: an ablation bit is a mode bit");
 static_assert(!(BNF_ABLATE_K_DECODE_SYS & BNF_MODE_K_DECODE_SYS), "k_decode_sys: an ablation bit is a mode bit");
-static_assert(!((BNF_ABLATE_NO_SW | BNF_ABLATE_NO_W8SPLIT) & BNF_MODE_MASK), "a host ablation bit is a mode bit");
+static_assert(!((BNF_ABLATE_NO_SW | BNF_ABLATE_NO_W8SPLIT | BNF_ABLATE_NO_EARLYOUT) & BNF_MODE_MASK), "a host ablation bit is a mode bit");
+static_assert(!(BNF_ABLATE_NO_EARLYOUT & (BNF_ABLATE_K_PARSE | BNF_ABLATE_K_DECODE | BNF_ABLATE_K_DECODE_ST | BNF_ABLATE_K_DECODE_SW |
+                                          BNF_ABLATE_K_DECODE_SYS | BNF_ABLATE_NO_SW | BNF_ABLATE_NO_W8SPLIT)),
+              "BNF_ABLATE_NO_EARLYOUT is another ablation bit");
+
+#define BNF_ORDER_NB 256u
+#define BNF_SUM_WORDS 8u
+#define BNF_ORDER_HDR (BNF_ORDER_NB + BNF_SUM_WORDS)
+enum {
+    BNF_SUM_ONE = 0,
+    BNF_SUM_KEY = 1,
+    BNF_SUM_NW8 = 2,
+    BNF_SUM_NREDO = 3,
+    BNF_SUM_NBAD = 4,
+    BNF_SUM_NLANE = 5,
+    BNF_SUM_SRC = 6
+};
 
 typedef struct {
     hipError_t (*upload_tables)(const uint8_t *crc8, const uint16_t *crc16x8, const uint16_t *xpow);
@@ -78,14 +95,14 @@
 #define BNF_DECODE_ARGS                                                                                              \
     const uint32_t *words, uint64_t nbytes, uint32_t nframes, bnf_stream_params sp, uint32_t chn_lanes, int fmt,   \
         uint8_t *out, uint64_t out_bytes, bnf_frame_info *info
-hipError_t bnf_launch_decode_w8(BNF_DECODE_ARGS, const uint32_t *perm, uint32_t mode, const uint32_t *seg, hipStream_t s);
-hipError_t bnf_launch_decode_w16(BNF_DECODE_ARGS, const uint32_t *perm, uint32_t mode, const uint32_t *seg, hipStream_t s);
-hipError_t bnf_launch_decode_w32(BNF_DECODE_ARGS, const uint32_t *perm, uint32_t mode, const uint32_t *seg, hipStream_t s);
+hipError_t bnf_launch_decode_w8(BNF_DECODE_ARGS, const uint32_t *perm, uint32_t mode, const uint32_t *seg, const uint32_t *sum, hipStream_t s);
+hipError_t bnf_launch_decode_w16(BNF_DECODE_ARGS, const uint32_t *perm, uint32_t mode, const uint32_t *seg, const uint32_t *sum, hipStream_t s);
+hipError_t bnf_launch_decode_w32(BNF_DECODE_ARGS, const uint32_t *perm, uint32_t mode, const uint32_t *seg, const uint32_t *sum, hipStream_t s);
 hipError_t bnf_launch_decode_list(BNF_DECODE_ARGS, const uint32_t *list, uint32_t mode, hipStream_t s);
-hipError_t bnf_launch_decode_seg(BNF_DECODE_ARGS, const uint32_t *perm, uint32_t mode, const uint32_t *seg, hipStream_t s);
-hipError_t bnf_launch_decode_st_fd(BNF_DECODE_ARGS, const uint32_t *perm, uint32_t mode, const uint32_t *crcp, hipStream_t s);
-hipError_t bnf_launch_decode_st_any(BNF_DECODE_ARGS, const uint32_t *perm, uint32_t mode, const uint32_t *crcp, hipStream_t s);
-hipError_t bnf_launch_decode_sw(BNF_DECODE_ARGS, const uint32_t *perm, uint32_t mode, const uint32_t *crcp, hipStream_t s);
+hipError_t bnf_launch_decode_seg(BNF_DECODE_ARGS, const uint32_t *perm, uint32_t mode, const uint32_t *seg, const uint32_t *sum, hipStream_t s);
+hipError_t bnf_launch_decode_st_fd(BNF_DECODE_ARGS, const uint32_t *perm, uint32_t mode, const uint32_t *crcp, uint32_t *sum, hipStream_t s);
+hipError_t bnf_launch_decode_st_any(BNF_DECODE_ARGS, const uint32_t *perm, uint32_t mode, const uint32_t *crcp, uint32_t *sum, hipStream_t s);
+hipError_t bnf_launch_decode_sw(BNF_DECODE_ARGS, const uint32_t *perm, uint32_t mode, const uint32_t *crcp, uint32_t *sum, hipStream_t s);
 hipError_t bnf_launch_decode_sys(BNF_DECODE_ARGS, const uint32_t *perm, uint32_t *redo, uint32_t mode, hipStream_t s);
 
 hipError_t bnf_upload_tables(const uint8_t *crc8, const uint16_t *crc16x8, const uint16_t *xpow);
@@ -102,12 +119,14 @@
 hipError_t bnf_parse_wave_stats(uint64_t *out8, int reset);
 hipError_t bnf_launch_parse(const uint32_t *words, uint64_t nbytes, const uint64_t *frame_offs, uint32_t nframes,
                             bnf_stream_params sp, const uint64_t *out_sample_in, uint64_t base_sample,
-                            bnf_frame_info *info, uint32_t *order, uint32_t *crcp, bool *handed, hipStream_t s);
+                            bnf_frame_info *info, uint32_t *order, uint32_t *crcp, bool *handed, uint32_t *phist,
+                            bool *counted, hipStream_t s);
 hipError_t bnf_launch_decode(const uint32_t *words, uint64_t nbytes, uint32_t nframes, bnf_stream_params sp,
                              uint32_t chn_lanes, int fmt, uint8_t *out, uint64_t out_bytes, bnf_frame_info *info,
-                             uint32_t *order, const uint32_t *crcp, hipStream_t s);
+                             uint32_t *order, const uint32_t *crcp, const uint32_t *phist, const uint32_t **summary,
+                             hipStream_t s);
 hipError_t bnf_launch_fill_bad(const bnf_frame_info *info, uint32_t nframes, bnf_stream_params sp, int fmt,
-                               uint8_t *out, uint64_t out_bytes, hipStream_t s);
+                               uint8_t *out, uint64_t out_bytes, const uint32_t *summary, hipStream_t s);
 hipError_t bnf_launch_chain(const uint8_t *bytes, uint64_t nbytes, const uint64_t *cand, uint32_t ncand,
                             const bnf_frame_info *info, uint64_t first_off, bnf_stream_params sp, uint32_t *gap_crc,
                             int32_t *jump, uint32_t levels, uint32_t *mark, uint32_t *pos, uint64_t *bs, uint8_t *small,
diff --git a/birdnest/audio_amd/csrc/bnflac_runtime.cpp b/birdnest/audio_amd/csrc/bnflac_runtime.cpp
--- a/birdnest/audio_amd/csrc/bnflac_runtime.cpp
+++ b/birdnest/audio_amd/csrc/bnflac_runtime.cpp
@@ -141,10 +141,15 @@
     CtxBuf cand, info, gap, jump, mark, pos, bs, small;
     CtxBuf ms;
     CtxBuf order, porder;
+    bool order_decoded = false;
     CtxBuf crcp;
     const void *crcp_bytes = nullptr, *crcp_info = nullptr;
     uint64_t crcp_nbytes = 0;
     uint32_t crcp_n = 0;
+    CtxBuf phist;
+    const void *phist_bytes = nullptr, *phist_info = nullptr;
+    uint64_t phist_nbytes = 0;
+    uint32_t phist_n = 0;
 };
 
 static bool crc_prefix_on() { return bnf_crc_mode() != 0; }
@@ -167,11 +172,22 @@
     return 0;
 }
 
+extern "C" BNFLAC_API int bnflac_debug_decode_summary(bnflac_ctx *ctx, uint32_t out8[8]) {
+    if (!ctx || !out8) return fail("bnflac_debug_decode_summary: null argument");
+    if (!ctx->order_decoded || !ctx->order.p) return fail("bnflac_debug_decode_summary: no decode on this context");
+    static_assert(BNF_SUM_WORDS == 8, "bnflac_debug_decode_summary copies 8 words");
+    DevGuard dg(ctx->device);
+    if (hipDeviceSynchronize() != hipSuccess ||
+        hipMemcpy(out8, (const uint32_t *)ctx->order.p + BNF_ORDER_NB, sizeof(uint32_t) * BNF_SUM_WORDS, hipMemcpyDeviceToHost) != hipSuccess)
+        return fail("bnflac_debug_decode_summary: HIP error");
+    return 0;
+}
+
 extern "C" BNFLAC_API void bnflac_ctx_destroy(bnflac_ctx *ctx) {
     if (!ctx) return;
     if (ctx->d_block_counts) (void)hipFree(ctx->d_block_counts);
     for (CtxBuf *b : {&ctx->cand, &ctx->info, &ctx->gap, &ctx->jump, &ctx->mark, &ctx->pos, &ctx->bs, &ctx->small,
-                      &ctx->ms, &ctx->order, &ctx->porder, &ctx->crcp})
+                      &ctx->ms, &ctx->order, &ctx->porder, &ctx->crcp, &ctx->phist})
         b->release();
     delete ctx;
 }
@@ -268,20 +284,28 @@
     DevGuard dg(ctx->device);
     bnf_stream_params p;
     memcpy(&p, sp, sizeof p);
-    if (!ctx->porder.grow(sizeof(uint32_t) * (256u + (size_t)nframes)))
+    if (!ctx->porder.grow(sizeof(uint32_t) * (BNF_ORDER_HDR + (size_t)nframes)))
         return fail("bnflac_parse_frames: out of device memory (parse-order scratch)");
     ctx->crcp_bytes = ctx->crcp_info = nullptr;
+    ctx->phist_bytes = ctx->phist_info = nullptr;
     const bool pre = crc_prefix_on() && ctx->crcp.grow(32u * std::max<size_t>(nframes, 1u));
-    bool handed = false;
+    const bool cnt = ctx->phist.grow(sizeof(uint32_t) * BNF_ORDER_HDR);
+    bool handed = false, counted = false;
     hipError_t e = bnf_launch_parse((const uint32_t *)d_bytes, nbytes, d_frame_offsets,
                                     nframes, p, d_out_sample, base_sample, (bnf_frame_info *)d_info,
                                     (uint32_t *)ctx->porder.p, pre ? (uint32_t *)ctx->crcp.p : nullptr, &handed,
-                                    (hipStream_t)hs);
+                                    cnt ? (uint32_t *)ctx->phist.p : nullptr, &counted, (hipStream_t)hs);
     if (e == hipSuccess && pre && handed) {
         ctx->crcp_bytes = d_bytes;
         ctx->crcp_info = d_info;
         ctx->crcp_nbytes = nbytes;
         ctx->crcp_n = nframes;
+    }
+    if (e == hipSuccess && counted) {
+        ctx->phist_bytes = d_bytes;
+        ctx->phist_info = d_info;
+        ctx->phist_nbytes = nbytes;
+        ctx->phist_n = nframes;
     }
     return e == hipSuccess ? 0 : fail(std::string("k_parse: ") + hipGetErrorString(e));
 }
@@ -294,17 +318,24 @@
     if (out_format < 0 || out_format > 3) return fail("bnflac_decode_parsed: bad out_format");
     bnf_stream_params p;
     memcpy(&p, sp, sizeof p);
-    if (!ctx->order.grow(sizeof(uint32_t) * (260u + 2u * (size_t)nframes)))
+    if (!ctx->order.grow(sizeof(uint32_t) * (BNF_ORDER_HDR + 4u + 2u * (size_t)nframes)))
         return fail("bnflac_decode_parsed: out of device memory (decode-order scratch)");
     const bool pre = ctx->crcp_bytes == d_bytes && ctx->crcp_info == d_info && ctx->crcp_nbytes == nbytes &&
                      ctx->crcp_n == nframes;
     ctx->crcp_bytes = ctx->crcp_info = nullptr;
+    const bool cnt = ctx->phist_bytes == d_bytes && ctx->phist_info == d_info && ctx->phist_nbytes == nbytes &&
+                     ctx->phist_n == nframes;
+    ctx->phist_bytes = ctx->phist_info = nullptr;
+    const uint32_t *summary = nullptr;
     hipError_t e = bnf_launch_decode((const uint32_t *)d_bytes, nbytes, nframes, p,
                                      lanes_for(sp->channels), out_format, d_out, out_bytes, (bnf_frame_info *)d_info,
                                      (uint32_t *)ctx->order.p, pre ? (const uint32_t *)ctx->crcp.p : nullptr,
+                                     cnt ? (const uint32_t *)ctx->phist.p : nullptr, &summary,
                                      (hipStream_t)hs);
+    ctx->order_decoded = e == hipSuccess && nframes && nbytes;
     if (e == hipSuccess)
-        e = bnf_launch_fill_bad((const bnf_frame_info *)d_info, nframes, p, out_format, d_out, out_bytes, (hipStream_t)hs);
+        e = bnf_launch_fill_bad((const bnf_frame_info *)d_info, nframes, p, out_format, d_out, out_bytes, summary,
+                                (hipStream_t)hs);
     return e == hipSuccess ? 0 : fail(std::string("k_decode: ") + hipGetErrorString(e));
 }
 
@@ -350,8 +381,9 @@
     bnf_stream_params p;
     memcpy(&p, sp, sizeof p);
     ctx->crcp_bytes = ctx->crcp_info = nullptr;
+    ctx->phist_bytes = ctx->phist_info = nullptr;
     hipError_t e = bnf_launch_parse((const uint32_t *)d_bytes, nbytes, (const uint64_t *)ctx->cand.p, ncand, p, nullptr,
-                                    0, (bnf_frame_info *)ctx->info.p, nullptr, nullptr, nullptr, s);
+                                    0, (bnf_frame_info *)ctx->info.p, nullptr, nullptr, nullptr, nullptr, nullptr, s);
     if (e == hipSuccess)
         e = bnf_launch_chain(d_bytes, nbytes, (const uint64_t *)ctx->cand.p, ncand, (const bnf_frame_info *)ctx->info.p,
                              first_offset, p, (uint32_t *)ctx->gap.p, (int32_t *)ctx->jump.p, levels,
@@ -376,6 +408,7 @@
     if (nstreams >= (1u << 30)) return fail("bnflac_index_streams: too many streams");
     hipStream_t s = (hipStream_t)hs;
     ctx->crcp_bytes = ctx->crcp_info = nullptr;
+    ctx->phist_bytes = ctx->phist_info = nullptr;
     if (!nstreams || !nbytes) {
         hipError_t e = hipMemsetAsync(d_status, 0, 4 * sizeof(uint32_t), s);
         if (e == hipSuccess) e = hipMemsetAsync(d_stream_frames, 0, sizeof(uint32_t) * ((size_t)nstreams + 1), s);
@@ -883,7 +916,7 @@
             }
             if (!d->d_info.grow(sizeof(bnf_frame_info) * ncand)) goto oom;
             if (bnf_launch_parse((const uint32_t *)d->d_bytes.p, n, (const uint64_t *)d->d_cand.p, ncand, sp,
-                                 nullptr, 0, (bnf_frame_info *)d->d_info.p, nullptr, nullptr, nullptr, d->stream) != hipSuccess)
+                                 nullptr, 0, (bnf_frame_info *)d->d_info.p, nullptr, nullptr, nullptr, nullptr, nullptr, d->stream) != hipSuccess)
                 goto hip_fail;
             if (hipMemcpyAsync(d->info.data(), d->d_info.p, sizeof(bnf_frame_info) * ncand, hipMemcpyDeviceToHost, d->stream) != hipSuccess)
                 goto hip_fail;
@@ -905,7 +938,7 @@
             spd.channels = pcm_ch;
             if (bnf_launch_decode((const uint32_t *)d->d_bytes.p, n, ncand, spd, lanes_for(pcm_ch), BNF_OUT_PLANAR32,
                                   (uint8_t *)d->d_pcm.p, (uint64_t)std::max<uint64_t>(tot, 1) * pcm_ch * 4,
-                                  (bnf_frame_info *)d->d_info.p, nullptr, nullptr, d->stream) != hipSuccess)
+                                  (bnf_frame_info *)d->d_info.p, nullptr, nullptr, nullptr, nullptr, d->stream) != hipSuccess)
                 goto hip_fail;
             d->pcm.resize((size_t)tot * pcm_ch);
             if (tot && hipMemcpyAsync(d->pcm.data(), d->d_pcm.p, sizeof(int32_t) * (size_t)tot * pcm_ch, hipMemcpyDeviceToHost, d->stream) != hipSuccess)
diff --git a/birdnest/audio_amd/libflac.py b/birdnest/audio_amd/libflac.py
--- a/birdnest/audio_amd/libflac.py
+++ b/birdnest/audio_amd/libflac.py
@@ -118,7 +118,7 @@
                  "bnflac_debug_set_decode_sys", "bnflac_debug_decode_seg_launches", "bnflac_md5_interleaved32", "bnflac_index_stream",
                  "bnflac_index_streams", "bnflac_md5_layout", "bnflac_md5_streams",
                  "bnflac_scan_streams", "bnflac_scan_stream_host",
-                 "bnflac_debug_set_crc_mode", "bnflac_debug_crc_handoff"]
+                 "bnflac_debug_set_crc_mode", "bnflac_debug_crc_handoff", "bnflac_debug_decode_summary"]
 READER_SYMBOLS = ["bnflac_reader_open", "bnflac_reader_params", "bnflac_reader_read", "bnflac_reader_close",
                   "bnflac_reader_last_error", "bnflac_reader_seek", "bnflac_reader_read_filereader",
                   "bnflac_reader_pool_release"]
@@ -171,6 +171,8 @@
     L.bnflac_debug_set_crc_mode.argtypes = [ctypes.c_int]
     L.bnflac_debug_crc_handoff.restype = i
     L.bnflac_debug_crc_handoff.argtypes = [p, p, ctypes.c_uint32]
+    if hasattr(L, "bnflac_debug_decode_summary"):
+        L.bnflac_debug_decode_summary.restype, L.bnflac_debug_decode_summary.argtypes = i, [p, p]
     L.bnflac_debug_decode_seg_launches.restype, L.bnflac_debug_decode_seg_launches.argtypes = ctypes.c_uint64, []
     L.bnflac_debug_parse_wave_stats.argtypes = [ctypes.POINTER(ctypes.c_uint64), ctypes.c_int]
     L.bnflac_debug_stats.argtypes = [ctypes.POINTER(ctypes.c_uint64), ctypes.c_int]
@@ -576,6 +578,13 @@
             raise RuntimeError(self.L.bnflac_last_error().decode())
         return a.reshape(nframes, 8)
 
+    def decode_summary(self) -> dict:
+        a = np.zeros(8, np.uint32)
+        if self.L.bnflac_debug_decode_summary(self.ctx, a.ctypes.data_as(ctypes.c_void_p)) != 0:
+            raise RuntimeError(self.L.bnflac_last_error().decode())
+        names = ("one_bucket", "key", "n_w8", "n_redo", "n_bad", "n_lane", "src")
+        return {k: int(v) for k, v in zip(names, a)}
+
 
 class Reader:
 
diff --git a/include/bnflac.h b/include/bnflac.h
--- a/include/bnflac.h
+++ b/include/bnflac.h
@@ -148,6 +148,8 @@
                                     uint64_t out_bytes, bnflac_frame_info *d_info, void *hip_stream);
 
 BNFLAC_API void bnflac_debug_set_ablate(uint32_t flags);
+#define BNFLAC_ABLATE_NO_EARLYOUT 0x2000000u
+BNFLAC_API int bnflac_debug_decode_summary(bnflac_ctx *ctx, uint32_t out8[8]);
 BNFLAC_API int bnflac_debug_crc_fold_check(void);
 BNFLAC_API void bnflac_debug_set_parse_wave(int mode);
 BNFLAC_API void bnflac_debug_set_decode_sys(int mode);
```

Result: no change. 769,200 MSamples/s (-0.5%).
